# epruesse/SINA

Hardware: AMD Instinct MI355X
Metric: aligned sequences/sec (whole node), 100k full-length 16S vs SILVA-NR-scale ref (higher is better)
Workload: dtype f32

## Files before the change

include/sina_hip.h:

```cpp
#ifndef SINA_HIP_H
#define SINA_HIP_H

#include <stddef.h>
#include <stdint.h>

#ifdef __cplusplus
extern "C" {
#endif

#define SINA_HIP_ABI_VERSION 5

typedef struct sina_hip_ctx sina_hip_ctx;


int sina_hip_abi_version(void);
const char *sina_hip_last_error(void);
int sina_hip_last_error_is_limit(void);

int sina_hip_init(int device, sina_hip_ctx **ctx);
int sina_hip_fork(sina_hip_ctx *parent, sina_hip_ctx **ctx);
int sina_hip_prewarm(sina_hip_ctx *ctx, int kind);
void sina_hip_destroy(sina_hip_ctx *ctx);
int sina_hip_sync(sina_hip_ctx *ctx);


int sina_hip_upload_refs(sina_hip_ctx *ctx, const uint32_t *ab, const uint64_t *off,
                         uint32_t n_refs, uint32_t width);

int sina_hip_build_index(sina_hip_ctx *ctx, unsigned k, int nofast);

int sina_hip_download_index(sina_hip_ctx *ctx, uint32_t *offsets, uint32_t *ids);

int sina_hip_upload_index(sina_hip_ctx *ctx, unsigned k, int nofast, const uint32_t *offsets,
                          const uint32_t *ids, uint64_t n_postings);

typedef struct sina_hip_store_view {
    void *ref_ab;       uint64_t ref_ab_bytes;
    void *ref_off;      uint64_t ref_off_bytes;
    void *idx_offsets;  uint64_t idx_offsets_bytes;
    void *idx_ids;      uint64_t idx_ids_bytes;
    uint32_t n_refs, width, k, nofast;
    uint64_t n_postings, total_bases;
} sina_hip_store_view;
int sina_hip_store_view_get(sina_hip_ctx *ctx, sina_hip_store_view *view);
int sina_hip_store_alloc_like(sina_hip_ctx *ctx, sina_hip_store_view *shape);

int sina_hip_kmer_topk(sina_hip_ctx *ctx, const uint8_t *qmask, const uint64_t *qoff, uint32_t nq,
                       uint32_t max, uint32_t *out_ids, float *out_scores, uint32_t *out_n);

int sina_hip_kmer_scores(sina_hip_ctx *ctx, const uint8_t *qmask, uint32_t qlen, int16_t *scores);

#define SINA_CMP_IUPAC_OPTIMISTIC 0
#define SINA_CMP_IUPAC_PESSIMISTIC 1
#define SINA_CMP_IUPAC_EXACT 2
typedef struct sina_hip_match_counts {
    int32_t only_a_overhang, only_b_overhang, only_a, only_b, match, mismatch;
} sina_hip_match_counts;
int sina_hip_compare(sina_hip_ctx *ctx, const uint32_t *q_ab, const uint64_t *q_off, uint32_t nq,
                     const uint32_t *cand_ids, const uint64_t *cand_off, int iupac_rule, int filter_lowercase,
                     sina_hip_match_counts *out);

enum { SINA_OVERHANG_ATTACH = 0, SINA_OVERHANG_REMOVE = 1, SINA_OVERHANG_EDGE = 2 };
enum { SINA_LOWERCASE_NONE = 0, SINA_LOWERCASE_ORIGINAL = 1, SINA_LOWERCASE_UNALIGNED = 2 };
enum { SINA_INSERTION_SHIFT = 0, SINA_INSERTION_FORBID = 1, SINA_INSERTION_REMOVE = 2 };

typedef struct sina_hip_align_params {
    float match_score;
    float mismatch_score;
    float gap_penalty;
    float gap_ext_penalty;
    float fs_weight;
    int32_t overhang;
    int32_t lowercase;
    int32_t insertion;
    const float *weights;
    uint32_t n_weights;
    int32_t assemble;
} sina_hip_align_params;
void sina_hip_align_params_default(sina_hip_align_params *p);
const uint32_t *sina_hip_staged_out_pos(sina_hip_ctx *ctx);

#define SINA_HIP_MAX_QUERY_LEN 10240u

typedef struct sina_hip_graph_batch {
    uint32_t nq;
    const uint64_t *node_off;
    const uint64_t *edge_off;
    const uint32_t *node_pos;
    const uint8_t *node_mask;
    const float *node_weight;
    const uint32_t *pred_off;
    const uint32_t *pred;
    const uint32_t *succ_minpos;
    uint32_t width;
    const float *node_score16;
    const float *self_score16;
} sina_hip_graph_batch;

typedef struct sina_hip_align_out {
    uint32_t end_m, end_s;
    float raw;
    float sum_weight;
    int32_t aligned_bases;
    int32_t cutoff_head, cutoff_tail;
    uint32_t n_out;
    int32_t status;
    uint32_t assembled;
    uint32_t nast_total, nast_longest, nast_last_run;
} sina_hip_align_out;

int sina_hip_align_graphs(sina_hip_ctx *ctx, const sina_hip_graph_batch *g, const uint8_t *qmask,
                          const uint64_t *qoff, const sina_hip_align_params *p,
                          sina_hip_align_out *out, uint32_t *out_pos);

#define SINA_HIP_WIDE_CELLS ((uint64_t)1 << 29)
int sina_hip_align_graphs_any(sina_hip_ctx *ctx, const sina_hip_graph_batch *g, const uint8_t *qmask,
                              const uint64_t *qoff, const sina_hip_align_params *p,
                              sina_hip_align_out *out, uint32_t *out_pos);
int sina_hip_wide_queries(sina_hip_ctx *ctx, uint64_t *n);

int sina_hip_align_families(sina_hip_ctx *ctx, const uint32_t *fam_ids, const uint64_t *fam_off,
                            uint32_t nq, const uint8_t *qmask, const uint64_t *qoff,
                            const sina_hip_align_params *p, sina_hip_align_out *out,
                            uint32_t *out_pos);

int sina_hip_align_profiles(sina_hip_ctx *ctx, const uint32_t *fam_ids, const uint64_t *fam_off,
                            uint32_t nq, const uint8_t *qmask, const uint64_t *qoff,
                            const sina_hip_align_params *p, sina_hip_align_out *out,
                            uint32_t *out_pos);

int sina_hip_debug_mesh(sina_hip_ctx *ctx, const sina_hip_graph_batch *g, const uint8_t *qmask,
                        uint32_t qlen, const sina_hip_align_params *p, uint32_t *tb_vm,
                        uint32_t *tb_vs, float *value, int prune);

int sina_hip_debug_mesh_wide(sina_hip_ctx *ctx, const sina_hip_graph_batch *g, const uint8_t *qmask,
                             uint32_t qlen, const sina_hip_align_params *p, uint32_t *tb_vm,
                             uint32_t *tb_vs, float *value);

typedef struct sina_hip_dp_info {
    uint32_t end_m, end_s;
    float raw;
    int32_t status;
    uint32_t rows_swept, cells_swept, attempts;
    float gain0, ubound;
    uint32_t prune_step, prune_gmin;
    float scout;
} sina_hip_dp_info;
int sina_hip_debug_dp_info(sina_hip_ctx *ctx, uint32_t q, sina_hip_dp_info *out);
int sina_hip_debug_rgain(sina_hip_ctx *ctx, uint32_t n, uint32_t *out, uint32_t *cols_right );

int sina_hip_debug_family_graph(sina_hip_ctx *ctx, const uint32_t *fam_ids, uint32_t F, float fs_weight,
                                uint32_t ring_depth, uint32_t *n_nodes, uint32_t *n_edges, uint32_t *pos,
                                uint8_t *mask, float *weight, uint32_t *pred_off, uint32_t *pred,
                                uint32_t *succ_minpos, uint8_t *sink, uint32_t *spill_idx, uint32_t cap_nodes,
                                uint32_t cap_edges);

int sina_hip_debug_family_profile(sina_hip_ctx *ctx, const uint32_t *fam_ids, uint32_t F, float match,
                                  float mismatch, float gap, float gap_ext, uint32_t *n_nodes, uint32_t *pos,
                                  float *score16, float *self16, uint32_t cap_nodes);

typedef struct sina_hip_stats {
    double dp_ms;
    double backtrack_ms;
    double graph_ms;
    double kmer_count_ms;
    double kmer_select_ms;
    uint64_t dp_cells;
    uint64_t postings;
    uint32_t dp_launches, kmer_launches;
    double compare_ms;
    uint64_t compare_bases;
    uint32_t compare_launches;
    uint32_t n_dense_lists;
    double dp_busy_ms;
    uint64_t dags_built;
    uint64_t dags_used;
    uint64_t dp_rows;
    uint64_t dp_rows_swept;
    uint64_t dp_cells_swept;
    uint64_t dp_queries_pruned;
    uint64_t dp_second_attempts;
    uint64_t dp_full_sweeps;
    double dp_prune_rho;
    uint64_t graph_bytes;
    uint32_t graph_launches, kmer_queries;
    double scout_ms;
    uint32_t scout_launches, pad_;
} sina_hip_stats;
int sina_hip_get_stats(sina_hip_ctx *ctx, sina_hip_stats *s);

#ifdef __cplusplus
}
#endif
#endif
```

sina_amd/capi.py:

```python
import ctypes as C
import os

import numpy as np

_HERE = os.path.dirname(os.path.abspath(__file__))
LIB_PATH = os.path.abspath(os.environ["SINA_HIP_LIB"]) if os.environ.get("SINA_HIP_LIB") else os.path.join(_HERE, "libsina_hip.so")

u8p = C.POINTER(C.c_uint8)
u32p = C.POINTER(C.c_uint32)
u64p = C.POINTER(C.c_uint64)
f32p = C.POINTER(C.c_float)
i16p = C.POINTER(C.c_int16)

ABI_SYMBOLS = [
    "sina_hip_abi_version", "sina_hip_last_error", "sina_hip_init", "sina_hip_fork", "sina_hip_prewarm", "sina_hip_destroy",
    "sina_hip_sync",
    "sina_hip_upload_refs", "sina_hip_build_index", "sina_hip_download_index", "sina_hip_upload_index", "sina_hip_store_view_get",
    "sina_hip_store_alloc_like", "sina_hip_kmer_topk", "sina_hip_kmer_scores", "sina_hip_compare",
    "sina_hip_align_params_default", "sina_hip_staged_out_pos", "sina_hip_align_graphs", "sina_hip_align_families",
    "sina_hip_align_profiles", "sina_hip_debug_family_profile",
    "sina_hip_debug_mesh", "sina_hip_debug_family_graph", "sina_hip_debug_dp_info", "sina_hip_debug_rgain", "sina_hip_get_stats",
    "sina_hip_align_graphs_any", "sina_hip_debug_mesh_wide", "sina_hip_wide_queries", "sina_hip_last_error_is_limit",
]


class AlignParams(C.Structure):
    _fields_ = [("match_score", C.c_float), ("mismatch_score", C.c_float), ("gap_penalty", C.c_float),
                ("gap_ext_penalty", C.c_float), ("fs_weight", C.c_float), ("overhang", C.c_int32),
                ("lowercase", C.c_int32), ("insertion", C.c_int32), ("weights", f32p),
                ("n_weights", C.c_uint32), ("assemble", C.c_int32)]


class GraphBatch(C.Structure):
    _fields_ = [("nq", C.c_uint32), ("node_off", u64p), ("edge_off", u64p), ("node_pos", u32p),
                ("node_mask", u8p), ("node_weight", f32p), ("pred_off", u32p), ("pred", u32p),
                ("succ_minpos", u32p), ("width", C.c_uint32), ("node_score16", f32p), ("self_score16", f32p)]


class AlignOut(C.Structure):
    _fields_ = [("end_m", C.c_uint32), ("end_s", C.c_uint32), ("raw", C.c_float), ("sum_weight", C.c_float),
                ("aligned_bases", C.c_int32), ("cutoff_head", C.c_int32), ("cutoff_tail", C.c_int32),
                ("n_out", C.c_uint32), ("status", C.c_int32), ("assembled", C.c_uint32),
                ("nast_total", C.c_uint32), ("nast_longest", C.c_uint32), ("nast_last_run", C.c_uint32)]


ALIGN_OUT_DTYPE = np.dtype([("end_m", "<u4"), ("end_s", "<u4"), ("raw", "<f4"), ("sum_weight", "<f4"),
                            ("aligned_bases", "<i4"), ("cutoff_head", "<i4"), ("cutoff_tail", "<i4"),
                            ("n_out", "<u4"), ("status", "<i4"), ("assembled", "<u4"), ("nast_total", "<u4"),
                            ("nast_longest", "<u4"), ("nast_last_run", "<u4")])


class StoreView(C.Structure):
    _fields_ = [("ref_ab", C.c_void_p), ("ref_ab_bytes", C.c_uint64), ("ref_off", C.c_void_p),
                ("ref_off_bytes", C.c_uint64), ("idx_offsets", C.c_void_p), ("idx_offsets_bytes", C.c_uint64),
                ("idx_ids", C.c_void_p), ("idx_ids_bytes", C.c_uint64), ("n_refs", C.c_uint32),
                ("width", C.c_uint32), ("k", C.c_uint32), ("nofast", C.c_uint32), ("n_postings", C.c_uint64),
                ("total_bases", C.c_uint64)]


class Stats(C.Structure):
    _fields_ = [("dp_ms", C.c_double), ("backtrack_ms", C.c_double), ("graph_ms", C.c_double),
                ("kmer_count_ms", C.c_double), ("kmer_select_ms", C.c_double), ("dp_cells", C.c_uint64),
                ("postings", C.c_uint64), ("dp_launches", C.c_uint32), ("kmer_launches", C.c_uint32),
                ("compare_ms", C.c_double), ("compare_bases", C.c_uint64), ("compare_launches", C.c_uint32),
                ("n_dense_lists", C.c_uint32), ("dp_busy_ms", C.c_double), ("dags_built", C.c_uint64),
                ("dags_used", C.c_uint64), ("dp_rows", C.c_uint64), ("dp_rows_swept", C.c_uint64),
                ("dp_cells_swept", C.c_uint64), ("dp_queries_pruned", C.c_uint64), ("dp_second_attempts", C.c_uint64),
                ("dp_full_sweeps", C.c_uint64), ("dp_prune_rho", C.c_double), ("graph_bytes", C.c_uint64),
                ("graph_launches", C.c_uint32), ("kmer_queries", C.c_uint32), ("scout_ms", C.c_double),
                ("scout_launches", C.c_uint32), ("pad_", C.c_uint32)]


class DpInfo(C.Structure):
    _fields_ = [("end_m", C.c_uint32), ("end_s", C.c_uint32), ("raw", C.c_float), ("status", C.c_int32),
                ("rows_swept", C.c_uint32), ("cells_swept", C.c_uint32), ("attempts", C.c_uint32),
                ("gain0", C.c_float), ("ubound", C.c_float), ("prune_step", C.c_uint32), ("prune_gmin", C.c_uint32),
                ("scout", C.c_float)]


_lib = None


def load():
    global _lib
    if _lib is not None:
        return _lib
    if not os.path.exists(LIB_PATH):
        raise RuntimeError("sina_amd/libsina_hip.so is missing: run `python -c 'import __graft_entry__ as g; "
                           "g.build()'` (hipcc --offload-arch=gfx950). There is no CPU fallback.")
    L = C.CDLL(LIB_PATH)
    vp = C.c_void_p
    L.sina_hip_abi_version.restype = C.c_int
    L.sina_hip_last_error.restype = C.c_char_p
    L.sina_hip_init.argtypes = [C.c_int, C.POINTER(vp)]
    L.sina_hip_fork.argtypes = [vp, C.POINTER(vp)]
    L.sina_hip_prewarm.argtypes = [vp, C.c_int]
    L.sina_hip_destroy.argtypes = [vp]
    L.sina_hip_destroy.restype = None
    L.sina_hip_sync.argtypes = [vp]
    L.sina_hip_staged_out_pos.restype = C.POINTER(C.c_uint32)
    L.sina_hip_staged_out_pos.argtypes = [vp]
    L.sina_hip_upload_refs.argtypes = [vp, u32p, u64p, C.c_uint32, C.c_uint32]
    L.sina_hip_build_index.argtypes = [vp, C.c_uint, C.c_int]
    L.sina_hip_upload_index.argtypes = [vp, C.c_uint, C.c_int, u32p, u32p, C.c_uint64]
    L.sina_hip_download_index.argtypes = [vp, u32p, u32p]
    L.sina_hip_store_view_get.argtypes = [vp, C.POINTER(StoreView)]
    L.sina_hip_store_alloc_like.argtypes = [vp, C.POINTER(StoreView)]
    L.sina_hip_kmer_topk.argtypes = [vp, u8p, u64p, C.c_uint32, C.c_uint32, u32p, f32p, u32p]
    L.sina_hip_kmer_scores.argtypes = [vp, u8p, C.c_uint32, i16p]
    L.sina_hip_compare.argtypes = [vp, u32p, u64p, C.c_uint32, u32p, u64p, C.c_int, C.c_int, C.c_void_p]
    L.sina_hip_align_params_default.argtypes = [C.POINTER(AlignParams)]
    L.sina_hip_align_params_default.restype = None
    L.sina_hip_align_graphs.argtypes = [vp, C.POINTER(GraphBatch), u8p, u64p, C.POINTER(AlignParams),
                                        C.POINTER(AlignOut), u32p]
    L.sina_hip_align_graphs_any.argtypes = L.sina_hip_align_graphs.argtypes
    L.sina_hip_wide_queries.argtypes = [vp, u64p]
    L.sina_hip_last_error_is_limit.restype = C.c_int
    L.sina_hip_debug_mesh_wide.argtypes = [vp, C.POINTER(GraphBatch), u8p, C.c_uint32, C.POINTER(AlignParams),
                                           u32p, u32p, f32p]
    L.sina_hip_align_families.argtypes = [vp, u32p, u64p, C.c_uint32, u8p, u64p, C.POINTER(AlignParams),
                                          C.POINTER(AlignOut), u32p]
    L.sina_hip_align_profiles.argtypes = L.sina_hip_align_families.argtypes
    L.sina_hip_debug_family_profile.argtypes = [vp, u32p, C.c_uint32, C.c_float, C.c_float, C.c_float, C.c_float, u32p, u32p,
                                                f32p, f32p, C.c_uint32]
    L.sina_hip_debug_mesh.argtypes = [vp, C.POINTER(GraphBatch), u8p, C.c_uint32, C.POINTER(AlignParams),
                                      u32p, u32p, f32p, C.c_int]
    L.sina_hip_debug_family_graph.argtypes = [vp, u32p, C.c_uint32, C.c_float, C.c_uint32, u32p, u32p, u32p, u8p,
                                              f32p, u32p, u32p, u32p, u8p, u32p, C.c_uint32, C.c_uint32]
    L.sina_hip_get_stats.argtypes = [vp, C.POINTER(Stats)]
    L.sina_hip_debug_dp_info.argtypes = [vp, C.c_uint32, C.POINTER(DpInfo)]
    L.sina_hip_debug_rgain.argtypes = [vp, C.c_uint32, u32p, u32p]
    _lib = L
    return L


class SinaHipError(RuntimeError):
    pass


def _ptr(a, t):
    return a.ctypes.data_as(t)


def _c(a, dt):
    return np.ascontiguousarray(a, dtype=dt)


class Context:

    def __init__(self, device=0, _parent=None):
        self.L = load()
        self.h = C.c_void_p()
        if _parent is None:
            self._check(self.L.sina_hip_init(device, C.byref(self.h)))
        else:
            self._check(self.L.sina_hip_fork(_parent.h, C.byref(self.h)))
        self._parent = _parent
        self.device = device
        self.n_refs = 0 if _parent is None else _parent.n_refs

    def fork(self):
        return Context(self.device, _parent=self)

    def _check(self, rc):
        if rc != 0:
            raise SinaHipError(self.L.sina_hip_last_error().decode())

    def close(self):
        if self.h:
            self.L.sina_hip_destroy(self.h)
            self.h = C.c_void_p()

    def __del__(self):
        try:
# ... 91 lines not shown
        gb.succ_minpos = _ptr(arrs["succ_minpos"], u32p) if "succ_minpos" in arrs else None
        gb.width = width
        if node_score16 is not None:
            arrs["node_score16"] = _c(np.asarray(node_score16).reshape(-1), np.float32)
            arrs["self_score16"] = _c(self_score16, np.float32)
            assert len(arrs["node_score16"]) == 16 * int(node_off[nq]) and len(arrs["self_score16"]) == 16
            gb.node_score16 = _ptr(arrs["node_score16"], f32p)
            gb.self_score16 = _ptr(arrs["self_score16"], f32p)
        gb._keep = arrs
        return gb

    def align_graphs(self, gb, qmask, qoff, params=None):
        params = params or self.params()
        qmask = _c(qmask, np.uint8)
        qoff = _c(qoff, np.uint64)
        out = np.zeros(gb.nq, ALIGN_OUT_DTYPE)
        pos = np.zeros(max(len(qmask), 1), np.uint32)
        self._check(self.L.sina_hip_align_graphs(self.h, C.byref(gb), _ptr(qmask, u8p), _ptr(qoff, u64p),
                                                 C.byref(params), out.ctypes.data_as(C.POINTER(AlignOut)),
                                                 _ptr(pos, u32p)))
        return out, pos

    def align_graphs_any(self, gb, qmask, qoff, params=None, staged=False):
        params = params or self.params()
        qmask = _c(qmask, np.uint8)
        qoff = _c(qoff, np.uint64)
        out = np.zeros(gb.nq, ALIGN_OUT_DTYPE)
        pos = np.zeros(max(len(qmask), 1), np.uint32)
        self._check(self.L.sina_hip_align_graphs_any(self.h, C.byref(gb), _ptr(qmask, u8p), _ptr(qoff, u64p),
                                                     C.byref(params), out.ctypes.data_as(C.POINTER(AlignOut)),
                                                     None if staged else _ptr(pos, u32p)))
        if staged:
            n = int(qoff[-1] - qoff[0])
            pos[:n] = np.ctypeslib.as_array(self.L.sina_hip_staged_out_pos(self.h), shape=(max(n, 1),))[:n]
        return out, pos

    def wide_queries(self):
        n = C.c_uint64()
        self._check(self.L.sina_hip_wide_queries(self.h, C.byref(n)))
        return int(n.value)

    def last_error_is_limit(self):
        return bool(self.L.sina_hip_last_error_is_limit())

    def debug_mesh_wide(self, gb, qmask, params=None, want_value=True):
        params = params or self.params()
        qmask = _c(qmask, np.uint8)
        n = int(gb._keep["node_off"][1])
        L = len(qmask)
        vm = np.zeros((n, L), np.uint32)
        vs = np.zeros((n, L), np.uint32)
        val = np.zeros((n, L), np.float32) if want_value else None
        self._check(self.L.sina_hip_debug_mesh_wide(self.h, C.byref(gb), _ptr(qmask, u8p), L, C.byref(params),
                                                    _ptr(vm, u32p), _ptr(vs, u32p),
                                                    _ptr(val, f32p) if want_value else None))
        return vm, vs, val

    def compare(self, q_ab, q_off, cand_ids, cand_off, iupac=0, filter_lc=False):
        q_ab = _c(q_ab, np.uint32)
        q_off = _c(q_off, np.uint64)
        cand_ids = _c(cand_ids, np.uint32)
        cand_off = _c(cand_off, np.uint64)
        out = np.zeros((max(len(cand_ids), 1), 6), np.int32)
        self._check(self.L.sina_hip_compare(self.h, _ptr(q_ab, u32p), _ptr(q_off, u64p), len(q_off) - 1,
                                            _ptr(cand_ids, u32p), _ptr(cand_off, u64p), int(iupac),
                                            int(filter_lc), out.ctypes.data_as(C.c_void_p)))
        return out[:len(cand_ids)]

    def align_families(self, fam_ids, fam_off, qmask, qoff, params=None):
        params = params or self.params()
        fam_ids = _c(fam_ids, np.uint32)
        fam_off = _c(fam_off, np.uint64)
        qmask = _c(qmask, np.uint8)
        qoff = _c(qoff, np.uint64)
        nq = len(qoff) - 1
        out = np.zeros(nq, ALIGN_OUT_DTYPE)
        pos = np.zeros(max(len(qmask), 1), np.uint32)
        self._check(self.L.sina_hip_align_families(self.h, _ptr(fam_ids, u32p), _ptr(fam_off, u64p), nq,
                                                   _ptr(qmask, u8p), _ptr(qoff, u64p), C.byref(params),
                                                   out.ctypes.data_as(C.POINTER(AlignOut)), _ptr(pos, u32p)))
        return out, pos

    def align_profiles(self, fam_ids, fam_off, qmask, qoff, params=None):
        params = params or self.params()
        fam_ids = _c(fam_ids, np.uint32)
        fam_off = _c(fam_off, np.uint64)
        qmask = _c(qmask, np.uint8)
        qoff = _c(qoff, np.uint64)
        nq = len(qoff) - 1
        out = np.zeros(nq, ALIGN_OUT_DTYPE)
        pos = np.zeros(max(len(qmask), 1), np.uint32)
        self._check(self.L.sina_hip_align_profiles(self.h, _ptr(fam_ids, u32p), _ptr(fam_off, u64p), nq,
                                                   _ptr(qmask, u8p), _ptr(qoff, u64p), C.byref(params),
                                                   out.ctypes.data_as(C.POINTER(AlignOut)), _ptr(pos, u32p)))
        return out, pos

    def debug_family_profile(self, fam_ids, match, mismatch, gap, gap_ext):
        fam_ids = _c(fam_ids, np.uint32)
        cap = 65536
        nn = C.c_uint32()
        pos = np.zeros(cap, np.uint32)
        sc = np.zeros((cap, 16), np.float32)
        own = np.zeros(16, np.float32)
        self._check(self.L.sina_hip_debug_family_profile(self.h, _ptr(fam_ids, u32p), len(fam_ids), match, mismatch, gap,
                                                         gap_ext, C.byref(nn), _ptr(pos, u32p), _ptr(sc, f32p),
                                                         _ptr(own, f32p), cap))
        return pos[:nn.value].copy(), sc[:nn.value].copy(), own

    def debug_mesh(self, gb, qmask, params=None, want_value=True, prune=False):
        params = params or self.params()
        qmask = _c(qmask, np.uint8)
        n = int(gb._keep["node_off"][1])
        L = len(qmask)
        vm = np.zeros((n, L), np.uint32)
        vs = np.zeros((n, L), np.uint32)
        val = np.zeros((n, L), np.float32) if want_value else None
        self._check(self.L.sina_hip_debug_mesh(self.h, C.byref(gb), _ptr(qmask, u8p), L, C.byref(params),
                                               _ptr(vm, u32p), _ptr(vs, u32p),
                                               _ptr(val, f32p) if want_value else None, 1 if prune else 0))
        return vm, vs, val

    def debug_family_graph(self, fam_ids, fs_weight=1.0, ring_depth=4):
        fam_ids = _c(fam_ids, np.uint32)
        cap_n, cap_e = 65536, 400000
        nn, ne = C.c_uint32(), C.c_uint32()
        pos = np.zeros(cap_n, np.uint32)
        mask = np.zeros(cap_n, np.uint8)
        w = np.zeros(cap_n, np.float32)
        poff = np.zeros(cap_n + 1, np.uint32)
        pred = np.zeros(cap_e, np.uint32)
        smin = np.zeros(cap_n, np.uint32)
        sink = np.zeros(cap_n, np.uint8)
        spill = np.zeros(cap_n, np.uint32)
        self._check(self.L.sina_hip_debug_family_graph(self.h, _ptr(fam_ids, u32p), len(fam_ids), fs_weight,
                                                       ring_depth, C.byref(nn), C.byref(ne), _ptr(pos, u32p),
                                                       _ptr(mask, u8p), _ptr(w, f32p), _ptr(poff, u32p),
                                                       _ptr(pred, u32p), _ptr(smin, u32p), _ptr(sink, u8p),
                                                       _ptr(spill, u32p), cap_n, cap_e))
        n, e = nn.value, ne.value
        return dict(n=n, pos=pos[:n].copy(), mask=mask[:n].copy(), weight=w[:n].copy(), pred_off=poff[:n + 1].copy(),
                    pred=pred[:e].copy(), succ_minpos=smin[:n].copy(), sink=sink[:n].copy(), spill=spill[:n].copy())

    def dp_info(self, q=0):
        d = DpInfo()
        self._check(self.L.sina_hip_debug_dp_info(self.h, q, C.byref(d)))
        return {f[0]: getattr(d, f[0]) for f in DpInfo._fields_}

    def rgain(self, n):
        out = np.zeros(max(n, 1), np.uint32)
        cols = np.zeros(max(n, 1), np.uint32)
        self._check(self.L.sina_hip_debug_rgain(self.h, n, _ptr(out, u32p), _ptr(cols, u32p)))
        return out[:n], cols[:n]

    def stats(self):
        s = Stats()
        self._check(self.L.sina_hip_get_stats(self.h, C.byref(s)))
        return {f[0]: getattr(s, f[0]) for f in Stats._fields_}
```

sina_amd/csrc/api.hip:

```cpp
#include <algorithm>
#include <cmath>
#include <cstdlib>
#include <cstring>

#include "common.h"
#include "ctx.h"

namespace sina_hip {

static thread_local std::string g_last_error;
static thread_local bool g_last_error_is_limit = false;
void set_error(const std::string &msg) {
    g_last_error = msg;
    g_last_error_is_limit = false;
}
void set_limit_error(const std::string &msg) {
    g_last_error = msg;
    g_last_error_is_limit = true;
}

int plan_dp(sina_hip_ctx *c, uint32_t maxL, DpPlan *pl) {
    if (!pick_geom(maxL, &pl->geom)) SH_FAIL_LIMIT("align: query longer than SINA_HIP_MAX_QUERY_LEN bases");
    const size_t slot = dp_slot_bytes(pl->geom), fixed = dp_fixed_lds_bytes(pl->geom);
    size_t budget = c->lds_budget ? c->lds_budget : dp_default_lds_budget(pl->geom);
// ... 19 lines not shown
    pp.kappa64 = 64.0f * 1.0001f * kappa;
    pp.amax = prune_gain_units(wmax, pp.kappa64);
    if (pp.amax > 250u || (uint64_t)pp.amax * maxL >= (1u << 23)) return pp;
    if (pp.kappa64 <= 0.f) pp.kappa64 = 1e-30f;
    DpGeom g;
    if (pick_geom(maxL, &g) && g.T <= 64) return pp;
    pp.on = 1;
    return pp;
}

struct HostPrep {
    std::vector<QDesc> qd;
    std::vector<uint4> rec;
    std::vector<uint2> rgain;
    bool rgain_ok = true;
    float wmax = 0.f, wmin = 0.f;
    std::vector<uint32_t> pred;
    std::vector<uint32_t> last;
    uint64_t tb_cells = 0, spill_rows = 0, cells = 0;
};

static int prep_range(const sina_hip_graph_batch *g, const uint64_t *qoff, uint32_t q0, uint32_t q1, int Lp, int W,
                       HostPrep *hp, float kappa64, uint32_t *spill_q) {
    const uint64_t nbase = g->node_off[q0], ebase = g->edge_off[q0];
    const uint64_t nn = g->node_off[q1] - nbase;
    hp->qd.resize(q1 - q0);
    hp->rec.resize(nn);
    hp->rgain.assign(kappa64 > 0.f ? nn : 0, uint2{0u, 0u});
    hp->rgain_ok = true;
    hp->pred.resize(g->edge_off[q1] - ebase + 8);
    hp->tb_cells = hp->spill_rows = hp->cells = 0;
    uint32_t erec_cursor = 0;
    for (uint32_t q = q0; q < q1; q++) {
        QDesc &d = hp->qd[q - q0];
        const uint64_t no = g->node_off[q], eo = g->edge_off[q];
        const uint32_t N = (uint32_t)(g->node_off[q + 1] - no);
        d.node_off = no - nbase;
        d.erec_off = erec_cursor;
        erec_cursor += dp_edge_entries(N);
        d.edge_off = eo - ebase;
        d.q_off = qoff[q] - qoff[q0];
        d.tb_off = hp->tb_cells;
        d.spill_off = hp->spill_rows;
        d.N = N;
        d.L = (uint32_t)(qoff[q + 1] - qoff[q]);
        const uint32_t *po = g->pred_off + no + q;
        uint4 *rec = hp->rec.data() + d.node_off;
        for (uint32_t m = 0; m < N; m++) {
            if (po[m + 1] < po[m]) SH_FAIL("align_graphs: a node has more than 255 predecessors (or pred_off is not ascending)");
            if (po[m + 1] - po[m] > 255u)
                SH_FAIL_LIMIT("align_graphs: a node has more than 255 predecessors (or pred_off is not ascending)");
            for (uint32_t e = po[m]; e < po[m + 1]; e++)
                if (g->pred[eo + e] >= m) SH_FAIL("align_graphs: predecessor ids must be smaller than the node's id");
            uint32_t wbits;
            memcpy(&wbits, &g->node_weight[no + m], 4);
            rec[m].x = po[m];
            rec[m].y = wbits;
            rec[m].z = ((po[m + 1] - po[m]) & 0xffu) | ((uint32_t)(g->node_mask[no + m] & 0xffu) << 8) | kRecSink;
            rec[m].w = kRowNone;
        }
        std::vector<uint32_t> &last = hp->last;
        last.assign(N, 0);
        for (uint32_t m = 0; m < N; m++) {
            for (uint32_t e = po[m]; e < po[m + 1]; e++) {
                const uint32_t p = g->pred[eo + e];
                rec[p].z &= ~kRecSink;
                last[p] = m;
                if (m - p > (uint32_t)kFarLds) rec[p].z |= kRecFence;
            }
        }
        d.first_sink = 0;
        d.gmin = 0;
        for (uint32_t m = 0; m < N; m++)
            if (rec[m].z & kRecSink) {
                d.first_sink = m;
                break;
            }
        uint32_t nsp = 0;
        uint32_t free_at[64];
        const uint32_t seg_len = dp_slot_segment(N);
        for (uint32_t m = 0; m < N; m++) {
            if (m % seg_len == 0)
                for (int x = 0; x < W; x++) free_at[x] = 0;
            if (rec[m].z & kRecSink) continue;
            if (last[m] == m + 1) continue;
            int slot = -1;
            const uint32_t seg_end = std::min<uint32_t>(N, (m / seg_len + 1) * seg_len);
            if (!(rec[m].z & kRecFence) && last[m] < seg_end)
                for (int x = 0; x < W; x++)
                    if (free_at[x] <= m) {
                        slot = x;
                        break;
                    }
            if (slot >= 0) {
                free_at[slot] = last[m];
                rec[m].w = (uint32_t)slot;
            } else {
                rec[m].w = kRowSpilled | nsp++;
            }
        }
        for (uint32_t m = 0; m < N; m++) {
            uint32_t first_far = 0;
            uint32_t dist = po[m + 1] > po[m] ? 0u : kRecDistFar;
            for (uint32_t e = po[m]; e < po[m + 1]; e++) {
                const uint32_t p = g->pred[eo + e];
                const uint32_t pw = rec[p].w == kRowNone ? 0u : rec[p].w;
                const bool sp = (pw & kRowSpilled) != 0;
                if (sp && first_far == 0) first_far = e - po[m] + 1;
                dist = std::max(dist, m - p);
                hp->pred[d.edge_off + e] = p | ((pw & 0x7FFFu) << 16) | (sp ? kPredSpilled : 0u);
            }
            rec[m].z |= (first_far << 24) | (std::min(dist, kRecDistFar) << kRecDistShift);
        }
        if (nsp > kMaxSpillRows) {
            if (spill_q) *spill_q = q;
            SH_FAIL_LIMIT("align_graphs: too many spill rows for one query");
        }
        if (kappa64 > 0.f) {
            uint2 *rg = hp->rgain.data() + d.node_off;
            const uint32_t *pos = g->node_pos + no;
            bool ok = true;
            for (uint32_t m = 0; m < N && ok; m++) {
                if (m > 0 && pos[m] < pos[m - 1]) ok = false;
                for (uint32_t e = po[m]; e < po[m + 1] && ok; e++)
                    if (pos[g->pred[eo + e]] >= pos[m]) ok = false;
            }
            if (!ok) hp->rgain_ok = false;
            uint32_t right = 0, cols_right = 0, gmin = 0xFFFFFFFFu;
            for (uint32_t m = N; ok && m > 0;) {
                uint32_t first = m - 1, mx = 0;
                while (first > 0 && pos[first - 1] == pos[m - 1]) first--;
                for (uint32_t j = first; j < m; j++) {
                    mx = std::max(mx, prune_gain_units(g->node_weight[no + j], kappa64));
                    rg[j] = uint2{right, last[j] | (cols_right << 16)};
                }
                right += mx;
                cols_right++;
                gmin = std::min(gmin, mx);
                m = first;
            }
            d.gmin = ok ? gmin : 0u;
        }
        d.n_spill = nsp;
        hp->spill_rows += nsp;
        hp->tb_cells += (uint64_t)N * Lp;
        hp->cells += (uint64_t)N * d.L;
    }
    return 0;
}

int run_dp_device(sina_hip_ctx *c, const DpPlan &pl, const QDesc *qd_host, uint32_t bq, uint64_t n_node_entries,
                  uint64_t tb_cells, uint64_t spill_rows, uint64_t cells, uint64_t nqm, const sina_hip_align_params *p, uint32_t width,
                  sina_hip_align_out *out, uint32_t *out_pos, bool want_dbg_value, const PrunePlan &pp,
                  const uint32_t *chain_ref) {
    hipStream_t s = c->stream;
    const int Lp = pl.geom.Lp();
    const bool weighted = p->weights != nullptr && p->n_weights > 0;
    const bool forbid = p->insertion == SINA_INSERTION_FORBID;
    uint64_t edge_entries = 0;
    for (uint32_t q = 0; q < bq; q++) edge_entries += dp_edge_entries(qd_host[q].N);
    (void)n_node_entries;
    if (c->spill.reserve(std::max<uint64_t>(spill_rows, 1) * 8 * (uint64_t)Lp) ||
        c->edge.reserve(std::max<uint64_t>(1, (uint64_t)(pl.geom.T / 64 - 1) * edge_entries) * sizeof(EdgeRec)) ||
        c->res.reserve(sizeof(DpResult) * bq) || c->out.reserve(sizeof(sina_hip_align_out) * bq) ||
        c->out_pos.reserve(4 * std::max<uint64_t>(nqm, 1)))
        return 1;
    if (want_dbg_value && c->dbg.reserve(4 * tb_cells)) return 1;
    std::vector<uint32_t> order(bq);
    for (uint32_t q = 0; q < bq; q++) order[q] = q;
    std::stable_sort(order.begin(), order.end(), [&](uint32_t x, uint32_t y) {
        return (uint64_t)qd_host[x].N * qd_host[x].L > (uint64_t)qd_host[y].N * qd_host[y].L;
    });
    if (c->order.reserve(4 * (size_t)bq)) return 1;
    if (upload(c, 0, c->order.p, order.data(), 4 * (size_t)bq, s)) return 1;
    DpArgs a;
    a.dry = DryArgs{nullptr, nullptr, 0};
    a.qd = c->qd.as<QDesc>();
    a.order = c->order.as<uint32_t>();
    a.rec = c->rec.as<uint4>();
    a.pred = c->pred.as<uint32_t>();
    a.node_pos = c->node_pos.as<uint32_t>();
    a.succ_minpos = c->succ_minpos.as<uint32_t>();
    a.qmask = c->qmask.as<uint8_t>();
    a.tb = nullptr;
    a.dbg_value = want_dbg_value ? c->dbg.as<float>() : nullptr;
    a.spill = c->spill.as<float>();
    a.edge = c->edge.as<EdgeRec>();
    a.edge_stride = edge_entries;
    a.res = c->res.as<DpResult>();
    a.weights = weighted ? c->weights.as<float>() : nullptr;
    a.n_weights = weighted ? p->n_weights : 0;
    a.ms = -p->match_score;
    a.mms = -p->mismatch_score;
    a.gp = p->gap_penalty;
    a.gpe = p->gap_ext_penalty;
    a.prof16 = c->profile_batch ? c->prof16.as<float>() : nullptr;
    c->last_bq = bq;
    c->last_prune_step = pp.on ? pp.amax : 0u;
    a.reach = pp.on ? c->rgain.as<uint2>() : nullptr;
    a.prune = pp.on;
    a.prune_amax = pp.amax;
    a.prune_rho = 0.f;
    bool rho_fixed = false;
    if (pp.on) {
        if (const std::string r = test_knob("rho"); !r.empty()) {
            a.prune_rho = (float)atof(r.c_str());
            rho_fixed = a.prune_rho > 0.f;
        }
        if (!rho_fixed) {
            std::lock_guard<std::mutex> slk(c->st->stats_mu);
            a.prune_rho = c->st->prune_rho;
        }
    }
    {
        uint32_t max_n = 0;
        for (uint32_t q = 0; q < bq; q++) max_n = std::max<uint32_t>(max_n, qd_host[q].N);
        a.below_init = (!weighted && !forbid && dp_below_init(max_n, a.gp, a.gpe)) ? 1 : 0;
    }
    a.scout_u = nullptr;
    a.scout_bias = (float)atof(test_knob("scout_add").c_str());
    c->last_scout = false;
    if (const std::string fixed = test_knob("scout_set"); !fixed.empty() && pp.on && !rho_fixed) {
        std::vector<float> vals(bq, (float)atof(fixed.c_str()));
        if (c->scout_u.reserve(4 * (size_t)bq)) return 1;
        if (upload(c, 7, c->scout_u.p, vals.data(), 4 * (size_t)bq, s)) return 1;
        a.scout_u = c->scout_u.as<float>();
        c->last_scout = true;
    } else if (chain_ref != nullptr && pp.on && !rho_fixed && a.below_init && a.gp >= a.gpe && pl.geom.T > 64 && test_knob("scout") != "0") {
        if (c->scout.reserve(4 * (size_t)bq) || c->scout_u.reserve(4 * (size_t)bq)) return 1;
        if (upload(c, 7, c->scout.p, chain_ref, 4 * (size_t)bq, s)) return 1;
        SH_CHECK(hipEventRecord(c->ev[3], s));
        if (launch_chain_scout(a, bq, c->st->ref_ab.as<uint32_t>(), c->st->ref_off.as<uint64_t>(), c->scout.as<uint32_t>(),
                               c->scout_u.as<float>(), s))
            return 1;
        SH_CHECK(hipEventRecord(c->ev[4], s));
        SH_CHECK(wait_event(c->ev[4]));
        float sms = 0;
        SH_CHECK(hipEventElapsedTime(&sms, c->ev[3], c->ev[4]));
        {
            std::lock_guard<std::mutex> slk(c->st->stats_mu);
            c->st->stats.scout_ms += sms;
            c->st->stats.scout_launches++;
        }
        a.scout_u = c->scout_u.as<float>();
        c->last_scout = true;
    }
    if (a.scout_u != nullptr && !rho_fixed) {
        std::lock_guard<std::mutex> slk(c->st->stats_mu);
        a.prune_rho = c->st->prune_rho_guard;
    }
    const uint64_t tb_bytes = tb_cell_bytes(forbid) * tb_cells;
    tb_plane_lease plane;
    if (plane.acquire(c, std::max<uint64_t>(tb_bytes, 16))) return 1;
    c->last_tb = plane.ptr;
    a.tb = plane.ptr;
    if (want_dbg_value && pp.on) SH_CHECK(hipMemsetD32Async(reinterpret_cast<hipDeviceptr_t>(c->dbg.p), 0x49742400 , tb_cells, s));
    if (c->dbg_planes && !forbid) SH_CHECK(hipMemsetD16Async(reinterpret_cast<hipDeviceptr_t>(plane.ptr), (unsigned short)kTbNone, tb_cells, s));

    BtArgs b;
    b.qd = a.qd;
    b.rec = a.rec;
    b.pred = a.pred;
    b.node_pos = a.node_pos;
    b.tb = a.tb;
    b.res = a.res;
    b.weights = a.weights;
    b.n_weights = a.n_weights;
    b.out = c->out.as<sina_hip_align_out>();
    b.out_pos = c->out_pos.as<uint32_t>();
    b.nq = bq;
    b.width = width;
    b.Lp = (uint32_t)Lp;
    b.ms = a.ms;
    b.overhang = p->overhang;
    b.lazy_sidx = forbid ? 0 : 1;
    b.qmask = a.qmask;
    b.lowercase = p->lowercase;
    b.self16 = c->profile_batch ? c->self16.as<float>() : nullptr;
    b.asm_cap = 0;
    for (uint32_t q = 0; q < bq; q++) b.asm_cap = std::max<uint32_t>(b.asm_cap, qd_host[q].L);
    uint64_t dp_no = ~0ull;
    bool bt_done = false;
    {
        SH_CHECK(hipEventRecord(c->ev[8], s));
        s = c->stream_dp;
        SH_CHECK(hipStreamWaitEvent(s, c->ev[8], 0));
        heavy_launch hl(c, s, kHeavyDp);
        SH_CHECK(hipEventRecord(c->ev[0], hl.stream()));
        a.dry = hl.dry();
        if (launch_mesh_dp(pl.geom, weighted, forbid, a, bq, pl.lds, hl.stream())) return 1;
        SH_CHECK(hipEventRecord(c->ev[1], hl.stream()));
        if (hl.lk.owns_lock() && c->st->dp_end[0]) {
            dp_no = c->st->dp_seq++;
            SH_CHECK(hipEventRecord(c->st->dp_end[dp_no % 8], hl.stream()));
            c->st->dp_end_no[dp_no % 8].store(dp_no, std::memory_order_release);
        }
        if (hl.chained) {
            if (launch_backtrack(b, hl.stream())) return 1;
            if (p->assemble && launch_assemble(b, hl.stream())) return 1;
            SH_CHECK(hipEventRecord(c->ev[2], hl.stream()));
            bt_done = true;
        }
        if (hl.done()) return 1;
    }
    if (!bt_done) {
        if (launch_backtrack(b, s)) return 1;
        if (p->assemble && launch_assemble(b, s)) return 1;
        SH_CHECK(hipEventRecord(c->ev[2], s));
    }
    if (c->h_out.reserve(sizeof(sina_hip_align_out) * bq) || c->h_res.reserve(sizeof(DpResult) * bq)) return 1;
    unsigned char *staged_pos = static_cast<unsigned char *>(c->h_out_pos.p) + 4 * c->out_pos_base;
    SH_CHECK(hipMemcpyAsync(c->h_out.p, c->out.p, sizeof(sina_hip_align_out) * bq, hipMemcpyDeviceToHost, s));
    SH_CHECK(hipMemcpyAsync(c->h_res.p, c->res.p, sizeof(DpResult) * bq, hipMemcpyDeviceToHost, s));
    SH_CHECK(hipMemcpyAsync(staged_pos, c->out_pos.p, 4 * nqm, hipMemcpyDeviceToHost, s));
    SH_CHECK(wait_stream(c, s));
    memcpy(out, c->h_out.p, sizeof(sina_hip_align_out) * bq);
    if (out_pos) memcpy(out_pos, staged_pos, 4 * nqm);
    float ms = 0;
    SH_CHECK(hipEventElapsedTime(&ms, c->ev[0], c->ev[1]));
    float shared = 0;
    if (dp_no != ~0ull && dp_no > 0 && c->st->dp_end_no[(dp_no - 1) % 8].load(std::memory_order_acquire) == dp_no - 1) {
        float to_prev_end = 0;
        const hipError_t e = hipEventElapsedTime(&to_prev_end, c->ev[0], c->st->dp_end[(dp_no - 1) % 8]);
        if (e == hipSuccess && c->st->dp_end_no[(dp_no - 1) % 8].load(std::memory_order_acquire) == dp_no - 1)
            shared = std::min(ms, std::max(0.f, to_prev_end));
        else (void)hipGetLastError();
    }
    const uint32_t kstrip = 64u * (uint32_t)pl.geom.B;
    uint64_t rows_nominal = 0, rows_swept = 0, cells_swept = 0, n_pruned = 0, n_second = 0, n_full = 0;
    std::vector<float> ratios;
    const DpResult *hres = c->h_res.as<DpResult>();
    for (uint32_t q = 0; q < bq; q++) {
        const uint64_t strips = (qd_host[q].L - 1) / kstrip + 1;
        rows_nominal += strips * qd_host[q].N;
        const DpResult &r = hres[q];
        if (r.attempts == 0) {
            rows_swept += strips * qd_host[q].N;
            cells_swept += (uint64_t)qd_host[q].N * qd_host[q].L;
            continue;
        }
        rows_swept += r.rows_done;
        cells_swept += r.cells_done;
        n_pruned++;
        n_second += r.attempts == 2 ? 1 : 0;
        n_full += r.attempts >= 3 ? 1 : 0;
        if (r.status == 0 && r.gain0 > 0.f && r.raw < 0.f) ratios.push_back(-r.raw / r.gain0);
    }
    float rho_seen = -1.f, rho_guard_seen = -1.f;
    if (!ratios.empty()) {
        rho_seen = *std::min_element(ratios.begin(), ratios.end()) - 0.015f;
        const size_t at = ratios.size() / 50;
        std::nth_element(ratios.begin(), ratios.begin() + (std::ptrdiff_t)at, ratios.end());
        rho_guard_seen = ratios[at] - 0.015f;
    }
    std::lock_guard<std::mutex> slk(c->st->stats_mu);
    c->st->stats.dp_ms += ms;
    c->st->stats.dp_busy_ms += ms - shared;
    SH_CHECK(hipEventElapsedTime(&ms, c->ev[1], c->ev[2]));
    c->st->stats.backtrack_ms += ms;
    c->st->stats.dp_cells += cells;
    c->st->stats.dp_launches++;
    c->st->stats.dp_rows += rows_nominal;
    c->st->stats.dp_rows_swept += rows_swept;
    c->st->stats.dp_cells_swept += cells_swept;
    c->st->stats.dp_queries_pruned += n_pruned;
    c->st->stats.dp_second_attempts += n_second;
    c->st->stats.dp_full_sweeps += n_full;
    if (rho_seen > 0.f) {
        float &rho = c->st->prune_rho;
        rho = rho_seen < rho ? rho_seen : 0.5f * (rho + rho_seen);
        rho = std::min(0.99f, std::max(0.05f, rho));
        float &rg = c->st->prune_rho_guard;
        rg = rho_guard_seen < rg ? rho_guard_seen : 0.5f * (rg + rho_guard_seen);
        rg = std::min(0.99f, std::max(0.05f, rg));
    }
    c->st->stats.dp_prune_rho = c->st->prune_rho;
    return 0;
}

int make_streams(sina_hip_ctx *c) {
    SH_CHECK(hipStreamCreateWithFlags(&c->stream, hipStreamNonBlocking));
    SH_CHECK(hipStreamCreateWithFlags(&c->stream_dp, hipStreamNonBlocking));
    return 0;
}

int upload_weights(sina_hip_ctx *c, const sina_hip_align_params *p) {
    if (p->weights != nullptr && p->n_weights > 0) {
        if (c->weights.reserve(sizeof(float) * p->n_weights)) return 1;
        SH_CHECK(hipMemcpyAsync(c->weights.p, p->weights, sizeof(float) * p->n_weights, hipMemcpyHostToDevice,
                                c->stream));
    }
    return 0;
}

static bool weighted_scheme(const sina_hip_align_params *p) { return p->weights != nullptr && p->n_weights > 0; }

static int align_graphs_impl(sina_hip_ctx *c, const sina_hip_graph_batch *g, const uint8_t *qmask,
                             const uint64_t *qoff, const sina_hip_align_params *p, sina_hip_align_out *out,
// ... 322 lines not shown
    c->free_all();
    for (auto &e : c->ev) (void)hipEventDestroy(e);
    (void)hipStreamDestroy(c->stream);
    if (c->stream_dp) (void)hipStreamDestroy(c->stream_dp);
    delete c;
}

int sina_hip_sync(sina_hip_ctx *c) {
    if (!c) SH_FAIL("sync: null ctx");
    SH_CHECK(hipSetDevice(c->device));
    SH_CHECK(hipStreamSynchronize(c->stream));
    SH_CHECK(hipStreamSynchronize(c->stream_dp));
    if (c->st->heavy) SH_CHECK(hipStreamSynchronize(c->st->heavy));
    if (c->st->heavy2) SH_CHECK(hipStreamSynchronize(c->st->heavy2));
    return 0;
}

const uint32_t *sina_hip_staged_out_pos(sina_hip_ctx *c) {
    return c ? static_cast<const uint32_t *>(c->h_out_pos.p) : nullptr;
}

void sina_hip_align_params_default(sina_hip_align_params *p) {
    memset(p, 0, sizeof(*p));
    p->match_score = 2;
    p->mismatch_score = -1;
    p->gap_penalty = 5;
    p->gap_ext_penalty = 2;
    p->fs_weight = 1;
    p->overhang = SINA_OVERHANG_ATTACH;
    p->lowercase = SINA_LOWERCASE_NONE;
    p->insertion = SINA_INSERTION_SHIFT;
}

int sina_hip_upload_refs(sina_hip_ctx *c, const uint32_t *ab, const uint64_t *off, uint32_t n_refs,
                         uint32_t width) {
    if (!c || !ab || !off) SH_FAIL("upload_refs: null argument");
    if (!c->owns_store) SH_FAIL("upload_refs: a forked context cannot change the reference store");
    std::lock_guard<std::mutex> lk(c->mu);
    SH_CHECK(hipSetDevice(c->device));
    const uint64_t total = off[n_refs];
    if (c->st->ref_ab.reserve(4 * std::max<uint64_t>(total, 1)) || c->st->ref_off.reserve(8 * ((uint64_t)n_refs + 1)))
        return 1;
    SH_CHECK(hipMemcpyAsync(c->st->ref_ab.p, ab, 4 * total, hipMemcpyHostToDevice, c->stream));
    SH_CHECK(hipMemcpyAsync(c->st->ref_off.p, off, 8 * ((uint64_t)n_refs + 1), hipMemcpyHostToDevice, c->stream));
    SH_CHECK(hipStreamSynchronize(c->stream));
    {
        std::lock_guard<std::mutex> alk(c->st->aux_mu);
        c->st->ref_off_host.assign(off, off + n_refs + 1);
        c->st->ref_off_host_ready.store(true, std::memory_order_release);
    }
    c->st->n_refs = n_refs;
    c->st->width = width;
    c->st->total_bases = total;
    c->st->have_refs = true;
    return 0;
}

int sina_hip_align_graphs(sina_hip_ctx *c, const sina_hip_graph_batch *g, const uint8_t *qmask,
                          const uint64_t *qoff, const sina_hip_align_params *p, sina_hip_align_out *out,
                          uint32_t *out_pos) {
    if (!c) SH_FAIL("align_graphs: null ctx");
    std::lock_guard<std::mutex> lk(c->mu);
    sina_hip_hint_guard hints(c);
    return align_graphs_impl(c, g, qmask, qoff, p, out, out_pos, nullptr, nullptr, nullptr);
}

int sina_hip_align_graphs_any(sina_hip_ctx *c, const sina_hip_graph_batch *g, const uint8_t *qmask,
                              const uint64_t *qoff, const sina_hip_align_params *p, sina_hip_align_out *out,
                              uint32_t *out_pos) {
    if (!c) SH_FAIL("align_graphs_any: null ctx");
    std::lock_guard<std::mutex> lk(c->mu);
    sina_hip_hint_guard hints(c);
    return align_graphs_any_impl(c, g, qmask, qoff, p, out, out_pos);
}

int sina_hip_wide_queries(sina_hip_ctx *c, uint64_t *n) {
    if (!c || !n) SH_FAIL("wide_queries: null argument");
    std::lock_guard<std::mutex> lk(c->mu);
    *n = c->wide_queries;
    return 0;
}

int sina_hip_debug_mesh_wide(sina_hip_ctx *c, const sina_hip_graph_batch *g, const uint8_t *qmask, uint32_t qlen,
                             const sina_hip_align_params *p, uint32_t *tb_vm, uint32_t *tb_vs, float *value) {
    if (!c || !g || g->nq != 1 || !qmask || !p || !tb_vm || !tb_vs) SH_FAIL("debug_mesh_wide: needs exactly one query");
    std::lock_guard<std::mutex> lk(c->mu);
    SH_CHECK(hipSetDevice(c->device));
    if (p->insertion == SINA_INSERTION_FORBID && !g->succ_minpos) SH_FAIL("debug_mesh_wide: insertion=forbid needs succ_minpos");
    if (g->node_score16 != nullptr && (!g->self_score16 || weighted_scheme(p)))
        SH_FAIL("debug_mesh_wide: a profile batch needs self_score16 and takes no positional weights");
    const uint64_t qoff[2] = {0, qlen};
    std::vector<uint8_t> wide;
    if (classify_any(g, qoff, true, &wide)) return 1;
    if (c->h_out_pos.reserve(4 * std::max<uint64_t>(qlen, 1))) return 1;
    sina_hip_align_out o;
    const uint32_t q0 = 0;
    return run_wide(c, g, qmask, qoff, p, &q0, 1, &o, nullptr, tb_vm, tb_vs, value);
}

int sina_hip_debug_mesh(sina_hip_ctx *c, const sina_hip_graph_batch *g, const uint8_t *qmask, uint32_t qlen,
                        const sina_hip_align_params *p, uint32_t *tb_vm, uint32_t *tb_vs, float *value, int prune) {
    if (!c || !g || g->nq != 1 || !tb_vm || !tb_vs) SH_FAIL("debug_mesh: needs exactly one query");
    std::lock_guard<std::mutex> lk(c->mu);
    struct no_prune_scope {
        sina_hip_ctx *c;
        ~no_prune_scope() { c->no_prune = false; }
    } scope{c};
    c->no_prune = prune == 0;
    const uint64_t qoff[2] = {0, qlen};
    sina_hip_align_out o;
    std::vector<uint32_t> pos(qlen);
    return align_graphs_impl(c, g, qmask, qoff, p, &o, pos.data(), value, tb_vm, tb_vs);
}

int sina_hip_debug_dp_info(sina_hip_ctx *c, uint32_t q, sina_hip_dp_info *out) {
    if (!c || !out) SH_FAIL("debug_dp_info: null argument");
    std::lock_guard<std::mutex> lk(c->mu);
    if (q >= c->last_bq || !c->res.p) SH_FAIL("debug_dp_info: no such query in the last launch");
    SH_CHECK(hipSetDevice(c->device));
    DpResult r;
    SH_CHECK(hipMemcpy(&r, c->res.as<DpResult>() + q, sizeof r, hipMemcpyDeviceToHost));
    out->end_m = r.end_m;
    out->end_s = r.end_s;
    out->raw = r.raw;
    out->status = r.status;
    out->rows_swept = r.rows_done;
    out->cells_swept = r.cells_done;
    out->attempts = r.attempts;
    out->gain0 = r.gain0;
    out->ubound = r.ubound;
    out->prune_step = c->last_prune_step;
    QDesc d;
    SH_CHECK(hipMemcpy(&d, c->qd.as<QDesc>() + q, sizeof d, hipMemcpyDeviceToHost));
    out->prune_gmin = d.gmin;
    out->scout = NAN;
    if (c->last_scout && c->scout_u.p) SH_CHECK(hipMemcpy(&out->scout, c->scout_u.as<float>() + q, sizeof(float), hipMemcpyDeviceToHost));
    return 0;
}

int sina_hip_debug_rgain(sina_hip_ctx *c, uint32_t n, uint32_t *out, uint32_t *cols_right) {
    if (!c || !out) SH_FAIL("debug_rgain: null argument");
    std::lock_guard<std::mutex> lk(c->mu);
    if (!c->rgain.p || c->rgain.cap < 8 * (size_t)n) SH_FAIL("debug_rgain: no bound of that many nodes on the device");
    SH_CHECK(hipSetDevice(c->device));
    std::vector<uint2> tmp(n);
    SH_CHECK(hipMemcpy(tmp.data(), c->rgain.p, 8 * (size_t)n, hipMemcpyDeviceToHost));
    for (uint32_t i = 0; i < n; i++) {
        out[i] = tmp[i].x;
        if (cols_right) cols_right[i] = tmp[i].y >> 16;
    }
    return 0;
}

int sina_hip_get_stats(sina_hip_ctx *c, sina_hip_stats *s) {
    if (!c || !s) SH_FAIL("get_stats: null argument");
    std::lock_guard<std::mutex> slk(c->st->stats_mu);
    *s = c->st->stats;
    s->n_dense_lists = c->st->dense_ready.load() ? c->st->n_dense : 0;
    return 0;
}

}
```

sina_amd/csrc/common.h:

```cpp
#pragma once

#include <hip/hip_runtime.h>
#include <stdint.h>

#include <algorithm>
#include <atomic>
#include <mutex>
#include <string>
#include <vector>

#include <cstdio>
#include <cstdlib>
#include <ctime>

#include "sina_hip.h"

namespace sina_hip {

void set_error(const std::string &msg);
void set_limit_error(const std::string &msg);

inline std::string test_knob(const char *key) {
    const char *e = getenv("SINA_HIP_TEST");
    if (!e) return std::string();
// ... 37 lines not shown
        if (bytes <= cap) return 0;
        if (p) (void)hipFree(p);
        p = nullptr;
        cap = 0;
        size_t want = bytes + bytes / 4 + 4096;
        if (hint) want = std::max(want, hint->load(std::memory_order_relaxed));
        trace_alloc(want);
        SH_CHECK(hipMalloc(&p, want));
        cap = want;
        return 0;
    }
    static void trace_alloc(size_t bytes) {
        static const bool on = getenv("SINA_HIP_TRACE_ALLOC") != nullptr;
        if (on) {
            timespec ts;
            clock_gettime(CLOCK_MONOTONIC, &ts);
            fprintf(stderr, "[sina_hip] %.3f hipMalloc %.1f MB\n", ts.tv_sec % 1000 + ts.tv_nsec * 1e-9, bytes / 1048576.0);
        }
    }
    int reserve_exact(size_t bytes) {
        if (bytes <= cap) return 0;
        if (p) (void)hipFree(p);
        p = nullptr;
        cap = 0;
        trace_alloc(bytes);
        SH_CHECK(hipMalloc(&p, bytes));
        cap = bytes;
        return 0;
    }
    void release() {
        if (p) (void)hipFree(p);
        p = nullptr;
        cap = 0;
    }
    template <typename T> T *as() const { return reinterpret_cast<T *>(p); }
};

struct HostBuf {
    void *p = nullptr;
    size_t cap = 0;
    int reserve(size_t bytes) {
        if (bytes <= cap) return 0;
        if (p) (void)hipHostFree(p);
        p = nullptr;
        cap = 0;
        const size_t want = bytes + bytes / 4 + 4096;
        if (getenv("SINA_HIP_TRACE_ALLOC")) {
            timespec ts;
            clock_gettime(CLOCK_MONOTONIC, &ts);
            fprintf(stderr, "[sina_hip] %.3f hipHostMalloc %.1f MB\n", ts.tv_sec % 1000 + ts.tv_nsec * 1e-9, want / 1048576.0);
        }
        SH_CHECK(hipHostMalloc(&p, want, hipHostMallocDefault));
        cap = want;
        return 0;
    }
    void release() {
        if (p) (void)hipHostFree(p);
        p = nullptr;
        cap = 0;
    }
    template <typename T> T *as() const { return reinterpret_cast<T *>(p); }
};

struct DryArgs {
    uint32_t *counter, *flag;
    uint32_t seq;
};
#ifdef __HIPCC__
__device__ __forceinline__ void dry_signal(const DryArgs &d, uint32_t n_workgroups, bool one_thread) {
    if (d.counter != nullptr && one_thread) {
        if (atomicAdd(d.counter, 1u) == n_workgroups - 1u) {
            __hip_atomic_store(d.counter, 0u, __ATOMIC_RELAXED, __HIP_MEMORY_SCOPE_AGENT);
            __hip_atomic_fetch_max(d.flag, d.seq, __ATOMIC_RELEASE, __HIP_MEMORY_SCOPE_SYSTEM);
        }
    }
}
#endif


struct QDesc {
    uint64_t node_off;
    uint64_t edge_off;
    uint64_t q_off;
    uint64_t tb_off;
    uint64_t spill_off;
    uint32_t N, L;
    uint32_t n_spill;
    uint32_t erec_off;
    uint32_t first_sink;
    uint32_t gmin;
};
static_assert(sizeof(QDesc) == 64, "uploaded as an array");

constexpr uint32_t kRecSink = 1u << 16;
constexpr uint32_t kRecFence = 1u << 17;
constexpr int kRecDistShift = 18;
constexpr uint32_t kRecDistFar = 63u;
constexpr uint32_t kRowNone = 0xFFFFFFFFu;
constexpr uint32_t kRowSpilled = 0x80000000u;
constexpr uint32_t kPredSpilled = 0x80000000u;
constexpr uint32_t kMaxSpillRows = 32768;
constexpr int kFarLds = 192;
__host__ __device__ inline uint32_t dp_slot_segment(uint32_t n_rows) {
    const uint32_t s = (n_rows + 15u) / 16u;
    return s < 256u ? 256u : s;
}

struct EdgeRec {
    float bnd;
    float xv;
    uint32_t xe;
    uint32_t gmax;
};
static_assert(sizeof(EdgeRec) == 16, "read back with one 16-byte scalar load");
inline uint32_t dp_edge_entries(uint32_t n_rows) { return (n_rows + 3u) & ~3u; }

constexpr uint32_t kTbSMask = 0x3FFFu;
constexpr uint32_t kTbExt = 1u << 14;
constexpr uint32_t kTbOpLast = 1u << 15;
static_assert(SINA_HIP_MAX_QUERY_LEN <= kTbSMask, "value_sidx field of the 32-bit trace-back cell");
constexpr uint32_t kTbTypeMask = 3u;
constexpr uint32_t kTbDel = 0u, kTbMatch = 1u, kTbIns = 2u, kTbNone = 3u;
constexpr uint32_t kTb16Ext = 1u << 2;
constexpr uint32_t kTb16XLast = 1u << 3;
constexpr int kTb16OrdShift = 4;
inline size_t tb_cell_bytes(bool forbid) { return forbid ? 4 : 2; }

struct DpResult {
    uint32_t end_m, end_s;
    float raw;
    int32_t status;
    uint32_t rows_done, cells_done, attempts;
    float gain0, ubound;
    uint32_t pad_;
};
static_assert(sizeof(DpResult) == 40, "downloaded as an array");

constexpr float kPruneUnit = 1.0f / 64.0f;
__host__ __device__ inline uint32_t prune_gain_units(float w, float kappa64) {
    const float x = w * kappa64;
    uint32_t u = (uint32_t)x;
    if ((float)u < x) u++;
    return u + 1u;
}
struct PrunePlan {
    int on = 0;
    float kappa64 = 0.f;
    uint32_t amax = 0;
};

inline bool dp_below_init(uint32_t max_n, float gp, float gpe) {
    return gp >= 0.f && gpe >= 0.f && 1.0f + (float)max_n * gp * 1.01f + gp + gpe < 900000.0f;
}

struct DpArgs {
    const QDesc *qd;
    const uint32_t *order;
    const uint4 *rec;
    const uint32_t *pred;
    const uint32_t *node_pos;
    const uint32_t *succ_minpos;
    const uint8_t *qmask;
    int below_init;
    void *tb;
    float *dbg_value;
    float *spill;
    EdgeRec *edge;
    uint64_t edge_stride;
    DpResult *res;
    const float *weights;
    uint32_t n_weights;
    float ms, mms, gp, gpe;
    const float *prof16;
    DryArgs dry;
    const uint2 *reach;
    int prune;
    float prune_rho;
    uint32_t prune_amax;
    float scout_bias;
    const float *scout_u;
};

struct BtArgs {
    const QDesc *qd;
    const uint4 *rec;
    const uint32_t *pred;
    const uint32_t *node_pos;
    const void *tb;
    const DpResult *res;
    const float *weights;
    uint32_t n_weights;
    sina_hip_align_out *out;
    uint32_t *out_pos;
    uint32_t nq, width, Lp;
    float ms;
    int overhang;
    int lazy_sidx;
    const uint8_t *qmask;
    int lowercase;
    uint32_t asm_cap;
    const float *self16;
};

struct DpGeom {
    int T, B;
    int Lp() const { return T * B; }
};
bool pick_geom(uint32_t maxL, DpGeom *g);
#ifndef SINA_DP_SIMPLE_WAVES8
#define SINA_DP_SIMPLE_WAVES8 3
#endif
constexpr int dp_waves_per_simd(int B) { return B <= 4 ? 5 : (B <= 8 ? SINA_DP_SIMPLE_WAVES8 : 2); }
size_t dp_slot_bytes(const DpGeom &g);
size_t dp_fixed_lds_bytes(const DpGeom &g);
int dp_max_ring(const DpGeom &g);
size_t dp_default_lds_budget(const DpGeom &g);
int launch_mesh_dp(const DpGeom &g, bool weighted, bool forbid, const DpArgs &a, uint32_t nq,
                   size_t lds_bytes, hipStream_t s);
constexpr int kScoutBand = 8;
int launch_chain_scout(const DpArgs &a, uint32_t nq, const uint32_t *ref_ab, const uint64_t *ref_off,
                       const uint32_t *chain_ref , float *out_u , hipStream_t s);
int launch_backtrack(const BtArgs &a, hipStream_t s);
bool backtrack_by_lanes(const BtArgs &a);
int launch_assemble(const BtArgs &a, hipStream_t s);
int allow_full_lds(const void *kernel);

struct DpPlan {
    DpGeom geom;
    int W;
    size_t lds;
};

}

struct sina_hip_ctx;

namespace sina_hip {
int plan_dp(sina_hip_ctx *c, uint32_t maxL, DpPlan *pl);
int upload_weights(sina_hip_ctx *c, const sina_hip_align_params *p);
int run_dp_device(sina_hip_ctx *c, const DpPlan &pl, const QDesc *qd_host, uint32_t bq, uint64_t n_node_entries,
                  uint64_t tb_cells, uint64_t spill_rows, uint64_t cells, uint64_t nqm, const sina_hip_align_params *p, uint32_t width,
                  sina_hip_align_out *out, uint32_t *out_pos, bool want_dbg_value, const PrunePlan &pp,
                  const uint32_t *chain_ref = nullptr);
PrunePlan prune_plan(const sina_hip_align_params *p, float wmax, float wmin, uint32_t maxL, bool profile_batch);

}
```

sina_amd/csrc/ctx.h:

```cpp
#pragma once

#include <atomic>
#include <algorithm>
#include <condition_variable>
#include <cmath>
#include <cstring>

#include "common.h"

struct sina_hip_store {
    sina_hip::DevBuf ref_ab, ref_off, idx_off, idx_ids;
    std::vector<uint64_t> ref_off_host;
    std::atomic<bool> ref_off_host_ready{false};
    uint32_t n_refs = 0, width = 0, k = 0, nofast = 0;
    uint64_t n_postings = 0, total_bases = 0;
    bool have_refs = false, have_index = false;
    sina_hip::DevBuf dense_id, dense_bits;
    uint32_t n_dense = 0, dense_words = 0;
    std::atomic<bool> dense_ready{false};
    std::mutex aux_mu;
    std::mutex stats_mu;
    hipStream_t heavy = nullptr;
    std::mutex heavy_mu;
    hipStream_t heavy2 = nullptr;
// ... 257 lines not shown
    for (;;) {
        const hipError_t e = hipEventQuery(ev);
        if (e != hipErrorNotReady) return e;
        if (timeout_s > 0.0) {
            timespec t1;
            clock_gettime(CLOCK_MONOTONIC, &t1);
            if ((double)(t1.tv_sec - t0.tv_sec) + 1e-9 * (double)(t1.tv_nsec - t0.tv_nsec) > timeout_s) return hipErrorNotReady;
        }
        timespec ts{0, ns};
        nanosleep(&ts, nullptr);
        if (ns < 1000000) ns += ns / 2;
    }
}
inline hipError_t wait_stream(sina_hip_ctx *c, hipStream_t s) {
    const hipError_t e = hipEventRecord(c->ev[9], s);
    return e != hipSuccess ? e : wait_event(c->ev[9]);
}
inline int upload(sina_hip_ctx *c, int slot, void *dst, const void *src, size_t bytes, hipStream_t s) {
    if (bytes == 0) return 0;
    if (c->h_stage[slot].reserve(bytes)) return 1;
    memcpy(c->h_stage[slot].p, src, bytes);
    SH_CHECK(hipMemcpyAsync(dst, c->h_stage[slot].p, bytes, hipMemcpyHostToDevice, s));
    return 0;
}
inline int download(sina_hip_ctx *c, int slot, const void *src, size_t bytes, hipStream_t s) {
    if (bytes == 0) return 0;
    if (c->h_stage[slot].reserve(bytes)) return 1;
    SH_CHECK(hipMemcpyAsync(c->h_stage[slot].p, src, bytes, hipMemcpyDeviceToHost, s));
    return 0;
}
inline bool chain_kernels() {
    static const bool on = [] {
        const char *v = getenv("SINA_HIP_CHAIN");
        if (v && *v) return *v != '0';
        const char *pmc = getenv("ROCPROF_COUNTER_COLLECTION");
        return !(pmc && *pmc && *pmc != '0');
    }();
    return on;
}
enum heavy_kind { kHeavyKmer = 0, kHeavyGraph = 1, kHeavyDp = 2 };
constexpr int kHeavyDepth = 2;
struct heavy_launch {
    sina_hip_ctx *c;
    hipStream_t own, hs;
    std::unique_lock<std::mutex> lk;
    bool failed = false;
    int turn = 0;
    int kind = 0;
    bool signals_dry = false;
    bool admitted = false;
    bool chained = false;
    uint32_t my_seq = 0;
    heavy_launch(sina_hip_ctx *c_, hipStream_t own_, int kind_ = kHeavyKmer) : c(c_), own(own_), hs(own_), kind(kind_) {
        if (!c->st->heavy) return;
        sina_hip_store *st = c->st;
        if (st->wedged.load(std::memory_order_relaxed)) {
            failed = true;
            return;
        }
        failed = hipEventRecord(c->ev[10], own) != hipSuccess;
        lk = std::unique_lock<std::mutex>(st->heavy_mu);
        const bool chain = chain_kernels() && st->heavy2 && st->dry_mem && !st->chain_broken.load(std::memory_order_relaxed);
        chained = chain;
        if (chain) {
            const uint64_t me = st->heavy_ticket++;
            st->heavy_waiting.push_back({me, kind});
            st->heavy_cv.wait(lk, [&] {
                if (st->heavy_outstanding >= kHeavyDepth) return false;
                auto oldest_of = [&](int k) {
                    const sina_hip_store::heavy_waiter *o = nullptr;
                    for (const auto &w : st->heavy_waiting)
                        if ((k < 0 || w.kind == k) && (!o || w.ticket < o->ticket)) o = &w;
                    return o;
                };
                const sina_hip_store::heavy_waiter *pick = oldest_of(kHeavyGraph);
                if (!pick) pick = oldest_of(kHeavyKmer);
                if (!pick) pick = oldest_of(-1);
                return pick && pick->ticket == me;
            });
            for (size_t i = 0; i < st->heavy_waiting.size(); i++)
                if (st->heavy_waiting[i].ticket == me) {
                    st->heavy_waiting.erase(st->heavy_waiting.begin() + (std::ptrdiff_t)i);
                    break;
                }
            ++st->heavy_outstanding;
            admitted = true;
        }
        turn = chain ? st->heavy_turn : 0;
        hs = turn ? st->heavy2 : st->heavy;
        failed = failed || hipStreamWaitEvent(hs, c->ev[10], 0) != hipSuccess;
        if (chain && st->heavy_prev_any) {
            if (st->heavy_prev_dry)
                failed = failed || hipStreamWaitValue32(hs, st->dry_flag, st->heavy_prev_seq, hipStreamWaitValueGte, 0xffffffffu) != hipSuccess;
            else
                failed = failed || hipStreamWaitEvent(hs, st->heavy_done[turn ^ 1], 0) != hipSuccess;
        }
        if (chain) my_seq = ++st->heavy_seq;
    }
    hipStream_t stream() const { return hs; }
    DryArgs dry() {
        DryArgs d{nullptr, nullptr, 0};
        sina_hip_store *st = c->st;
        if (!lk.owns_lock() || !chained) return d;
        d.flag = st->dry_flag;
        d.counter = st->dry_mem + my_seq % sina_hip_store::kDryCounters;
        d.seq = my_seq;
        signals_dry = true;
        return d;
    }
    int done() {
        if (hs == own) return failed ? 1 : 0;
        failed = failed || hipEventRecord(c->ev[11], hs) != hipSuccess;
        if (lk.owns_lock()) {
            sina_hip_store *st = c->st;
            if (chained) {
                failed = failed || hipEventRecord(st->heavy_done[turn], hs) != hipSuccess;
                st->heavy_prev_dry = signals_dry && !failed;
                st->heavy_prev_seq = my_seq;
                st->heavy_prev_any = true;
                st->heavy_turn = turn ^ 1;
            }
            lk.unlock();
            c->st->heavy_cv.notify_all();
        }
        const hipError_t we = wait_event(c->ev[11], chained ? kChainTimeoutS : 0.0);
        if (we == hipErrorNotReady) {
            c->st->chain_broken.store(true, std::memory_order_relaxed);
            c->st->wedged.store(true, std::memory_order_relaxed);
            leave();
            set_error("heavy_launch: a chained launch did not end within 120 s -- a tool that serialises kernels across "
                      "queues? (set SINA_HIP_CHAIN=0); the store takes no further launches, its buffers stay allocated");
            return 1;
        }
        failed = failed || we != hipSuccess;
        leave();
        if (failed) set_error("heavy_launch: event hand-over failed");
        return failed ? 1 : 0;
    }
    void leave() {
        if (!admitted) return;
        admitted = false;
        sina_hip_store *st = c->st;
        if (!lk.owns_lock()) lk = std::unique_lock<std::mutex>(st->heavy_mu);
        --st->heavy_outstanding;
        lk.unlock();
        st->heavy_cv.notify_all();
    }
    ~heavy_launch() { leave(); }
};
}

namespace sina_hip {
constexpr int kFamilyMax = 128;
constexpr int kBuiltWords = 8;
struct BuiltGraphs {
    uint32_t ncap = 0;
    std::vector<uint64_t> pred_off;
    std::vector<uint32_t> sizes;
};
using family_builder = int (*)(sina_hip_ctx *c, const uint32_t *fam_ids, const uint64_t *fam_off, uint32_t q0, uint32_t n,
                               const sina_hip_align_params *p, int W, const PrunePlan &pp, BuiltGraphs *bg);
int align_family_batches(sina_hip_ctx *c, const char *who, family_builder build, bool profile_batch, const uint32_t *fam_ids,
                         const uint64_t *fam_off, uint32_t nq, const uint8_t *qmask, const uint64_t *qoff,
                         const sina_hip_align_params *p, sina_hip_align_out *out, uint32_t *out_pos);
}

namespace sina_hip {
uint64_t wide_budget_cells();
int run_wide(sina_hip_ctx *c, const sina_hip_graph_batch *g, const uint8_t *qmask, const uint64_t *qoff,
             const sina_hip_align_params *p, const uint32_t *qs, uint32_t n, sina_hip_align_out *out, uint32_t *out_pos,
             uint32_t *dbg_vm = nullptr, uint32_t *dbg_vs = nullptr, float *dbg_value = nullptr);
}

struct sina_hip_hint_guard {
    sina_hip_ctx *c;
    explicit sina_hip_hint_guard(sina_hip_ctx *c) : c(c) {}
    ~sina_hip_hint_guard() { c->publish_hints(); }
};
```

sina_amd/csrc/graph_build.hip:

```cpp
#include <algorithm>
#include <cstring>
#include <type_traits>

#include "common.h"
#include "ctx.h"

namespace sina_hip {
namespace {

#ifndef SINA_GRAPH_THREADS
#define SINA_GRAPH_THREADS 512
#endif
#ifndef SINA_GRAPH_MINWAVES
#define SINA_GRAPH_MINWAVES 8
#endif
constexpr int kGT = SINA_GRAPH_THREADS;
constexpr uint32_t kNoPrev = 0xFFFFu;
constexpr int kMaxFam = kFamilyMax;
constexpr int kSz = kBuiltWords;
#ifndef SINA_GRAPH_KTC
#define SINA_GRAPH_KTC 128
#endif
#ifndef SINA_GRAPH_TNW
#define SINA_GRAPH_TNW 512
#endif
constexpr int kTC = SINA_GRAPH_KTC;
constexpr int kTNW = SINA_GRAPH_TNW;
static_assert(kTC % 64 == 0 && kTC < 255 && kTNW >= 32 && kTNW % 2 == 0, "tile geometry");
static_assert((kMaxFam * (kTC / 64) + SINA_GRAPH_THREADS / 64 - 1) / (SINA_GRAPH_THREADS / 64) <= 64, "far-entry flags of a wave fit 64 bits");

#ifdef SINA_DP_PROFILE
__device__ unsigned long long g_graph_prof[16];
#define GP_DECL unsigned long long gp_[16] = {}; unsigned long long gt_ = __builtin_amdgcn_s_memtime();
#define GP(i) { const unsigned long long t_ = __builtin_amdgcn_s_memtime(); gp_[i] += t_ - gt_; gt_ = t_; }
#define GP_FLUSH if (threadIdx.x == 0) { for (int i_ = 0; i_ < 16; i_++) atomicAdd(&g_graph_prof[i_], gp_[i_]); }
#else
#define GP_DECL
#define GP(i)
#define GP_FLUSH
#endif

struct GraphArgs {
    const uint32_t *ref_ab;
    const uint64_t *ref_off;
    const uint32_t *fam_ids;
    const uint64_t *fam_off;
    const uint64_t *pred_off;
    const float *wtab;
    uint4 *rec;
    uint32_t *node_pos;
    uint32_t *succ_min;
    uint32_t *far_mark;
    uint32_t *pred;
    uint32_t *sizes;
    uint32_t width, ncap;
    uint32_t tile_bytes;
    uint32_t bitmap_off;
    uint32_t member_off;
    uint32_t member_cap;
    uint32_t fam_cap;
    int W;
    int want_smin;
    uint2 *reach;
    float kappa64;
};

struct Member {
    uint64_t beg;
    uint32_t len;
    uint32_t cur, curn;
    uint32_t carry, carryn;
    uint32_t id;
};
static_assert(sizeof(Member) == 32, "LDS layout");
constexpr uint32_t kOCpos = 0;
constexpr uint32_t kONbase = kOCpos + 4 * kTC;
constexpr uint32_t kOPres = kONbase + 4 * (kTC + 2);
constexpr uint32_t kOWA = kOPres + 4 * kTC;
constexpr uint32_t kOWC = kOWA + 4 * kTNW;
constexpr uint32_t kOWD = kOWC + 4 * kTNW;
constexpr uint32_t kOWB = (kOWD + 4 * kTNW + 7) & ~7u;
constexpr uint32_t kOLi = kOWB + 8 * kTNW;
constexpr uint32_t kONn = kOLi + 32 * kTC;
constexpr uint32_t kONfar = kONn + kTC;
constexpr uint32_t kOMask = kONfar + kTNW;
constexpr uint32_t kONcol = kOMask + kTNW;
constexpr uint32_t kOE = (kONcol + kTNW + 15) & ~15u;

template <typename In, typename Out>
__device__ uint32_t block_exscan(const In *in, Out *out, uint32_t n, uint32_t *tmp) {
    const uint32_t tid = threadIdx.x;
    const uint32_t chunk = (n + kGT - 1) / kGT;
    const uint32_t b = min(n, tid * chunk), e = min(n, b + chunk);
    uint32_t s = 0;
    for (uint32_t i = b; i < e; i++) s += (uint32_t)in[i];
    uint32_t x = s;
    const int lane = tid & 63, wave = tid >> 6;
#pragma unroll
    for (int off = 1; off < 64; off <<= 1) {
        const uint32_t y = __shfl_up(x, off);
        if (lane >= off) x += y;
    }
    if (lane == 63) tmp[wave] = x;
    __syncthreads();
    uint32_t base = 0, total = 0;
    for (int w = 0; w < kGT / 64; w++) {
        if (w < wave) base += tmp[w];
        total += tmp[w];
    }
    uint32_t run = base + x - s;
    __syncthreads();
    for (uint32_t i = b; i < e; i++) {
        const uint32_t v = (uint32_t)in[i];
        out[i] = (Out)run;
        run += v;
    }
    __syncthreads();
    return total;
}

template <typename Get, typename Out>
__device__ uint32_t block_exscan_f(uint32_t n, Get get, Out *out, uint32_t *tmp) {
    const uint32_t tid = threadIdx.x;
    const uint32_t chunk = (n + kGT - 1) / kGT;
    const uint32_t b = min(n, tid * chunk), e = min(n, b + chunk);
    uint32_t s = 0;
    for (uint32_t i = b; i < e; i++) s += get(i);
    uint32_t x = s;
    const int lane = tid & 63, wave = tid >> 6;
#pragma unroll
    for (int off = 1; off < 64; off <<= 1) {
        const uint32_t y = __shfl_up(x, off);
        if (lane >= off) x += y;
    }
    if (lane == 63) tmp[wave] = x;
    __syncthreads();
    uint32_t base = 0, total = 0;
    for (int w = 0; w < kGT / 64; w++) {
        if (w < wave) base += tmp[w];
        total += tmp[w];
    }
    uint32_t run = base + x - s;
    __syncthreads();
    for (uint32_t i = b; i < e; i++) {
        const uint32_t v = get(i);
        out[i] = (Out)run;
        run += v;
    }
    __syncthreads();
    return total;
}

__device__ __attribute__((noinline)) void fill_tile(const uint32_t *__restrict__ ref_ab, uint32_t bitmap_off, uint32_t member_off,
                                                    uint32_t nwords, uint32_t n_tasks, uint32_t c0, uint32_t tc) {
    extern __shared__ __attribute__((aligned(16))) unsigned char smem[];
    uint32_t *cposT = reinterpret_cast<uint32_t *>(smem + kOCpos);
    uint32_t *presT = reinterpret_cast<uint32_t *>(smem + kOPres);
    uint16_t *eE = reinterpret_cast<uint16_t *>(smem + kOE);
    const uint32_t *bitmap = reinterpret_cast<const uint32_t *>(smem + bitmap_off);
    const uint16_t *wrank = reinterpret_cast<const uint16_t *>(bitmap + nwords);
    Member *mb = reinterpret_cast<Member *>(smem + member_off);
    constexpr uint32_t kEAbsent = 0x00FFu, kEFirst = 1u << 13;
    constexpr uint32_t kCH = kTC / 64, kNW = kGT / 64;
    const uint32_t wave = (uint32_t)__builtin_amdgcn_readfirstlane((int)(threadIdx.x >> 6));
    const uint32_t lane = threadIdx.x & 63u;
    auto rank = [&](uint32_t pos) -> uint32_t {
        return (uint32_t)wrank[pos >> 5] + __popc(bitmap[pos >> 5] & ((1u << (pos & 31)) - 1u));
    };
        for (uint32_t t4 = wave; t4 < n_tasks; t4 += 8 * kNW) {
            uint32_t abv[8];
#pragma unroll
            for (int u = 0; u < 8; u++) {
                const uint32_t task = t4 + (uint32_t)u * kNW;
                abv[u] = 0xFFFFFFFFu;
                if (task < n_tasks) {
                    const uint32_t j = task / kCH;
                    const uint32_t cur = (uint32_t)__builtin_amdgcn_readfirstlane((int)mb[j].cur);
                    const uint32_t len = (uint32_t)__builtin_amdgcn_readfirstlane((int)mb[j].len);
                    const uint64_t beg = mb[j].beg;
                    const uint64_t begs = ((uint64_t)(uint32_t)__builtin_amdgcn_readfirstlane((int)(uint32_t)(beg >> 32)) << 32) |
                                          (uint32_t)__builtin_amdgcn_readfirstlane((int)(uint32_t)beg);
                    const uint32_t i = cur + (task % kCH) * 64u + lane;
                    if (i < len) abv[u] = ref_ab[begs + i];
                }
            }
#pragma unroll
            for (int u = 0; u < 8; u++) {
                const uint32_t task = t4 + (uint32_t)u * kNW;
                if (task >= n_tasks) continue;
                const uint32_t j = task / kCH, slot0 = (task % kCH) * 64u, slot = slot0 + lane;
                const uint32_t cur = (uint32_t)__builtin_amdgcn_readfirstlane((int)mb[j].cur);
                uint32_t ev = kEAbsent;
                if (abv[u] != 0xFFFFFFFFu) {
                    const uint32_t ab = abv[u];
                    const uint32_t pos = ab & 0xFFFFFFu;
                    const uint32_t c = rank(pos) - c0;
                    if (c < tc) {
                        const uint32_t m = (ab >> 24) & 0x1Fu;
                        ev = c | (m << 8) | (cur + slot == 0 ? kEFirst : 0u);
                        atomicOr(&presT[c], 1u << m);
                        cposT[c] = pos;
                    }
                }
                eE[j * (uint32_t)kTC + slot] = (uint16_t)ev;
                const uint32_t n_in = (uint32_t)__popcll(__builtin_amdgcn_ballot_w64(ev != kEAbsent));
                if (n_in && lane == 0) atomicMax(&mb[j].curn, cur + slot0 + n_in);
            }
        }
}

__device__ __forceinline__ uint32_t node_of_entry(uint32_t ev) {
    extern __shared__ __attribute__((aligned(16))) unsigned char smem[];
    const uint32_t *nbaseT = reinterpret_cast<const uint32_t *>(smem + kONbase);
    const uint32_t *presT = reinterpret_cast<const uint32_t *>(smem + kOPres);
    const uint8_t *liOf = smem + kOLi;
    const uint32_t c = ev & 0xFFu, m = (ev >> 8) & 31u;
    const uint32_t b = nbaseT[c];
    return b + liOf[b + __popc(presT[c] & ((1u << m) - 1u))];
}
__global__ void __launch_bounds__(kGT) __attribute__((amdgpu_waves_per_eu(SINA_GRAPH_MINWAVES, SINA_GRAPH_MINWAVES))) family_graph_kernel(GraphArgs a) {
    extern __shared__ __attribute__((aligned(16))) unsigned char smem[];
    __shared__ uint32_t s_tmp[kGT / 64 + 8];
    const uint32_t q = blockIdx.x, tid = threadIdx.x;
    const uint32_t nwords = (a.width + 31) / 32;
    const uint64_t f0 = a.fam_off[q];
    const uint32_t F = (uint32_t)(a.fam_off[q + 1] - f0);
    uint32_t *cposT = reinterpret_cast<uint32_t *>(smem + kOCpos);
    uint32_t *nbaseT = reinterpret_cast<uint32_t *>(smem + kONbase);
    uint32_t *presT = reinterpret_cast<uint32_t *>(smem + kOPres);
    uint32_t *wA = reinterpret_cast<uint32_t *>(smem + kOWA);
    uint32_t *wC = reinterpret_cast<uint32_t *>(smem + kOWC);
    uint32_t *wD = reinterpret_cast<uint32_t *>(smem + kOWD);
    unsigned long long *wB = reinterpret_cast<unsigned long long *>(smem + kOWB);
    uint8_t *liOf = smem + kOLi;
    uint8_t *nn = smem + kONn;
    uint8_t *nfarN = smem + kONfar;
    uint8_t *maskN = smem + kOMask;
    uint8_t *ncolN = smem + kONcol;
    uint16_t *eE = reinterpret_cast<uint16_t *>(smem + kOE);
    uint32_t *bitmap = reinterpret_cast<uint32_t *>(smem + a.bitmap_off);
    uint16_t *wrank = reinterpret_cast<uint16_t *>(bitmap + nwords);
    Member *mb = reinterpret_cast<Member *>(smem + a.member_off);
    constexpr uint32_t kEFirst = 1u << 13;
    constexpr uint32_t kCH = kTC / 64, kNW = kGT / 64;
    const uint32_t wave = (uint32_t)__builtin_amdgcn_readfirstlane((int)(threadIdx.x >> 6));
    const uint32_t lane = threadIdx.x & 63u;
    const uint32_t n_tasks = F * kCH;

    uint32_t *sz = a.sizes + kSz * (size_t)q;
    for (uint32_t j = tid; j < F; j += kGT) {
        const uint32_t id = a.fam_ids[f0 + j];
        mb[j].id = id;
        mb[j].beg = a.ref_off[id];
        mb[j].len = (uint32_t)(a.ref_off[id + 1] - a.ref_off[id]);
        mb[j].cur = mb[j].curn = 0;
        mb[j].carry = mb[j].carryn = kNoPrev;
    }
    for (uint32_t i = tid; i < nwords; i += kGT) bitmap[i] = 0;
    __syncthreads();
    GP_DECL

    for (uint32_t j0 = 0; j0 < F; j0 += 8) {
        uint32_t maxlen = 0;
#pragma unroll
        for (int u = 0; u < 8; u++) maxlen = max(maxlen, j0 + u < F ? mb[j0 + u].len : 0u);
        for (uint32_t i = tid; i < maxlen; i += kGT) {
            uint32_t ab[8];
#pragma unroll
            for (int u = 0; u < 8; u++)
                ab[u] = (j0 + u < F && i < mb[j0 + u].len) ? a.ref_ab[mb[j0 + u].beg + i] : 0xFFFFFFFFu;
#pragma unroll
            for (int u = 0; u < 8; u++)
                if (ab[u] != 0xFFFFFFFFu) {
                    const uint32_t pos = ab[u] & 0xFFFFFFu;
                    atomicOr(&bitmap[pos >> 5], 1u << (pos & 31));
                }
        }
    }
    __syncthreads();
    GP(0)
    {
        const uint32_t chunk = (nwords + kGT - 1) / kGT;
        const uint32_t b = min(nwords, tid * chunk), e = min(nwords, b + chunk);
        uint32_t s = 0;
        for (uint32_t i = b; i < e; i++) s += __popc(bitmap[i]);
        uint32_t x = s;
        const int lane = tid & 63, wave = tid >> 6;
#pragma unroll
        for (int off = 1; off < 64; off <<= 1) {
            const uint32_t y = __shfl_up(x, off);
            if (lane >= off) x += y;
        }
        if (lane == 63) s_tmp[wave] = x;
        __syncthreads();
        uint32_t base = 0, total = 0;
        for (int w = 0; w < kGT / 64; w++) {
            if (w < wave) base += s_tmp[w];
            total += s_tmp[w];
        }
        uint32_t run = base + x - s;
        for (uint32_t i = b; i < e; i++) {
            wrank[i] = (uint16_t)run;
            run += __popc(bitmap[i]);
        }
        if (tid == 0) s_tmp[kGT / 64] = total;
    }
    __syncthreads();
    const uint32_t NC = s_tmp[kGT / 64];
    if (NC > 65535u) {
        if (tid == 0) {
            sz[0] = NC;
            sz[1] = sz[2] = 0;
            sz[3] = 2;
        }
        return;
    }
    auto rank = [&](uint32_t pos) -> uint32_t {
        return (uint32_t)wrank[pos >> 5] + __popc(bitmap[pos >> 5] & ((1u << (pos & 31)) - 1u));
    };
    uint4 *rec = a.rec + (size_t)q * a.ncap;
    uint32_t *node_pos = a.node_pos + (size_t)q * a.ncap;
    uint32_t *smin = a.succ_min + (size_t)q * a.ncap;
    uint32_t *last = a.far_mark + (size_t)q * a.ncap;
    uint32_t *pred = a.pred + a.pred_off[q];
    const float *wt = a.wtab + (size_t)F * (kMaxFam + 1);
    uint32_t N = 0, E = 0;
    GP(1)

    for (uint32_t c0 = 0; c0 < NC; c0 += kTC) {
        const uint32_t tc = min((uint32_t)kTC, NC - c0);
        for (uint32_t i = tid; i < (uint32_t)kTC; i += kGT) presT[i] = 0;
        __syncthreads();
        GP(2)
        fill_tile(a.ref_ab, a.bitmap_off, a.member_off, nwords, n_tasks, c0, tc);
        __syncthreads();
        for (uint32_t c = tid; c < tc; c += kGT) nn[c] = (uint8_t)__popc(presT[c]);
        __syncthreads();
        GP(3)
        const uint32_t tn = block_exscan(nn, nbaseT, tc, s_tmp);
        if (tid == 0) nbaseT[tc] = tn;
        for (uint32_t ln = tid; ln < tn; ln += kGT)
            if (N + ln < a.ncap) {
                last[N + ln] = 0;
                if (a.want_smin) smin[N + ln] = 0xFFFFFFFFu;
            }
        __syncthreads();
        GP(5)
        uint32_t te = 0;
        for (uint32_t ca = 0; ca < tc;) {
            const uint32_t w0 = nbaseT[ca];
            uint32_t cb = tc;
            if (tn - w0 > (uint32_t)kTNW) {
                uint32_t lo = ca + 1, hi = tc;
                while (lo < hi) {
                    const uint32_t mid = (lo + hi + 1) / 2;
                    if (nbaseT[mid] - w0 <= (uint32_t)kTNW) lo = mid;
                    else hi = mid - 1;
                }
                cb = lo;
            }
            const uint32_t wn = nbaseT[cb] - w0;
            for (uint32_t i = tid; i < wn; i += kGT) {
                wA[i] = 0;
                wB[i] = 0;
                wC[i] = 0xFFFFFFFFu;
                nfarN[i] = 0;
            }
            __syncthreads();
            for (uint32_t task = wave; task < n_tasks; task += kNW) {
                const uint32_t j = task / kCH, slot = (task % kCH) * 64u + lane;
                const uint32_t ev = eE[j * (uint32_t)kTC + slot];
                const uint32_t c = ev & 0xFFu;
                if (c >= ca && c < cb) {
                    const uint32_t m = (ev >> 8) & 31u;
                    atomicMin(&wC[nbaseT[c] + __popc(presT[c] & ((1u << m) - 1u)) - w0], j);
                }
            }
            __syncthreads();
            for (uint32_t c = ca + tid; c < cb; c += kGT) {
                const uint32_t base = nbaseT[c], k = nn[c];
                uint32_t pp = presT[c];
                for (uint32_t x = 0; x < k; x++) {
                    const uint32_t mj = wC[base - w0 + x];
                    uint32_t r = 0;
                    for (uint32_t y = 0; y < k; y++) r += (wC[base - w0 + y] < mj) ? 1u : 0u;
                    liOf[base + x] = (uint8_t)r;
                    maskN[base - w0 + r] = (uint8_t)(__ffs(pp) - 1);
                    ncolN[base - w0 + r] = (uint8_t)c;
                    pp &= pp - 1u;
                }
            }
            __syncthreads();
            GP(4)
            auto node_of = [&](uint32_t ev) -> uint32_t { return node_of_entry(ev); };
            unsigned long long farbits = 0;
            {
                uint32_t it = 0;
                for (uint32_t task = wave; task < n_tasks; task += kNW, it++) {
                    const uint32_t j = task / kCH, slot = (task % kCH) * 64u + lane;
                    const uint32_t ev = eE[j * (uint32_t)kTC + slot];
                    const uint32_t c = ev & 0xFFu;
                    const bool mine = c >= ca && c < cb;
                    const uint32_t ln = mine ? node_of(ev) : 0u;
                    uint32_t lnp = __shfl_up(ln, 1);
                    const bool left_mine = __shfl_up(mine ? 1 : 0, 1) != 0;
                    if (!mine) continue;
                    const uint32_t node = N + ln;
                    const bool first = (ev & kEFirst) != 0;
                    atomicAdd(&wA[ln - w0], first ? 1u : 0x10001u);
                    if (mb[j].cur + slot + 1 == mb[j].curn) mb[j].carryn = node;
                    if (!first) {
                        if (slot && (lane == 0 || !left_mine)) lnp = node_of(eE[j * (uint32_t)kTC + slot - 1]);
                        const uint32_t pn = slot ? N + lnp : mb[j].carry;
                        const uint32_t d = node - pn;
                        if (d <= 64u) atomicOr(&wB[ln - w0], 1ull << (d - 1u));
                        else farbits |= 1ull << it;
                    }
                }
            }
            for (uint32_t i = tid; i < wn; i += kGT) wC[i] = 0xFFFFFFFFu;
            __syncthreads();
            GP(6)
            const uint32_t te_w = block_exscan_f(wn, [&](uint32_t i) { return wA[i] >> 16; }, wD, s_tmp);
            while (__syncthreads_or(farbits != 0 ? 1 : 0)) {
                uint32_t it = 0;
                for (uint32_t task = wave; task < n_tasks; task += kNW, it++) {
                    if (!((farbits >> it) & 1ull)) continue;
                    const uint32_t j = task / kCH, slot = (task % kCH) * 64u + lane;
                    const uint32_t ln = node_of(eE[j * (uint32_t)kTC + slot]);
                    const uint32_t pn = slot ? N + node_of(eE[j * (uint32_t)kTC + slot - 1]) : mb[j].carry;
                    atomicMin(&wC[ln - w0], pn);
                }
                __syncthreads();
                it = 0;
                for (uint32_t task = wave; task < n_tasks; task += kNW, it++) {
                    if (!((farbits >> it) & 1ull)) continue;
                    const uint32_t j = task / kCH, slot = (task % kCH) * 64u + lane;
                    const uint32_t ln = node_of(eE[j * (uint32_t)kTC + slot]);
                    const uint32_t pn = slot ? N + node_of(eE[j * (uint32_t)kTC + slot - 1]) : mb[j].carry;
                    if (wC[ln - w0] == pn) farbits &= ~(1ull << it);
                }
                __syncthreads();
                for (uint32_t i = tid; i < wn; i += kGT) {
                    const uint32_t v = wC[i];
                    if (v == 0xFFFFFFFFu) continue;
                    const uint32_t node = N + w0 + i;
                    if (node < a.ncap) {
                        pred[E + te + wD[i] + nfarN[i]] = v;
                        if (a.want_smin) atomicMin(&smin[v], cposT[ncolN[i]]);
                        atomicMax(&last[v], node);
                    }
                    nfarN[i]++;
                    wC[i] = 0xFFFFFFFFu;
                }
            }
            for (uint32_t i = tid; i < wn; i += kGT) {
                const uint32_t node = N + w0 + i;
                if (node >= a.ncap) continue;
                const uint32_t seg = E + te + wD[i];
                const uint32_t pos = cposT[ncolN[i]];
                uint32_t np = nfarN[i];
                unsigned long long bits = wB[i];
                while (bits) {
                    const uint32_t hi = 63u - (uint32_t)__clzll((long long)bits);
                    bits ^= 1ull << hi;
                    const uint32_t pa = node - (hi + 1u);
                    pred[seg + np] = pa;
                    np++;
                    if (a.want_smin) atomicMin(&smin[pa], pos);
                    atomicMax(&last[pa], node);
                }
                uint4 r;
                r.x = seg;
                r.y = __float_as_uint(wt[wA[i] & 0xFFFFu]);
                r.z = (np & 0xFFu) | ((uint32_t)maskN[i] << 8);
                r.w = kRowNone;
                rec[node] = r;
                node_pos[node] = pos;
            }
            te += te_w;
            ca = cb;
            __syncthreads();
        }
        for (uint32_t j = tid; j < F; j += kGT) {
            mb[j].cur = mb[j].curn;
            mb[j].carry = mb[j].carryn;
        }
        N += tn;
        E += te;
        __syncthreads();
        GP(7)
    }
    if (N > a.ncap || N > 65535u) {
        if (tid == 0) {
            sz[0] = N;
            sz[1] = sz[2] = 0;
            sz[3] = 2;
        }
        return;
    }
    GP(8)
    const uint32_t seg_len = dp_slot_segment(N);
    const uint32_t n_seg = (N + seg_len - 1) / seg_len;
    uint32_t *codeL = reinterpret_cast<uint32_t *>(smem);
    const bool in_lds = (size_t)N * 4 <= a.tile_bytes;
    if (tid == 0) s_tmp[kGT / 64 + 1] = 0xFFFFFFFFu;
    __syncthreads();
    for (uint32_t i = tid; i < N; i += kGT) {
        uint32_t z = rec[i].z;
        const uint32_t l = last[i];
        if (l == 0) {
            z |= kRecSink;
            atomicMin(&s_tmp[kGT / 64 + 1], i);
            if (a.want_smin) smin[i] = 1000000u;
        }
        if (l > i && l - i > (uint32_t)kFarLds) z |= kRecFence;
        rec[i].z = z;
        if (in_lds) codeL[i] = l | ((z & kRecSink) ? (1u << 30) : 0u) | ((z & kRecFence) ? (1u << 31) : 0u);
    }
    __syncthreads();
    GP(9)
    if (tid < n_seg) {
        auto walk = [&](auto kslots) {
            constexpr int K = decltype(kslots)::value;
            uint32_t fa[K];
#pragma unroll
            for (int x = 0; x < K; x++) fa[x] = (x < a.W) ? 0u : 0xFFFFFFFFu;
            uint32_t nsp = 0;
            const uint32_t b = tid * seg_len, e = min(N, b + seg_len);
            for (uint32_t m = b; m < e; m++) {
                uint32_t l, sink, fence;
                if (in_lds) {
                    const uint32_t cd = codeL[m];
                    l = cd & 0xFFFFu;
                    sink = cd & (1u << 30);
                    fence = cd & (1u << 31);
                } else {
                    const uint32_t z = rec[m].z;
                    l = last[m];
                    sink = z & kRecSink;
                    fence = z & kRecFence;
                }
                uint32_t wv = kRowNone;
                if (!sink && l != m + 1) {
                    const bool may_slot = !fence && l < e;
                    uint32_t slot = K;
#pragma unroll
                    for (int x = K - 1; x >= 0; x--) slot = (may_slot && fa[x] <= m) ? (uint32_t)x : slot;
#pragma unroll
                    for (int x = 0; x < K; x++) fa[x] = (slot == (uint32_t)x) ? l : fa[x];
                    wv = slot < (uint32_t)K ? slot : (kRowSpilled | nsp++);
                }
                if (in_lds) codeL[m] = wv;
                else rec[m].w = wv;
            }
            mb[tid].id = nsp;
        };
        if (a.W <= 4) walk(std::integral_constant<int, 4>());
        else walk(std::integral_constant<int, 8>());
    }
    __syncthreads();
    {
        uint32_t tot = 0;
        for (uint32_t g = 0; g < n_seg; g++) tot += mb[g].id;
        for (uint32_t i = tid; i < N; i += kGT) {
            uint32_t w = in_lds ? codeL[i] : rec[i].w;
            if (w != kRowNone && (w & kRowSpilled)) {
                uint32_t base = 0;
                for (uint32_t g = 0; g < i / seg_len; g++) base += mb[g].id;
                w += base;
            }
            rec[i].w = w;
            if (in_lds) codeL[i] = w;
        }
        if (tid == 0) {
            sz[0] = N;
            sz[1] = E;
            sz[2] = tot;
            sz[3] = (tot > kMaxSpillRows) ? 4u : 0u;
            sz[4] = s_tmp[kGT / 64 + 1];
        }
    }
    __syncthreads();
    GP(10)
    for (uint32_t i = tid; i < N; i += kGT) {
        const uint4 r = rec[i];
        const uint32_t np = r.z & 0xFFu;
        uint32_t first_far = 0;
        uint32_t dist = np ? 0u : kRecDistFar;
        for (uint32_t x = 0; x < np; x++) {
            const uint32_t pa = pred[r.x + x];
            uint32_t pw = in_lds ? codeL[pa] : rec[pa].w;
            if (pw == kRowNone) pw = 0;
            const bool sp = (pw & kRowSpilled) != 0;
            if (sp && first_far == 0) first_far = x + 1;
            dist = max(dist, i - pa);
            pred[r.x + x] = pa | ((pw & 0x7FFFu) << 16) | (sp ? kPredSpilled : 0u);
        }
        rec[i].z = r.z | (first_far << 24) | (min(dist, kRecDistFar) << kRecDistShift);
    }
    GP(11)
    if (a.reach != nullptr) {
        uint2 *rg = a.reach + (size_t)q * a.ncap;
        uint32_t *cw = in_lds ? codeL : (a.want_smin ? last : smin);
        if (tid == 0) s_tmp[kGT / 64 + 2] = 0xFFFFFFFFu;
        __syncthreads();
        for (uint32_t i = tid; i < N; i += kGT) {
            const uint32_t pos = node_pos[i];
            if (i > 0 && node_pos[i - 1] == pos) continue;
            uint32_t mx = 0;
            for (uint32_t j = i; j < N && node_pos[j] == pos; j++) {
                mx = max(mx, prune_gain_units(__uint_as_float(rec[j].y), a.kappa64));
                cw[j] = 0;
            }
            cw[i] = mx;
            atomicMin(&s_tmp[kGT / 64 + 2], mx);
        }
        __syncthreads();
        if (tid == 0) sz[5] = s_tmp[kGT / 64 + 2];
        const uint32_t total = block_exscan(cw, cw, N, s_tmp);
        for (uint32_t i = tid; i < N; i += kGT) {
            const uint32_t pos = node_pos[i];
            if (i > 0 && node_pos[i - 1] == pos) continue;
            const uint32_t right = (i + 1 < N) ? total - cw[i + 1] : 0u;
            const uint32_t cols_right = NC - 1u - rank(pos);
            for (uint32_t j = i; j < N && node_pos[j] == pos; j++) rg[j] = uint2{right, ((a.want_smin && !in_lds) ? 0u : last[j]) | (cols_right << 16)};
        }
    }
    GP(12)
    GP_FLUSH
}

size_t graph_bitmap_off(uint32_t max_family) { return ((size_t)kOE + 2 * (size_t)max_family * kTC + 15) & ~(size_t)15; }
size_t graph_lds_bytes(uint32_t width, uint32_t max_family) {
    const size_t nwords = (width + 31) / 32;
    return graph_bitmap_off(max_family) + ((6 * nwords + 15) & ~(size_t)15);
}
size_t graph_member_cap(uint32_t max_family) { return std::max<size_t>(16, (max_family + 1) & ~(size_t)1); }
size_t graph_lds_total(uint32_t width, uint32_t max_family) {
    return graph_lds_bytes(width, max_family) + sizeof(Member) * graph_member_cap(max_family);
}

}
}

using namespace sina_hip;

namespace {

int build_family_graphs(sina_hip_ctx *c, const uint32_t *fam_ids, const uint64_t *fam_off, uint32_t q0,
                        uint32_t bq, float fs_weight, int W, BuiltGraphs *bg, bool want_smin, float kappa64) {
    hipStream_t s = c->stream;
    if (ensure_ref_off_host(c)) return 1;
    if (!(c->wtab_fs_weight == fs_weight) || !c->g_wtab.p) {
        std::vector<float> wt((size_t)(kMaxFam + 1) * (kMaxFam + 1), 0.f);
        const float weight = fs_weight;
        for (unsigned F = 1; F <= (unsigned)kMaxFam; F++)
            for (unsigned cnt = 0; cnt <= F; cnt++)
                wt[(size_t)F * (kMaxFam + 1) + cnt] =
                    (float)(1.0 / (double)(weight + 1) + (double)(weight * ((float)cnt / (float)F)));
        if (c->g_wtab.reserve(wt.size() * 4)) return 1;
        SH_CHECK(hipMemcpyAsync(c->g_wtab.p, wt.data(), wt.size() * 4, hipMemcpyHostToDevice, s));
        SH_CHECK(hipStreamSynchronize(s));
        c->wtab_fs_weight = fs_weight;
    }
    std::vector<uint64_t> foff(bq + 1), elems(bq, 0);
    uint32_t max_f = 1;
    bg->pred_off.assign(bq, 0);
    for (uint32_t q = 0; q <= bq; q++) foff[q] = fam_off[q0 + q] - fam_off[q0];
    for (uint32_t q = 0; q < bq; q++) {
        max_f = std::max<uint32_t>(max_f, (uint32_t)(foff[q + 1] - foff[q]));
        for (uint64_t x = fam_off[q0 + q]; x < fam_off[q0 + q + 1]; x++) {
            const uint32_t id = fam_ids[x];
            if (id >= c->st->n_refs) SH_FAIL("align_families: reference id out of range");
            elems[q] += c->st->ref_off_host[id + 1] - c->st->ref_off_host[id];
        }
    }
    uint32_t ncap = std::min<uint32_t>(65535, 12288);
    for (int attempt = 0;; attempt++) {
        uint64_t pred_total = 0;
        for (uint32_t q = 0; q < bq; q++) {
            bg->pred_off[q] = pred_total;
            pred_total += elems[q] + 8;
        }
        const size_t glds_tables = graph_lds_bytes(c->st->width, max_f);
        const size_t glds = graph_lds_total(c->st->width, max_f);
        if (glds > 160 * 1024) SH_FAIL_LIMIT("align_families: family too wide for the device DAG build");
        if (c->g_fam_ids.reserve(4 * std::max<uint64_t>(foff[bq], 1)) || c->g_fam_off.reserve(8 * ((uint64_t)bq + 1)) ||
            c->g_tmp1.reserve(8 * (uint64_t)bq) ||
            c->rec.reserve(sizeof(uint4) * (uint64_t)bq * ncap) || c->node_pos.reserve(4 * (uint64_t)bq * ncap) ||
            c->succ_minpos.reserve(4 * (uint64_t)bq * ncap) || c->g_tmp3.reserve(4 * (uint64_t)bq * ncap) ||
            c->pred.reserve(4 * pred_total) || c->g_sizes.reserve(4 * kSz * (uint64_t)bq) ||
            (kappa64 > 0.f && c->rgain.reserve(8 * (uint64_t)bq * ncap)))
            return 1;
        if (upload(c, 1, c->g_fam_ids.p, fam_ids + fam_off[q0], 4 * foff[bq], s) ||
            upload(c, 2, c->g_fam_off.p, foff.data(), 8 * ((uint64_t)bq + 1), s) ||
            upload(c, 3, c->g_tmp1.p, bg->pred_off.data(), 8 * (uint64_t)bq, s))
            return 1;
        GraphArgs ga;
        ga.ref_ab = c->st->ref_ab.as<uint32_t>();
        ga.ref_off = c->st->ref_off.as<uint64_t>();
        ga.fam_ids = c->g_fam_ids.as<uint32_t>();
        ga.fam_off = c->g_fam_off.as<uint64_t>();
        ga.pred_off = c->g_tmp1.as<uint64_t>();
        ga.wtab = c->g_wtab.as<float>();
        ga.rec = c->rec.as<uint4>();
        ga.node_pos = c->node_pos.as<uint32_t>();
        ga.succ_min = c->succ_minpos.as<uint32_t>();
        ga.far_mark = c->g_tmp3.as<uint32_t>();
        ga.pred = c->pred.as<uint32_t>();
        ga.sizes = c->g_sizes.as<uint32_t>();
        ga.width = c->st->width;
        ga.ncap = ncap;
        ga.bitmap_off = (uint32_t)graph_bitmap_off(max_f);
        ga.tile_bytes = ga.bitmap_off;
        ga.member_off = (uint32_t)glds_tables;
        ga.member_cap = (uint32_t)graph_member_cap(max_f);
        ga.fam_cap = max_f;
        ga.W = W;
        ga.want_smin = want_smin ? 1 : 0;
        ga.reach = kappa64 > 0.f ? c->rgain.as<uint2>() : nullptr;
        ga.kappa64 = kappa64;
        if (allow_full_lds(reinterpret_cast<const void *>(family_graph_kernel))) return 1;
        bg->sizes.resize(kSz * (size_t)bq);
        {
            heavy_launch hl(c, s, kHeavyGraph);
            SH_CHECK(hipEventRecord(c->ev[6], hl.stream()));
            hipLaunchKernelGGL(family_graph_kernel, dim3(bq), dim3(kGT), glds, hl.stream(), ga);
            SH_CHECK(hipGetLastError());
            SH_CHECK(hipEventRecord(c->ev[7], hl.stream()));
            if (hl.done()) return 1;
        }
        if (download(c, 4, c->g_sizes.p, 4 * kSz * (uint64_t)bq, s)) return 1;
        SH_CHECK(wait_stream(c, s));
        memcpy(bg->sizes.data(), c->h_stage[4].p, 4 * kSz * (uint64_t)bq);
        float gms = 0;
        SH_CHECK(hipEventElapsedTime(&gms, c->ev[6], c->ev[7]));
        {
            uint64_t bytes = 0;
            for (uint32_t q = 0; q < bq; q++)
                bytes += 4 * elems[q] + (uint64_t)bg->sizes[kSz * q] * (16 + 4 + (kappa64 > 0.f ? 8 : 0)) + 4 * (uint64_t)bg->sizes[kSz * q + 1];
            std::lock_guard<std::mutex> slk(c->st->stats_mu);
            c->st->stats.graph_ms += gms;
            c->st->stats.graph_bytes += bytes;
            c->st->stats.graph_launches++;
        }
        uint32_t need_n = 0;
        for (uint32_t q = 0; q < bq; q++) {
            if (bg->sizes[kSz * q + 3] == 2) need_n = std::max(need_n, bg->sizes[kSz * q]);
            if (bg->sizes[kSz * q + 3] == 4) SH_FAIL_LIMIT("align_families: too many spill rows for one query");
        }
        if (!need_n) break;
        if (attempt >= 3 || need_n > 65535u) SH_FAIL_LIMIT("align_families: family DAG exceeds device limits");
        ncap = std::min<uint32_t>(65535, need_n + need_n / 8 + 16);
    }
    bg->ncap = ncap;
    return 0;
}

int build_graphs_for_launch(sina_hip_ctx *c, const uint32_t *fam_ids, const uint64_t *fam_off, uint32_t q0, uint32_t n,
                            const sina_hip_align_params *p, int W, const PrunePlan &pp, BuiltGraphs *bg) {
    return build_family_graphs(c, fam_ids, fam_off, q0, n, p->fs_weight, W, bg, p->insertion == SINA_INSERTION_FORBID,
                               pp.on ? pp.kappa64 : 0.f);
}

}

namespace sina_hip {

int align_family_batches(sina_hip_ctx *c, const char *who, family_builder build, bool profile_batch, const uint32_t *fam_ids,
                         const uint64_t *fam_off, uint32_t nq, const uint8_t *qmask, const uint64_t *qoff,
                         const sina_hip_align_params *p, sina_hip_align_out *out, uint32_t *out_pos) {
    const std::string w(who);
    if (!c || !fam_ids || !fam_off || !qmask || !qoff || !p || !out)
        SH_FAIL(w + ": null argument");
    std::lock_guard<std::mutex> lk(c->mu);
    sina_hip_hint_guard hints(c);
    if (!c->st->have_refs) SH_FAIL(w + ": upload references first");
    if (nq == 0) return 0;
    SH_CHECK(hipSetDevice(c->device));
    hipStream_t s = c->stream;
    if (c->st->width > 524288u) SH_FAIL_LIMIT(w + ": alignment wider than 524288 columns (use align_graphs)");
    if (profile_batch && p->weights != nullptr && p->n_weights > 0)
        SH_FAIL(w + ": a profile batch takes no positional weights (scoring_scheme_profile)");
    uint32_t maxL = 0;
    for (uint32_t q = 0; q < nq; q++) {
        const uint64_t L = qoff[q + 1] - qoff[q], F = fam_off[q + 1] - fam_off[q];
        if (L == 0 || L > 65535) SH_FAIL(w + ": query length must be in 1..65535");
        if (F == 0 || F > (uint64_t)kMaxFam) SH_FAIL(w + ": family size must be in 1..128");
        maxL = std::max<uint32_t>(maxL, (uint32_t)L);
    }
    DpPlan pl;
    if (plan_dp(c, maxL, &pl)) return 1;
    const int Lp = pl.geom.Lp();
    if (upload_weights(c, p)) return 1;
    if (c->h_out_pos.reserve(4 * std::max<uint64_t>(qoff[nq] - qoff[0], 1))) return 1;

    const uint64_t tb_budget_cells = tb_plane_budget(c) / tb_cell_bytes(p->insertion == SINA_INSERTION_FORBID);
    const uint32_t slots = dp_wave_slots(c, pl.geom.B);
    const uint32_t chunk_q = 3 * slots;
    BuiltGraphs bg;
    std::vector<uint32_t> dag_of;
    std::vector<uint32_t> ufam_ids;
    std::vector<uint64_t> ufam_off;
    for (uint32_t q0 = 0; q0 < nq; q0 += chunk_q) {
        const uint32_t bq = std::min(chunk_q, nq - q0);
        dag_of.assign(bq, 0);
        uint32_t n_dags = bq;
        const uint32_t *b_ids = fam_ids;
        const uint64_t *b_off = fam_off;
        uint32_t b_q0 = q0;
        if (bq > 1) {
            auto fam_hash = [&](uint32_t q) {
                uint64_t h = 0xcbf29ce484222325ull ^ (fam_off[q + 1] - fam_off[q]);
                for (uint64_t x = fam_off[q]; x < fam_off[q + 1]; x++) {
                    h = (h ^ fam_ids[x]) * 0x100000001b3ull;
                    h ^= h >> 31;
                }
                return h;
            };
            size_t cap = 16;
            while (cap < 2 * (size_t)bq) cap <<= 1;
            std::vector<uint32_t> slot(cap, 0xFFFFFFFFu), first;
            std::vector<uint64_t> hq(bq);
            for (uint32_t q = 0; q < bq; q++) {
                hq[q] = fam_hash(q0 + q);
                size_t at = (size_t)(hq[q] >> 17) & (cap - 1);
                for (;;) {
                    const uint32_t u = slot[at];
                    if (u == 0xFFFFFFFFu) {
                        slot[at] = (uint32_t)first.size();
                        dag_of[q] = (uint32_t)first.size();
                        first.push_back(q);
                        break;
                    }
                    const uint32_t f = first[u];
                    const uint64_t la = fam_off[q0 + q + 1] - fam_off[q0 + q], lb = fam_off[q0 + f + 1] - fam_off[q0 + f];
                    if (hq[f] == hq[q] && la == lb && memcmp(fam_ids + fam_off[q0 + q], fam_ids + fam_off[q0 + f], 4 * la) == 0) {
                        dag_of[q] = u;
                        break;
                    }
                    at = (at + 1) & (cap - 1);
                }
            }
            n_dags = (uint32_t)first.size();
            if (n_dags < bq) {
                ufam_off.assign((size_t)n_dags + 1, 0);
                for (uint32_t u = 0; u < n_dags; u++)
                    ufam_off[u + 1] = ufam_off[u] + (fam_off[q0 + first[u] + 1] - fam_off[q0 + first[u]]);
                ufam_ids.resize(ufam_off[n_dags]);
                for (uint32_t u = 0; u < n_dags; u++)
                    memcpy(ufam_ids.data() + ufam_off[u], fam_ids + fam_off[q0 + first[u]], 4 * (ufam_off[u + 1] - ufam_off[u]));
                b_ids = ufam_ids.data();
                b_off = ufam_off.data();
                b_q0 = 0;
            } else {
                for (uint32_t q = 0; q < bq; q++) dag_of[q] = q;
            }
        } else {
            for (uint32_t q = 0; q < bq; q++) dag_of[q] = q;
        }
        PrunePlan pp;
        if (!profile_batch)
            pp = prune_plan(p, (float)(1.0 / (double)(p->fs_weight + 1) + (double)p->fs_weight), p->fs_weight >= 0.f ? 0.f : -1.f, maxL, false);
        if (build(c, b_ids, b_off, b_q0, n_dags, p, pl.W, pp, &bg)) return 1;
        {
            std::lock_guard<std::mutex> slk(c->st->stats_mu);
            c->st->stats.dags_built += n_dags;
            c->st->stats.dags_used += bq;
        }
        uint32_t r0 = 0;
        while (r0 < bq) {
            uint32_t r1 = r0;
            uint64_t tbc = 0, sprows = 0, cells = 0;
            uint32_t erec_cursor = 0;
            std::vector<QDesc> qd;
            std::vector<uint32_t> chain_ref;
            while (r1 < bq) {
                const uint32_t u = dag_of[r1];
                const uint32_t N = bg.sizes[kSz * u];
                if (r1 > r0 && tbc + (uint64_t)N * Lp > tb_budget_cells) break;
                QDesc d;
                d.node_off = (uint64_t)u * bg.ncap;
                d.edge_off = bg.pred_off[u];
                d.q_off = qoff[q0 + r1] - qoff[q0 + r0];
                d.tb_off = tbc;
                d.spill_off = sprows;
                d.N = N;
                d.L = (uint32_t)(qoff[q0 + r1 + 1] - qoff[q0 + r1]);
                d.n_spill = bg.sizes[kSz * u + 2];
                d.first_sink = bg.sizes[kSz * u + 4];
                d.gmin = bg.sizes[kSz * u + 5];
                d.erec_off = erec_cursor;
                erec_cursor += dp_edge_entries(N);
                qd.push_back(d);
                chain_ref.push_back(fam_ids[fam_off[q0 + r1]]);
                tbc += (uint64_t)N * Lp;
                sprows += d.n_spill;
                cells += (uint64_t)N * d.L;
                r1++;
            }
            {
                const uint32_t r1r = dp_round_range(r0, r1, bq, slots);
                for (uint32_t r = r1r; r < r1; r++) {
                    tbc -= (uint64_t)qd[r - r0].N * Lp;
                    sprows -= qd[r - r0].n_spill;
                    cells -= (uint64_t)qd[r - r0].N * qd[r - r0].L;
                }
                qd.resize(r1r - r0);
                chain_ref.resize(r1r - r0);
                r1 = r1r;
            }
            const uint32_t rq = r1 - r0;
            const uint64_t qbase = qoff[q0 + r0], nqm = qoff[q0 + r1] - qbase;
            if (c->qd.reserve(sizeof(QDesc) * rq) || c->qmask.reserve(std::max<uint64_t>(nqm, 1))) return 1;
            if (upload(c, 5, c->qd.p, qd.data(), sizeof(QDesc) * rq, s) || upload(c, 6, c->qmask.p, qmask + qbase, nqm, s))
                return 1;
            c->profile_batch = profile_batch;
            c->out_pos_base = qbase - qoff[0];
            if (run_dp_device(c, pl, qd.data(), rq, (uint64_t)n_dags * bg.ncap, tbc, sprows, cells, nqm, p, c->st->width,
                              out + q0 + r0, out_pos ? out_pos + qbase : nullptr, false, pp, profile_batch ? nullptr : chain_ref.data()))
                return 1;
            r0 = r1;
        }
    }
    return 0;
}

}

extern "C" {

int sina_hip_align_families(sina_hip_ctx *c, const uint32_t *fam_ids, const uint64_t *fam_off, uint32_t nq,
                            const uint8_t *qmask, const uint64_t *qoff, const sina_hip_align_params *p,
                            sina_hip_align_out *out, uint32_t *out_pos) {
    return align_family_batches(c, "align_families", build_graphs_for_launch, false, fam_ids, fam_off, nq, qmask, qoff, p, out, out_pos);
}

#ifdef SINA_DP_PROFILE
int sina_hip_debug_graph_profile(unsigned long long *out16, int reset) {
    SH_CHECK(hipMemcpyFromSymbol(out16, HIP_SYMBOL(g_graph_prof), sizeof(unsigned long long) * 16));
    if (reset) {
        unsigned long long z[16] = {};
        SH_CHECK(hipMemcpyToSymbol(HIP_SYMBOL(g_graph_prof), z, sizeof z));
    }
    return 0;
}
#endif

int sina_hip_debug_family_graph(sina_hip_ctx *c, const uint32_t *fam_ids, uint32_t F, float fs_weight,
                                uint32_t ring_depth, uint32_t *n_nodes, uint32_t *n_edges, uint32_t *pos,
                                uint8_t *mask, float *weight, uint32_t *pred_off, uint32_t *pred,
                                uint32_t *succ_minpos, uint8_t *sink, uint32_t *spill_idx, uint32_t cap_nodes,
                                uint32_t cap_edges) {
    if (!c || !fam_ids || !n_nodes || !n_edges) SH_FAIL("debug_family_graph: null argument");
    std::lock_guard<std::mutex> lk(c->mu);
    if (!c->st->have_refs) SH_FAIL("debug_family_graph: upload references first");
    if (F == 0 || F > (uint32_t)kMaxFam) SH_FAIL("debug_family_graph: family size must be in 1..128");
    SH_CHECK(hipSetDevice(c->device));
    const uint64_t foff[2] = {0, F};
    BuiltGraphs bg;
    if (build_family_graphs(c, fam_ids, foff, 0, 1, fs_weight, (int)ring_depth, &bg, true, fs_weight >= 0.f ? 64.0f * 1.0001f * 2.0f : 0.f)) return 1;
    const uint32_t N = bg.sizes[0];
    std::vector<uint4> rec(N);
    std::vector<uint32_t> pr(bg.sizes[1] + 8);
    SH_CHECK(hipMemcpy(rec.data(), c->rec.p, sizeof(uint4) * N, hipMemcpyDeviceToHost));
    SH_CHECK(hipMemcpy(pr.data(), c->pred.p, 4 * pr.size(), hipMemcpyDeviceToHost));
    uint32_t E = 0;
    for (uint32_t m = 0; m < N; m++) E += rec[m].z & 0xffu;
    *n_nodes = N;
    *n_edges = E;
    if (N > cap_nodes || E > cap_edges) SH_FAIL("debug_family_graph: output buffers too small");
    SH_CHECK(hipMemcpy(pos, c->node_pos.p, 4 * N, hipMemcpyDeviceToHost));
    SH_CHECK(hipMemcpy(succ_minpos, c->succ_minpos.p, 4 * N, hipMemcpyDeviceToHost));
    uint32_t e = 0;
    for (uint32_t m = 0; m < N; m++) {
        mask[m] = (uint8_t)((rec[m].z >> 8) & 0xffu);
        memcpy(&weight[m], &rec[m].y, 4);
        sink[m] = (rec[m].z & kRecSink) ? 1 : 0;
        spill_idx[m] = rec[m].w;
        pred_off[m] = e;
        for (uint32_t x = 0; x < (rec[m].z & 0xffu); x++) pred[e++] = pr[rec[m].x + x] & 0xffffu;
    }
    pred_off[N] = e;
    return 0;
}

}
```

sina_amd/csrc/mesh_dp.hip:

```cpp
#include <cstdio>
#include <cstdlib>
#include <type_traits>

#include "common.h"

namespace sina_hip {

namespace {

struct ChainState {
    float v;
    uint32_t e;
    uint32_t gsi;
    uint32_t gmax;
};

template <bool GSI>
__device__ __forceinline__ bool same_state(const ChainState &a, const ChainState &b) {
    if constexpr (GSI) return a.v == b.v && a.e == b.e && (!a.e || (a.gsi == b.gsi && a.gmax == b.gmax));
    else return a.v == b.v && a.e == b.e;
}

__device__ __forceinline__ uint32_t lane_shr1(uint32_t x) {
    return (uint32_t)__builtin_amdgcn_update_dpp(0, (int)x, 0x138 , 0xf, 0xf, false);
// ... 587 lines not shown
            const int b_ = it_ <= 4 ? it_ : (it_ <= 8 ? 5 : (it_ <= 16 ? 6 : (it_ <= 32 ? 7 : 8)));
            pa_[16 + b_] += 1;
        }
#endif
        SH_PROF(5)

        sload_wait(npe);
        if (have_left_strip) sload_wait(nedge);
        if (lane == 63 && have_right_strip) {
            EdgeRec er;
            er.bnd = fv[B - 1];
            er.xv = ex.v;
            er.xe = (ex.e << 31) | (kGsi ? ex.gsi : 0u);
            er.gmax = FORBID ? ex.gmax : 0u;
            e_out[m] = er;
        }
        if (r.keep != kRowNone && !SH_ABL(32)) {
            if (!(r.keep & kRowSpilled)) {
                unsigned char *myslot = ring + (size_t)r.keep * kSlotBytes;
                store_slot<B>(reinterpret_cast<float *>(myslot), lane, fv);
                store_slot<B>(reinterpret_cast<float *>(myslot + kValBytes), lane, gm);
                if (lane == 0 && have_left_strip) *reinterpret_cast<float *>(myslot + 2 * kValBytes) = edge_val;
            } else if (!SH_ABL(2)) {
                float *row = spill + (size_t)(r.keep & ~kRowSpilled) * (2 * Lp);
                store_cells<B>(row + s0, fv);
                store_cells<B>(row + Lp + s0, gm);
            }
        }
        SH_PROF(6)

        if (!SH_ABL(4)) {
            uint32_t tc[B];
#pragma unroll
            for (int k = 0; k < B; k++)
                tc[k] = kLazy ? (fvm[k] | (oplast[k] ? 0u : kTb16XLast)) : (fvm[k] | fvs[k] | (oplast[k] ? kTagOpLast : 0u));
            if constexpr (kLazy) {
                uint32_t tp[B / 2];
#pragma unroll
                for (int k = 0; k < B / 2; k++) tp[k] = tc[2 * k] | (tc[2 * k + 1] << 16);
                store_cells<B / 2>(reinterpret_cast<uint32_t *>(tb + (size_t)m * Lp + s0), tp);
            } else {
                store_cells<B>(tb + (size_t)m * Lp + s0, tc);
            }
        }
        if constexpr (DBG) {
            if (qi == 0) store_cells<B>(dbg_value + (size_t)m * Lp + s0, fv);
        }

        if (strip == strip_last && !SH_ABL(64)) {
            float v = 0.f;
            auto pick4 = [&](auto g4_tag) {
                constexpr int g4 = decltype(g4_tag)::value;
                if constexpr (4 * g4 < B) {
                    if (g4 == kg_last) {
                        uint32_t t = __float_as_uint(fv[4 * g4]);
                        t = (kr_is1 & __float_as_uint(fv[4 * g4 + 1])) | (~kr_is1 & t);
                        t = (kr_is2 & __float_as_uint(fv[4 * g4 + 2])) | (~kr_is2 & t);
                        t = (kr_is3 & __float_as_uint(fv[4 * g4 + 3])) | (~kr_is3 & t);
                        asm volatile("" : "+v"(t));
                        v = __uint_as_float(t);
                    }
                }
            };
            pick4(std::integral_constant<int, 0>{});
            pick4(std::integral_constant<int, 1>{});
            pick4(std::integral_constant<int, 2>{});
            static_assert(B <= 12, "pick4 covers three groups of four");
            if (own_last && (!lc_any || v < lc_min)) {
                lc_min = v;
                lc_arg = m;
                lc_any = true;
            }
            if (own_last && is_sink && !sk_any) lc_snk0 = v;
        }
        if (is_sink && !SH_ABL(64)) {
            float bv = __builtin_inff();
            uint32_t bs = 0xffffffffu;
#pragma unroll
            for (int k = 0; k < B; k++) {
                const uint32_t s = s0 + k;
                const bool b = (s < L) && (fv[k] < bv);
                bv = b ? fv[k] : bv;
                bs = b ? s : bs;
            }
#pragma unroll
            for (int off = 32; off > 0; off >>= 1) {
                const float ov = __shfl_xor(bv, off);
                const uint32_t os = __shfl_xor(bs, off);
                const bool b = (ov < bv) || (ov == bv && os < bs);
                bv = b ? ov : bv;
                bs = b ? os : bs;
            }
            if (!sk_any) snk0 = m;
            if (bv < sk_min) {
                sk_min = bv;
                sk_m = m;
                sk_s = bs;
            }
            sk_any = true;
        }
        SH_PROF(7)
        SH_PROF_CNT(8, 1)
        cur = nrec;
        cur_edge = nedge;
        cur_pe = npe;
#pragma unroll
        for (int i = 0; i < B / 4; i++) {
            prev_v.v[i] = typename Cells<B>::V{fv[4 * i], fv[4 * i + 1], fv[4 * i + 2], fv[4 * i + 3]};
            prev_g.v[i] = typename Cells<B>::V{gm[4 * i], gm[4 * i + 1], gm[4 * i + 2], gm[4 * i + 3]};
        }
        prev_edge_val = edge_val;
    }
    if (sk_any && (!all_any || sk_min < all_min || (sk_min == all_min && sk_m < all_m))) {
        all_min = sk_min;
        all_m = sk_m;
        all_s = sk_s;
    }
    all_any = all_any || sk_any;
    if (have_right_strip) {
        asm volatile("s_waitcnt vmcnt(0)" ::: "memory");
        __builtin_amdgcn_s_dcache_inv();
    }
    }
    SH_PROF_FLUSH

    const float v1min = __shfl(lc_min, lane_last);
    const float v_snk0 = __shfl(lc_snk0, lane_last);
    const uint32_t v1arg = __shfl(lc_arg, lane_last);
    if (lane == 0) {
        DpResult r;
        r.status = 0;
        uint32_t em = snk0, es = L - 1;
        float ev = v_snk0;
        if (v1min < v_snk0) {
            em = v1arg;
            ev = v1min;
        }
        if (all_any && all_min < ev) {
            em = all_m;
            es = all_s;
            ev = all_min;
        }
        if (!all_any) r.status = -2;
        r.end_m = em;
        r.end_s = es;
        r.raw = ev;
        r.rows_done = r.cells_done = r.attempts = r.pad_ = 0u;
        r.gain0 = 0.f;
        r.ubound = __builtin_inff();
        resv[qi] = r;
    }
}

template <int B, bool DBG, bool PRUNE>
__global__ void __launch_bounds__(64, (B <= 4 ? 4 : (B <= 8 ? SINA_DP_SIMPLE_WAVES8 : 2)))
mesh_dp_simple_kernel(const QDesc *__restrict__ qdv, const uint32_t *__restrict__ orderv, const uint4 *__restrict__ recv,
                      const uint32_t *__restrict__ predv, const uint8_t *__restrict__ qmaskv, void *__restrict__ tbv,
                      float *__restrict__ dbg_value, float *spillv, EdgeRec *edgev, uint64_t edge_stride,
                      uint32_t n_strips, DpResult *__restrict__ resv, float ms, float mms, float gp, float gpe, DryArgs dry,
                      const uint2 *__restrict__ reachv, float prune_rho, uint32_t prune_amax, uint32_t n_slots,
                      const float *__restrict__ scout_uv, float scout_bias) {
    static_assert(B % 4 == 0, "16-byte accesses per array");
    constexpr int kStrip = 64 * B;
    extern __shared__ __attribute__((aligned(16))) unsigned char smem[];
    const int lane = threadIdx.x;
    dry_signal(dry, gridDim.x, lane == 0);
    const uint32_t qi = orderv[blockIdx.x];
    const QDesc d = qdv[qi];
    const uint32_t N = uniform(d.N), L = uniform(d.L);
    const uint32_t Lp = n_strips * (uint32_t)kStrip;
    const uint32_t S = min(n_strips, (L - 1) / (uint32_t)kStrip + 1);
    const uint64_t node_off = uniform(d.node_off);
    const uint64_t erec_off = uniform(d.erec_off);
    unsigned char *ring = smem;
    constexpr size_t kValBytes = (size_t)kStrip * 4;
    constexpr size_t kSlotBytes = 2 * kValBytes + 16;
    const uint4 *__restrict__ rec = recv + node_off;
    const uint32_t *__restrict__ pred = predv + uniform(d.edge_off);
    uint16_t *__restrict__ tb = reinterpret_cast<uint16_t *>(tbv) + uniform(d.tb_off);
    float *spill = spillv + uniform(d.spill_off) * (size_t)(2 * Lp);
    const uint64_t q_off = uniform(d.q_off);

    const uint32_t strip_last = (L - 1) / (uint32_t)kStrip;
    const int lane_last = (int)(((L - 1) / B) & 63u);
    const int k_last = (int)((L - 1) % B);

    constexpr int32_t kNoBound = 1 << 29;
    constexpr float kDead = 1000000.0f;
    const uint2 *__restrict__ reach = PRUNE ? reachv + node_off : nullptr;
    const uint32_t gmin = uniform(d.gmin);

    const uint32_t first_sink = uniform(d.first_sink);
    int32_t U64 = kNoBound, U_scout = kNoBound;
    float gain0 = 0.f;
    auto col_bound = [&](uint2 rc, int32_t r) -> int32_t {
        const int32_t excess = (int32_t)(rc.y >> 16) - r;
        return U64 + (int32_t)rc.x - (excess > 0 ? (int32_t)gmin * excess : 0);
    };
    if constexpr (PRUNE) {
        const uint2 r0 = reach[0];
        const int32_t excess0 = (int32_t)(r0.y >> 16) + 1 - (int32_t)(L - 1);
        const uint32_t g_cols = uniform(r0.x) + prune_amax - (excess0 > 0 ? gmin * (uint32_t)excess0 : 0u), g_len = prune_amax * (L - 1);
        const uint32_t g0 = g_cols < g_len ? g_cols : g_len;
        gain0 = (float)g0 * kPruneUnit;
        U64 = -(int32_t)uniform((uint32_t)(int32_t)(prune_rho * (float)g0));
        if (scout_uv != nullptr) {
            const float su = __uint_as_float(uniform(__float_as_uint(scout_uv[qi]))) + scout_bias;
            if (su > -100000.0f && su < 100000.0f) {
                const float up = su * 64.0f;
                int32_t u = (int32_t)up;
                if ((float)u < up) u++;
                U_scout = u;
                const int32_t guard = -(int32_t)uniform((uint32_t)(int32_t)(fmaxf(prune_rho - 0.06f, 0.f) * (float)g0));
                U64 = u < guard ? u : guard;
            }
        }
    }
    uint32_t rows_done = 0, cells_done = 0, attempt = 0;
    const float gmin_f = (float)gmin * kPruneUnit;
    SH_PROF_DECL
    uint32_t res_m = 0, res_s = 0;
    float res_v = 0.f;
    int32_t res_status = 0;
    for (;;) {
    ++attempt;
    const float U_f = (float)U64 * kPruneUnit;
    float lc_min = PRUNE ? __builtin_inff() : 0.f, lc_snk0 = PRUNE ? kDead : 0.f;
    uint32_t lc_arg = 0;
    bool lc_any = false;
    float all_min = __builtin_inff();
    uint32_t all_m = 0, all_s = 0xffffffffu, snk0 = PRUNE ? first_sink : 0u;
    bool all_any = PRUNE;
    uint32_t m_free_dead = 0;
    constexpr uint32_t kNone = 0xFFFFFFFFu;
    uint32_t out_first = kNone, out_last = 0;
    if constexpr (PRUNE) {
        if (U64 + (int32_t)(prune_amax * (L - 1)) >= 64) {
            uint32_t lo = 0, hi = N;
            while (lo < hi) {
                const uint32_t mid = (lo + hi) >> 1;
                if (col_bound(reach[mid], (int32_t)(L - 1)) < 64) hi = mid;
                else lo = mid + 1;
            }
            m_free_dead = lo;
        }
    }

#ifdef SH_PROF_TIMERS
    if (attempt == 1 && lane == 0 && blockIdx.x < 16384) g_dp_span[2 * blockIdx.x] = wall_clock64();
#endif
    constexpr uint32_t kXL = kTb16XLast, kExtXL = kTb16Ext | kTb16XLast;
    const float gpv = opaque_v(gp), gpev = opaque_v(gpe);

    for (uint32_t strip = 0; strip < S; ++strip) {
    const uint32_t s0 = (strip * 64u + (uint32_t)lane) * B;
    const bool lane0 = lane == 0;
    const bool col0_mine = (strip == 0) && lane0;
    const uint64_t e_in = uniform((uint64_t)(edgev + (size_t)(strip ? strip - 1 : 0) * edge_stride + erec_off));
    EdgeRec *e_out = edgev + (size_t)strip * edge_stride + erec_off;
    const bool have_left_strip = uniform((uint32_t)(strip > 0)) != 0, have_right_strip = strip + 1 < S;

    uint32_t qcls[B];
#pragma unroll
    for (int k = 0; k < B; k++) {
        const uint32_t s = s0 + k;
        const uint32_t q = (s < L) ? (uint32_t)(qmaskv[q_off + s] & 0xf) : 0u;
        qcls[k] = ((q & 1u) << 6) | ((q & 2u) << 7) | ((q & 4u) << 7) | (q & 8u);
    }
    const bool own_last = (strip == strip_last) && (lane == lane_last);
    float sk_min = __builtin_inff();
    uint32_t sk_m = 0, sk_s = 0xffffffffu;
    bool sk_any = false;

    const uint64_t pred_addr = uniform((uint64_t)pred);
    uint32_t m_begin = 0, edge_end = 0, stop_at = 0;
    if constexpr (PRUNE) {
        const bool free_starts = U64 + (int32_t)prune_amax * ((int32_t)(L - 1) - (int32_t)(strip * (uint32_t)kStrip)) >= 64;
        if (strip == 0) {
            edge_end = m_free_dead;
        } else {
            edge_end = out_first != kNone ? out_last + 1u : 0u;
            if (!free_starts) m_begin = out_first != kNone ? out_first : N;
        }
        stop_at = (free_starts && m_free_dead > edge_end) ? m_free_dead : edge_end;
        out_first = kNone;
        out_last = 0;
    }
    const uint32_t jump_lo = m_begin;
    uint4 cur = rec[m_begin < N ? m_begin : 0u];
    u32x4 cur_pe = sload16(pred_addr + (uint64_t)cur.x * 4);
    u32x4 cur_edge = {0, 0, 0, 0};
    if (have_left_strip) cur_edge = sload16(e_in + (uint64_t)(m_begin < N ? m_begin : 0u) * sizeof(EdgeRec));
    uint2 reach_cur = {0u, 0u};
    if constexpr (PRUNE) reach_cur = reach[m_begin < N ? m_begin : 0u];
    sload_wait(cur_pe);
    sload_wait(cur_edge);
    Cells<B> prev_v, prev_g;
    float prev_edge_val = 0.f;
#pragma unroll
    for (int i = 0; i < B / 4; i++) prev_v.v[i] = prev_g.v[i] = typename Cells<B>::V{0.f, 0.f, 0.f, 0.f};

    float A_lane = 0.f, r_lane = 0.f;
    uint32_t dead_run = (PRUNE && m_begin > 0) ? 64u : 0u;
    uint32_t slot_dead = 0, rows_strip = 0;
    bool prev_dead = PRUNE && m_begin > 0;
    bool pe_valid = true;
    if constexpr (PRUNE) {
        A_lane = (float)(U64 + (int32_t)prune_amax * ((int32_t)(L - 1) - (int32_t)s0)) * kPruneUnit;
        r_lane = (float)((int32_t)(L - 1) - (int32_t)s0);
        if (m_begin > 0) {
            float dead_cells[B];
#pragma unroll
            for (int k = 0; k < B; k++) dead_cells[k] = kDead;
            for (uint32_t x = 0; x < n_slots; x++) {
                unsigned char *slot = ring + (size_t)x * kSlotBytes;
                store_slot<B>(reinterpret_cast<float *>(slot), lane, dead_cells);
                store_slot<B>(reinterpret_cast<float *>(slot + kValBytes), lane, dead_cells);
                if (lane0) *reinterpret_cast<float *>(slot + 2 * kValBytes) = kDead;
            }
            slot_dead = (1u << n_slots) - 1u;
        }
    }

    for (uint32_t m = m_begin; m < N; ++m) {
        if constexpr (PRUNE) {
            if (m >= stop_at) break;
        }
        if ((m & 127u) == 0) issue_priority_by_progress(strip * N + m, S * N);
        const uint32_t m_next = m + 1 < N ? m + 1 : m;
        const uint4 nrec = rec[m_next];
        uint2 nreach = {0u, 0u};
        if constexpr (PRUNE) nreach = reach[m_next];
        u32x4 nedge = {0, 0, 0, 0};
        if (have_left_strip) nedge = sload16(e_in + (uint64_t)m_next * sizeof(EdgeRec));

        SH_PROF(0)
        if constexpr (PRUNE) {
            if (have_left_strip && m >= edge_end) {
                cur_edge.x = cur_edge.y = __float_as_uint(kDead);
                cur_edge.z = cur_edge.w = 0u;
            }
        }
        const uint32_t r_pb = cur.x, r_z = cur.z, r_keep = cur.w;
        const uint32_t npred = r_z & 0xffu, mmask = (r_z >> 8) & 0xfu;
        const float wgt = __uint_as_float(cur.y);
        const float vM = ms * wgt, vX = mms * wgt;
        const float edge_val = __uint_as_float(cur_edge.x);
        const bool is_sink = (r_z & kRecSink) != 0;

        bool edge_dead = false;
        uint2 cur_reach = {0u, 0u};
        float Bm_row = 0.f, nc_row = 0.f;
        if constexpr (PRUNE) {
            edge_dead = m >= edge_end || (have_left_strip && cur_edge.w == 0u);
            const uint32_t dist = (r_z >> kRecDistShift) & 63u;
            const bool skip = edge_dead && dist != kRecDistFar && dist <= dead_run;
            if (skip) {
                if (lane == 63 && have_right_strip) {
                    EdgeRec er;
                    er.bnd = kDead;
// ... 702 lines not shown
        } else if (a.overhang == SINA_OVERHANG_EDGE) {
            int k = (int)s;
            while (k--) emit(width - (uint32_t)k - 1);
        }
    }
    o.sum_weight = sum_weight;
    o.aligned_bases = aligned;
    o.n_out = n;
    if (mem.writes) a.out[q] = o;
}

template <bool LAZY>
__global__ void __launch_bounds__(64) backtrack_kernel(BtArgs a) {
    __shared__ typename BtWindow<LAZY>::Lds lds;
    const uint32_t q = blockIdx.x;
    if (q >= a.nq) return;
    const QDesc d = a.qd[q];
    BtWindow<LAZY> mem(a, d, lds, threadIdx.x);
    walk_query<LAZY>(a, q, d, mem);
}

template <bool LAZY>
__global__ void __launch_bounds__(64) backtrack_lanes_kernel(BtArgs a) {
    const uint32_t q = blockIdx.x * 64u + threadIdx.x;
    if (q >= a.nq) return;
    const QDesc d = a.qd[q];
    BtDirect<LAZY> mem(a, d);
    walk_query<LAZY>(a, q, d, mem);
}


constexpr int kAsmMax = 4096;
__global__ void __launch_bounds__(64) assemble_kernel(BtArgs a) {
    extern __shared__ __attribute__((aligned(16))) unsigned char asm_lds[];
    unsigned long long *dupm = reinterpret_cast<unsigned long long *>(asm_lds);
    unsigned long long *movedm = dupm + kAsmMax / 64;
    uint32_t *colm = reinterpret_cast<uint32_t *>(movedm + kAsmMax / 64);
    __shared__ uint32_t facts[4];
    const uint32_t q = blockIdx.x, lane = threadIdx.x;
    if (q >= a.nq) return;
    const QDesc d = a.qd[q];
    const sina_hip_align_out o = a.out[q];
    const uint32_t n = o.n_out, width = a.width;
    if (o.status != 0 || n == 0 || n > a.asm_cap) return;
    uint32_t *pos = a.out_pos + d.q_off;
    const uint8_t *qm = a.qmask + d.q_off;
    const bool keep_over = a.overhang != SINA_OVERHANG_REMOVE;
    const uint32_t tail = keep_over ? (uint32_t)o.cutoff_tail : 0u;
    const uint32_t n_aligned = (uint32_t)o.aligned_bases;
    uint32_t carry = 0;
    bool beyond = false;
    for (uint32_t base = 0; base < n; base += 64) {
        const uint32_t i = base + lane;
        uint32_t v = i < n ? pos[i] : 0u;
#pragma unroll
        for (int off = 1; off < 64; off <<= 1) {
            const uint32_t y = __shfl_up(v, off);
            if ((int)lane >= off) v = max(v, y);
        }
        v = max(v, carry);
        uint32_t prev = __shfl_up(v, 1);
        if (lane == 0) prev = carry;
        const bool dup = i < n && i > 0 && v == prev;
        const unsigned long long dm = __builtin_amdgcn_ballot_w64(dup);
        if (lane == 0) {
            dupm[base >> 6] = dm;
            movedm[base >> 6] = 0ull;
        }
        if (i < n) {
            colm[i] = v;
            beyond = beyond || v >= width;
        }
        carry = __shfl(v, 63);
    }
    const bool any_beyond = __builtin_amdgcn_ballot_w64(beyond) != 0ull;
    __syncthreads();
    if (lane == 0) {
        uint32_t total = 0, longest = 0, last_run = 0, ok = any_beyond ? 0u : 1u;
        bool first = true;
        uint32_t i = 1;
        while (ok && i < n) {
            const unsigned long long word = dupm[i >> 6] >> (i & 63);
            if (word == 0ull) {
                i = ((i >> 6) + 1) << 6;
                continue;
            }
            i += (uint32_t)__ffsll((long long)word) - 1u;
            const uint32_t i0 = i - 1;
            uint32_t r = 0;
            while (i < n && ((dupm[i >> 6] >> (i & 63)) & 1ull)) {
                r++;
                i++;
            }
            const uint32_t anchor_col = width - 1 - colm[i0];
            const uint32_t next_col = i0 > 0 ? width - 1 - colm[i0 - 1] : width;
            if (next_col - (anchor_col + 1) < r) {
                ok = 0;
                break;
            }
            for (uint32_t t = 0; t < r; t++) {
                colm[i0 + t] = width - next_col + t;
                movedm[(i0 + t) >> 6] |= 1ull << ((i0 + t) & 63);
            }
            total += r;
            longest = max(longest, r);
            if (first) last_run = r;
            first = false;
        }
        facts[0] = ok;
        facts[1] = total;
        facts[2] = longest;
        facts[3] = last_run;
    }
    __syncthreads();
    if (!facts[0]) return;
    const uint32_t keep_case = a.lowercase == SINA_LOWERCASE_ORIGINAL ? 0xFFu : 0xEFu;
    const uint32_t lower = a.lowercase == SINA_LOWERCASE_UNALIGNED ? 0x10u : 0u;
    const uint32_t first_q = (uint32_t)o.end_s + tail;
    for (uint32_t base = 0; base < n; base += 64) {
        const uint32_t i = base + lane;
        if (i >= n) break;
        const bool overhang_base = i < tail || i >= tail + n_aligned;
        const bool moved = (movedm[i >> 6] >> (i & 63)) & 1ull;
        const uint32_t bits = ((uint32_t)qm[first_q - i] & keep_case) | ((overhang_base || moved) ? lower : 0u);
        pos[n - 1 - i] = ((width - 1 - colm[i]) & 0xFFFFFFu) | (bits << 24);
    }
    if (lane == 0) {
        sina_hip_align_out *out = a.out + q;
        out->assembled = 1;
        out->nast_total = facts[1];
        out->nast_longest = facts[2];
        out->nast_last_run = facts[3];
    }
}

template <int B>
int launch_tb(bool weighted, bool forbid, const DpArgs &a, uint32_t nq, uint32_t n_strips, size_t lds, hipStream_t s) {
#define SH_LAUNCH(WG, FB, BL)                                                                              \
    do {                                                                                                \
        auto kfn = a.dbg_value ? mesh_dp_kernel<B, WG, FB, BL, true> : mesh_dp_kernel<B, WG, FB, BL, false>;     \
        if (allow_full_lds(reinterpret_cast<const void *>(kfn))) return 1;                               \
        hipLaunchKernelGGL(kfn, dim3(nq), dim3(64), lds, s, a.qd, a.order, a.rec, a.pred, a.node_pos, a.succ_minpos, \
                           a.qmask, a.weights, a.n_weights, a.tb, a.dbg_value, a.spill, a.edge, a.edge_stride, \
                           n_strips, a.res, a.ms, a.mms, a.gp, a.gpe, a.prof16, a.dry);                  \
    } while (0)
    const bool generic_only = atoi(test_knob("generic").c_str()) != 0;
    if (!weighted && !forbid && a.below_init && a.gp >= a.gpe && !generic_only && a.prof16 == nullptr) {
        const bool prune = a.prune && a.reach != nullptr && n_strips >= 2;
        auto kfn = prune ? (a.dbg_value ? mesh_dp_simple_kernel<B, true, true> : mesh_dp_simple_kernel<B, false, true>)
                         : (a.dbg_value ? mesh_dp_simple_kernel<B, true, false> : mesh_dp_simple_kernel<B, false, false>);
        if (allow_full_lds(reinterpret_cast<const void *>(kfn))) return 1;
        hipLaunchKernelGGL(kfn, dim3(nq), dim3(64), lds, s, a.qd, a.order, a.rec, a.pred, a.qmask, a.tb, a.dbg_value, a.spill,
                           a.edge, a.edge_stride, n_strips, a.res, a.ms, a.mms, a.gp, a.gpe, a.dry, a.reach, a.prune_rho,
                           a.prune_amax, (uint32_t)(lds / dp_slot_bytes(DpGeom{64 * (int)n_strips, B})), prune ? a.scout_u : nullptr, a.scout_bias);
    } else if (!weighted && !forbid && a.below_init) SH_LAUNCH(false, false, true);
    else if (!weighted && !forbid) SH_LAUNCH(false, false, false);
    else if (weighted && !forbid) SH_LAUNCH(true, false, false);
    else if (!weighted && forbid) SH_LAUNCH(false, true, false);
    else SH_LAUNCH(true, true, false);
#undef SH_LAUNCH
    SH_CHECK(hipGetLastError());
    return 0;
}

}

int allow_full_lds(const void *kernel) {
    static std::mutex mu;
    static std::vector<std::pair<int, const void *>> done;
    int dev = 0;
    SH_CHECK(hipGetDevice(&dev));
    std::lock_guard<std::mutex> lk(mu);
    for (const auto &k : done)
        if (k.first == dev && k.second == kernel) return 0;
    hipFuncAttributes fa;
    SH_CHECK(hipFuncGetAttributes(&fa, kernel));
    const int room = 160 * 1024 - (int)fa.sharedSizeBytes;
    SH_CHECK(hipFuncSetAttribute(kernel, hipFuncAttributeMaxDynamicSharedMemorySize, room));
    done.emplace_back(dev, kernel);
    return 0;
}

static const int kLaneCells[] = {4, 8, 12};
static const double kLaneRate[] = {226.0, 461.0, 403.0};
constexpr int kMaxStrips = 40;

bool pick_geom(uint32_t maxL, DpGeom *g) {
    const std::string ov = test_knob("geom");
    if (!ov.empty()) {
        int t = 0, b = 0;
        if (sscanf(ov.c_str(), "%d,%d", &t, &b) == 2 && (uint32_t)(t * b) >= maxL && t % 64 == 0 && t >= 64 &&
            t <= 64 * kMaxStrips && (b == 4 || b == 8 || b == 12)) {
            g->T = t;
            g->B = b;
            return true;
        }
    }
    for (int i = 0; i < 3; i++)
        if (maxL <= 64u * (uint32_t)kLaneCells[i]) {
            g->T = 64;
            g->B = kLaneCells[i];
            return true;
        }
    double best = 0;
    bool found = false;
    for (int i = 1; i < 3; i++) {
        const int b = kLaneCells[i];
        const uint32_t strips = (maxL + 64u * b - 1) / (64u * b);
        if (strips > (uint32_t)kMaxStrips) continue;
        const double cost = (double)(strips * 64u * b) / kLaneRate[i];
        if (!found || cost < best) {
            best = cost;
            g->T = (int)strips * 64;
            g->B = b;
            found = true;
        }
    }
    return found;
}

size_t dp_slot_bytes(const DpGeom &g) { return (size_t)64 * g.B * 8 + 16; }
size_t dp_fixed_lds_bytes(const DpGeom &) { return 0; }
int dp_max_ring(const DpGeom &) { return 8; }
size_t dp_default_lds_budget(const DpGeom &g) { return (size_t)160 * 1024 / (4 * dp_waves_per_simd(g.B)) - 64; }

int launch_mesh_dp(const DpGeom &g, bool weighted, bool forbid, const DpArgs &a, uint32_t nq,
                   size_t lds, hipStream_t s) {
    const uint32_t n_strips = (uint32_t)g.T / 64;
    if (g.B == 4) return launch_tb<4>(weighted, forbid, a, nq, n_strips, lds, s);
    if (g.B == 8) return launch_tb<8>(weighted, forbid, a, nq, n_strips, lds, s);
    if (g.B == 12) return launch_tb<12>(weighted, forbid, a, nq, n_strips, lds, s);
    SH_FAIL("mesh_dp: unsupported geometry");
}

#ifdef SINA_DP_PROFILE
extern "C" int sina_hip_debug_dp_ablate(int mask) {
    SH_CHECK(hipMemcpyToSymbol(HIP_SYMBOL(g_dp_abl), &mask, sizeof mask));
    return 0;
}
extern "C" int sina_hip_debug_dp_spans(unsigned long long *out, unsigned n_queries) {
#if SINA_DP_PROFILE == 1
    SH_CHECK(hipMemcpyFromSymbol(out, HIP_SYMBOL(g_dp_span), sizeof(unsigned long long) * 2 * (n_queries < 16384u ? n_queries : 16384u)));
    return 0;
#else
    (void)out; (void)n_queries;
    return 1;
#endif
}
extern "C" int sina_hip_debug_dp_profile(unsigned long long *out32, int reset) {
    SH_CHECK(hipMemcpyFromSymbol(out32, HIP_SYMBOL(g_dp_prof), sizeof(unsigned long long) * 32));
    if (reset) {
        unsigned long long z[32] = {};
        SH_CHECK(hipMemcpyToSymbol(HIP_SYMBOL(g_dp_prof), z, sizeof z));
    }
    return 0;
}
#endif

int launch_assemble(const BtArgs &a0, hipStream_t s) {
    BtArgs a = a0;
    a.asm_cap = std::min<uint32_t>((a.asm_cap + 63u) & ~63u, (uint32_t)kAsmMax);
    const size_t lds = 2 * (size_t)(kAsmMax / 64) * 8 + 4 * (size_t)a.asm_cap;
    hipLaunchKernelGGL(assemble_kernel, dim3(a.nq), dim3(64), lds, s, a);
    SH_CHECK(hipGetLastError());
    return 0;
}

constexpr uint32_t kBtLanesMin = 8192, kBtLanesMaxLen = 2048;
bool backtrack_by_lanes(const BtArgs &a) {
    bool lanes = a.nq >= kBtLanesMin && a.asm_cap <= kBtLanesMaxLen;
    if (const std::string e = test_knob("bt_lanes"); !e.empty()) lanes = atoi(e.c_str()) != 0;
    return lanes;
}
int launch_backtrack(const BtArgs &a, hipStream_t s) {
    if (backtrack_by_lanes(a)) {
        if (a.lazy_sidx) hipLaunchKernelGGL(backtrack_lanes_kernel<true>, dim3((a.nq + 63u) / 64u), dim3(64), 0, s, a);
        else hipLaunchKernelGGL(backtrack_lanes_kernel<false>, dim3((a.nq + 63u) / 64u), dim3(64), 0, s, a);
    } else if (a.lazy_sidx) hipLaunchKernelGGL(backtrack_kernel<true>, dim3(a.nq), dim3(64), 0, s, a);
    else hipLaunchKernelGGL(backtrack_kernel<false>, dim3(a.nq), dim3(64), 0, s, a);
    SH_CHECK(hipGetLastError());
    return 0;
}

}
```

sina_amd/csrc/scout.hip:

```cpp
#include <algorithm>

#include "common.h"
#include "ctx.h"

namespace sina_hip {
namespace {

constexpr float kScoutDead = 1000000.0f;

template <int K>
__global__ void __launch_bounds__(64) chain_scout_kernel(const QDesc *__restrict__ qdv, const uint32_t *__restrict__ orderv,
                                                         const uint4 *__restrict__ recv, const uint32_t *__restrict__ node_posv,
                                                         const uint8_t *__restrict__ qmaskv, const uint32_t *__restrict__ ref_ab,
                                                         const uint64_t *__restrict__ ref_off, const uint32_t *__restrict__ chain_ref,
                                                         uint32_t nq, float ms, float mms, float gp, float gpe,
                                                         float *__restrict__ out_u) {
    static_assert(K % 4 == 0 && K >= 8 && K <= 32, "band width");
    const uint32_t slot = blockIdx.x * 64u + threadIdx.x;
    if (slot >= nq) return;
    const uint32_t qi = orderv[slot];
    const QDesc d = qdv[qi];
    const uint32_t N = d.N, L = d.L;
    const uint4 *__restrict__ rec = recv + d.node_off;
    const uint32_t *__restrict__ node_pos = node_posv + d.node_off;
    const uint32_t member = chain_ref[qi];
    const uint64_t b0 = ref_off[member], b1 = ref_off[member + 1];
    const int c_max = L > (uint32_t)K ? (int)(L - (uint32_t)K) : 0;
    const float credit = (float)d.gmin * kPruneUnit;

    float best = __builtin_inff();
    float pv[K], pg[K];
#pragma unroll
    for (int k = 0; k < K; k++) pv[k] = pg[k] = kScoutDead;
    int c = 0;
    int a_rel = K / 2;
    bool have_prev = false;
    uint32_t m = 0;
    uint32_t w[K / 4 + 1];
#pragma unroll
    for (int i = 0; i <= K / 4; i++) w[i] = 0u;
    uint64_t w_at = ~(uint64_t)0 - 16;
    uint32_t ab_next = b0 < b1 ? ref_ab[b0] : 0u;
    uint32_t wpos[3] = {0xFFFFFFFFu, 0xFFFFFFFFu, 0xFFFFFFFFu};
    uint4 wrec[3] = {};
    auto load_window = [&](uint32_t at) {
#pragma unroll
        for (int i = 0; i < 3; i++) {
            const uint32_t x = at + (uint32_t)i;
            wpos[i] = x < N ? node_pos[x] : 0xFFFFFFFFu;
            wrec[i] = rec[x < N ? x : 0];
        }
    };
    load_window(0);
    for (uint64_t bi = b0; bi < b1; ++bi) {
        const uint32_t ab = ab_next;
        if (bi + 1 < b1) ab_next = ref_ab[bi + 1];
        const uint32_t col = ab & 0xFFFFFFu, bmask = (ab >> 24) & 31u;
        uint32_t row = N;
        uint4 r = wrec[0];
        bool found = false;
#pragma unroll
        for (int i = 0; i < 3; i++)
            if (!found && wpos[i] == col && ((wrec[i].z >> 8) & 31u) == bmask) {
                found = true;
                row = m + (uint32_t)i;
                r = wrec[i];
            }
        if (!found) {
            while (m < N && node_pos[m] < col) ++m;
            row = m;
            r = rec[row < N ? row : 0];
            while (row < N && ((r.z >> 8) & 31u) != bmask) {
                ++row;
                if (row < N) r = rec[row];
            }
            if (row >= N || node_pos[row] != col) break;
        }
        m = row + 1;
        load_window(m);
        const uint32_t mmask = (r.z >> 8) & 0xfu;
        const float wgt = __uint_as_float(r.y);
        const float vM = ms * wgt, vX = mms * wgt;
        int delta = 0;
        if (have_prev) {
            delta = a_rel + 1 - K / 2;
            delta = delta < 0 ? 0 : (delta > 2 ? 2 : delta);
        }
        int cn = c + delta;
        cn = cn > c_max ? c_max : cn;
        delta = cn - c;
        c = cn;
        float csel[K];
        {
            const uint64_t at = d.q_off + (uint64_t)c;
            const uint64_t at4 = at & ~(uint64_t)3;
            if (at4 != w_at) {
                const uint32_t *qw = reinterpret_cast<const uint32_t *>(qmaskv + at4);
                if (at4 == w_at + 4) {
#pragma unroll
                    for (int i = 0; i < K / 4; i++) w[i] = w[i + 1];
                    w[K / 4] = qw[K / 4];
                } else {
#pragma unroll
                    for (int i = 0; i <= K / 4; i++) w[i] = qw[i];
                }
                w_at = at4;
            }
            const uint32_t sh = ((uint32_t)at & 3u) * 8u;
#pragma unroll
            for (int i = 0; i < K / 4; i++) {
                const uint32_t x = sh ? ((w[i] >> sh) | (w[i + 1] << (32u - sh))) : w[i];
#pragma unroll
                for (int j = 0; j < 4; j++) {
                    const int k = 4 * i + j;
                    const uint32_t s = (uint32_t)c + (uint32_t)k;
                    const uint32_t q = s < L ? ((x >> (8 * j)) & 0xfu) : 0u;
                    csel[k] = (q & mmask) != 0u ? vM : vX;
                }
            }
        }
        const bool col0 = c == 0;
        float loc[K], gm[K];
        if (!have_prev) {
            const bool source = (r.z & 0xffu) == 0u;
#pragma unroll
            for (int k = 0; k < K; k++) loc[k] = gm[k] = (source || (k == 0 && col0)) ? 1.0f : kScoutDead;
        } else {
            float sv[K + 1], sg[K];
#pragma unroll
            for (int k = 0; k <= K; k++) {
                const float d0 = k >= 1 ? pv[k - 1] : kScoutDead;
                const float d1 = k < K ? pv[k] : kScoutDead;
                const float d2 = k + 1 < K ? pv[k + 1] : kScoutDead;
                sv[k] = delta == 0 ? d0 : (delta == 1 ? d1 : d2);
            }
#pragma unroll
            for (int k = 0; k < K; k++) {
                const float d0 = pg[k];
                const float d1 = k + 1 < K ? pg[k + 1] : kScoutDead;
                const float d2 = k + 2 < K ? pg[k + 2] : kScoutDead;
                sg[k] = delta == 0 ? d0 : (delta == 1 ? d1 : d2);
            }
#pragma unroll
            for (int k = 0; k < K; k++) {
                const float v = sv[k + 1] + gp;
                const float g = sg[k] + gpe;
                const float cand = v < g ? v : g;
                gm[k] = cand;
                float mv = sv[k] + csel[k];
                float dv = cand;
                if (k == 0 && col0) {
                    mv = __builtin_inff();
                    dv = cand < 1.0f ? cand : 1.0f;
                }
                loc[k] = mv < dv ? mv : dv;
            }
        }
        float fv[K];
        fv[0] = loc[0];
        bool e_prev = col0 && fv[0] == 1.0f;
#pragma unroll
        for (int k = 1; k < K; k++) {
            const float gsx = fv[k - 1] + (e_prev ? gpe : gp);
            const bool ins = gsx <= loc[k];
            fv[k] = ins ? gsx : loc[k];
            e_prev = ins;
        }
        float vmin = __builtin_inff(), vcred = __builtin_inff();
#pragma unroll
        for (int k = 0; k < K; k++) {
            const bool real = (uint32_t)c + (uint32_t)k < L;
            fv[k] = real ? fv[k] : kScoutDead;
            gm[k] = real ? gm[k] : kScoutDead;
            vmin = fv[k] < vmin ? fv[k] : vmin;
            const float cr = fv[k] + credit * (float)k;
            if (cr < vcred) {
                vcred = cr;
                a_rel = k;
            }
            if ((uint32_t)c + (uint32_t)k == L - 1u) best = fv[k] < best ? fv[k] : best;
            pv[k] = fv[k];
            pg[k] = gm[k];
        }
        if (r.z & kRecSink) best = vmin < best ? vmin : best;
        have_prev = true;
    }
    out_u[qi] = best;
}

}

int launch_chain_scout(const DpArgs &a, uint32_t nq, const uint32_t *ref_ab, const uint64_t *ref_off,
                       const uint32_t *chain_ref, float *out_u, hipStream_t s) {
    const uint32_t blocks = (nq + 63u) / 64u;
    hipLaunchKernelGGL((chain_scout_kernel<kScoutBand>), dim3(blocks), dim3(64), 0, s, a.qd, a.order, a.rec, a.node_pos,
                       a.qmask, ref_ab, ref_off, chain_ref, nq, a.ms, a.mms, a.gp, a.gpe, out_u);
    SH_CHECK(hipGetLastError());
    return 0;
}

}
```

Baseline: 272,600.

## Fold chain scout into mesh DP kernel using graph-built chain rows and wave DPP

Removes the separate chain_scout kernel launch, which walked the reference's alignment per thread. That launch also needed a host-side event wait and timing step. The graph builder now records the chain row indices for the first family member. The DP kernel computes the scout upper bound inline with a 64-lane wave-wide banded DP that uses DPP shifts and prefix-min reductions. This removes a device-to-host synchronisation and a kernel launch per batch. In exchange it adds work and register pressure inside the DP kernel, and the band is now a fixed 64-wide window instead of an adaptive 8-wide one.

Result: faster. 293,800, median of 6 (+7.8%).

```diff
diff --git a/include/sina_hip.h b/include/sina_hip.h
--- a/include/sina_hip.h
+++ b/include/sina_hip.h
@@ -148,6 +148,7 @@
 } sina_hip_dp_info;
 int sina_hip_debug_dp_info(sina_hip_ctx *ctx, uint32_t q, sina_hip_dp_info *out);
 int sina_hip_debug_rgain(sina_hip_ctx *ctx, uint32_t n, uint32_t *out, uint32_t *cols_right );
+int sina_hip_debug_chain_rows(sina_hip_ctx *ctx, uint16_t *out, uint32_t cap, uint32_t *len);
 
 int sina_hip_debug_family_graph(sina_hip_ctx *ctx, const uint32_t *fam_ids, uint32_t F, float fs_weight,
                                 uint32_t ring_depth, uint32_t *n_nodes, uint32_t *n_edges, uint32_t *pos,
diff --git a/sina_amd/capi.py b/sina_amd/capi.py
--- a/sina_amd/capi.py
+++ b/sina_amd/capi.py
@@ -19,7 +19,7 @@
     "sina_hip_store_alloc_like", "sina_hip_kmer_topk", "sina_hip_kmer_scores", "sina_hip_compare",
     "sina_hip_align_params_default", "sina_hip_staged_out_pos", "sina_hip_align_graphs", "sina_hip_align_families",
     "sina_hip_align_profiles", "sina_hip_debug_family_profile",
-    "sina_hip_debug_mesh", "sina_hip_debug_family_graph", "sina_hip_debug_dp_info", "sina_hip_debug_rgain", "sina_hip_get_stats",
+    "sina_hip_debug_mesh", "sina_hip_debug_family_graph", "sina_hip_debug_dp_info", "sina_hip_debug_rgain", "sina_hip_debug_chain_rows", "sina_hip_get_stats",
     "sina_hip_align_graphs_any", "sina_hip_debug_mesh_wide", "sina_hip_wide_queries", "sina_hip_last_error_is_limit",
 ]
 
@@ -417,6 +417,13 @@
         self._check(self.L.sina_hip_debug_rgain(self.h, n, _ptr(out, u32p), _ptr(cols, u32p)))
         return out[:n], cols[:n]
 
+    def chain_rows(self):
+        cap = 65536
+        out = np.zeros(cap, np.uint16)
+        n = C.c_uint32()
+        self._check(self.L.sina_hip_debug_chain_rows(self.h, out.ctypes.data_as(C.POINTER(C.c_uint16)), cap, C.byref(n)))
+        return out[:min(n.value, cap)].copy()
+
     def stats(self):
         s = Stats()
         self._check(self.L.sina_hip_get_stats(self.h, C.byref(s)))
diff --git a/sina_amd/csrc/api.hip b/sina_amd/csrc/api.hip
--- a/sina_amd/csrc/api.hip
+++ b/sina_amd/csrc/api.hip
@@ -195,7 +195,7 @@
 int run_dp_device(sina_hip_ctx *c, const DpPlan &pl, const QDesc *qd_host, uint32_t bq, uint64_t n_node_entries,
                   uint64_t tb_cells, uint64_t spill_rows, uint64_t cells, uint64_t nqm, const sina_hip_align_params *p, uint32_t width,
                   sina_hip_align_out *out, uint32_t *out_pos, bool want_dbg_value, const PrunePlan &pp,
-                  const uint32_t *chain_ref) {
+                  uint32_t chain_ncap) {
     hipStream_t s = c->stream;
     const int Lp = pl.geom.Lp();
     const bool weighted = p->weights != nullptr && p->n_weights > 0;
@@ -225,7 +225,6 @@
     a.node_pos = c->node_pos.as<uint32_t>();
     a.succ_minpos = c->succ_minpos.as<uint32_t>();
     a.qmask = c->qmask.as<uint8_t>();
-    a.tb = nullptr;
     a.dbg_value = want_dbg_value ? c->dbg.as<float>() : nullptr;
     a.spill = c->spill.as<float>();
     a.edge = c->edge.as<EdgeRec>();
@@ -261,6 +260,9 @@
         a.below_init = (!weighted && !forbid && dp_below_init(max_n, a.gp, a.gpe)) ? 1 : 0;
     }
     a.scout_u = nullptr;
+    a.chain_rows = nullptr;
+    a.chain_sizes = nullptr;
+    a.chain_ncap = 0;
     a.scout_bias = (float)atof(test_knob("scout_add").c_str());
     c->last_scout = false;
     if (const std::string fixed = test_knob("scout_set"); !fixed.empty() && pp.on && !rho_fixed) {
@@ -269,24 +271,16 @@
         if (upload(c, 7, c->scout_u.p, vals.data(), 4 * (size_t)bq, s)) return 1;
         a.scout_u = c->scout_u.as<float>();
         c->last_scout = true;
-    } else if (chain_ref != nullptr && pp.on && !rho_fixed && a.below_init && a.gp >= a.gpe && pl.geom.T > 64 && test_knob("scout") != "0") {
-        if (c->scout.reserve(4 * (size_t)bq) || c->scout_u.reserve(4 * (size_t)bq)) return 1;
-        if (upload(c, 7, c->scout.p, chain_ref, 4 * (size_t)bq, s)) return 1;
-        SH_CHECK(hipEventRecord(c->ev[3], s));
-        if (launch_chain_scout(a, bq, c->st->ref_ab.as<uint32_t>(), c->st->ref_off.as<uint64_t>(), c->scout.as<uint32_t>(),
-                               c->scout_u.as<float>(), s))
-            return 1;
-        SH_CHECK(hipEventRecord(c->ev[4], s));
-        SH_CHECK(wait_event(c->ev[4]));
-        float sms = 0;
-        SH_CHECK(hipEventElapsedTime(&sms, c->ev[3], c->ev[4]));
-        {
-            std::lock_guard<std::mutex> slk(c->st->stats_mu);
-            c->st->stats.scout_ms += sms;
-            c->st->stats.scout_launches++;
-        }
+    } else if (chain_ncap != 0 && !weighted && !forbid && pp.on && !rho_fixed && a.below_init && a.gp >= a.gpe && pl.geom.T > 64 &&
+               test_knob("scout") != "0" && atoi(test_knob("generic").c_str()) == 0) {
+        if (c->scout_u.reserve(4 * (size_t)bq)) return 1;
         a.scout_u = c->scout_u.as<float>();
+        a.chain_rows = c->scout.as<uint16_t>();
+        a.chain_sizes = c->g_sizes.as<uint32_t>();
+        a.chain_ncap = chain_ncap;
         c->last_scout = true;
+        std::lock_guard<std::mutex> slk(c->st->stats_mu);
+        c->st->stats.scout_launches++;
     }
     if (a.scout_u != nullptr && !rho_fixed) {
         std::lock_guard<std::mutex> slk(c->st->stats_mu);
@@ -915,6 +909,19 @@
     return 0;
 }
 
+int sina_hip_debug_chain_rows(sina_hip_ctx *c, uint16_t *out, uint32_t cap, uint32_t *len) {
+    if (!c || !out || !len) SH_FAIL("debug_chain_rows: null argument");
+    std::lock_guard<std::mutex> lk(c->mu);
+    if (!c->scout.p || !c->g_sizes.p) SH_FAIL("debug_chain_rows: no device-built DAG in this context");
+    SH_CHECK(hipSetDevice(c->device));
+    uint32_t sizes[kBuiltWords];
+    SH_CHECK(hipMemcpy(sizes, c->g_sizes.p, sizeof sizes, hipMemcpyDeviceToHost));
+    *len = sizes[kBuiltChainLen];
+    const size_t n = std::min<size_t>(std::min<uint32_t>(*len, cap), c->scout.cap / 2);
+    if (n) SH_CHECK(hipMemcpy(out, c->scout.p, 2 * n, hipMemcpyDeviceToHost));
+    return 0;
+}
+
 int sina_hip_get_stats(sina_hip_ctx *c, sina_hip_stats *s) {
     if (!c || !s) SH_FAIL("get_stats: null argument");
     std::lock_guard<std::mutex> slk(c->st->stats_mu);
diff --git a/sina_amd/csrc/common.h b/sina_amd/csrc/common.h
--- a/sina_amd/csrc/common.h
+++ b/sina_amd/csrc/common.h
@@ -213,6 +213,9 @@
 inline bool dp_below_init(uint32_t max_n, float gp, float gpe) {
     return gp >= 0.f && gpe >= 0.f && 1.0f + (float)max_n * gp * 1.01f + gp + gpe < 900000.0f;
 }
+
+constexpr int kBuiltWords = 8;
+constexpr int kBuiltChainLen = 6;
 
 struct DpArgs {
     const QDesc *qd;
@@ -239,7 +242,10 @@
     float prune_rho;
     uint32_t prune_amax;
     float scout_bias;
-    const float *scout_u;
+    float *scout_u;
+    const uint16_t *chain_rows;
+    const uint32_t *chain_sizes;
+    uint32_t chain_ncap;
 };
 
 struct BtArgs {
@@ -278,9 +284,6 @@
 size_t dp_default_lds_budget(const DpGeom &g);
 int launch_mesh_dp(const DpGeom &g, bool weighted, bool forbid, const DpArgs &a, uint32_t nq,
                    size_t lds_bytes, hipStream_t s);
-constexpr int kScoutBand = 8;
-int launch_chain_scout(const DpArgs &a, uint32_t nq, const uint32_t *ref_ab, const uint64_t *ref_off,
-                       const uint32_t *chain_ref , float *out_u , hipStream_t s);
 int launch_backtrack(const BtArgs &a, hipStream_t s);
 bool backtrack_by_lanes(const BtArgs &a);
 int launch_assemble(const BtArgs &a, hipStream_t s);
@@ -302,7 +305,7 @@
 int run_dp_device(sina_hip_ctx *c, const DpPlan &pl, const QDesc *qd_host, uint32_t bq, uint64_t n_node_entries,
                   uint64_t tb_cells, uint64_t spill_rows, uint64_t cells, uint64_t nqm, const sina_hip_align_params *p, uint32_t width,
                   sina_hip_align_out *out, uint32_t *out_pos, bool want_dbg_value, const PrunePlan &pp,
-                  const uint32_t *chain_ref = nullptr);
+                  uint32_t chain_ncap = 0);
 PrunePlan prune_plan(const sina_hip_align_params *p, float wmax, float wmin, uint32_t maxL, bool profile_batch);
 
 }
diff --git a/sina_amd/csrc/ctx.h b/sina_amd/csrc/ctx.h
--- a/sina_amd/csrc/ctx.h
+++ b/sina_amd/csrc/ctx.h
@@ -433,7 +433,6 @@
 
 namespace sina_hip {
 constexpr int kFamilyMax = 128;
-constexpr int kBuiltWords = 8;
 struct BuiltGraphs {
     uint32_t ncap = 0;
     std::vector<uint64_t> pred_off;
diff --git a/sina_amd/csrc/graph_build.hip b/sina_amd/csrc/graph_build.hip
--- a/sina_amd/csrc/graph_build.hip
+++ b/sina_amd/csrc/graph_build.hip
@@ -53,6 +53,7 @@
     uint32_t *far_mark;
     uint32_t *pred;
     uint32_t *sizes;
+    uint16_t *chain_rows;
     uint32_t width, ncap;
     uint32_t tile_bytes;
     uint32_t bitmap_off;
@@ -323,6 +324,7 @@
     uint32_t *smin = a.succ_min + (size_t)q * a.ncap;
     uint32_t *last = a.far_mark + (size_t)q * a.ncap;
     uint32_t *pred = a.pred + a.pred_off[q];
+    uint16_t *chain_rows = a.chain_rows + (size_t)q * a.ncap;
     const float *wt = a.wtab + (size_t)F * (kMaxFam + 1);
     uint32_t N = 0, E = 0;
     GP(1)
@@ -409,6 +411,7 @@
                     const bool first = (ev & kEFirst) != 0;
                     atomicAdd(&wA[ln - w0], first ? 1u : 0x10001u);
                     if (mb[j].cur + slot + 1 == mb[j].curn) mb[j].carryn = node;
+                    if (j == 0 && mb[0].cur + slot < a.ncap) chain_rows[mb[0].cur + slot] = (uint16_t)node;
                     if (!first) {
                         if (slot && (lane == 0 || !left_mine)) lnp = node_of(eE[j * (uint32_t)kTC + slot - 1]);
                         const uint32_t pn = slot ? N + lnp : mb[j].carry;
@@ -579,6 +582,7 @@
             sz[2] = tot;
             sz[3] = (tot > kMaxSpillRows) ? 4u : 0u;
             sz[4] = s_tmp[kGT / 64 + 1];
+            sz[kBuiltChainLen] = mb[0].len;
         }
     }
     __syncthreads();
@@ -691,6 +695,7 @@
             c->rec.reserve(sizeof(uint4) * (uint64_t)bq * ncap) || c->node_pos.reserve(4 * (uint64_t)bq * ncap) ||
             c->succ_minpos.reserve(4 * (uint64_t)bq * ncap) || c->g_tmp3.reserve(4 * (uint64_t)bq * ncap) ||
             c->pred.reserve(4 * pred_total) || c->g_sizes.reserve(4 * kSz * (uint64_t)bq) ||
+            c->scout.reserve(2 * (uint64_t)bq * ncap) ||
             (kappa64 > 0.f && c->rgain.reserve(8 * (uint64_t)bq * ncap)))
             return 1;
         if (upload(c, 1, c->g_fam_ids.p, fam_ids + fam_off[q0], 4 * foff[bq], s) ||
@@ -710,6 +715,7 @@
         ga.far_mark = c->g_tmp3.as<uint32_t>();
         ga.pred = c->pred.as<uint32_t>();
         ga.sizes = c->g_sizes.as<uint32_t>();
+        ga.chain_rows = c->scout.as<uint16_t>();
         ga.width = c->st->width;
         ga.ncap = ncap;
         ga.bitmap_off = (uint32_t)graph_bitmap_off(max_f);
@@ -875,7 +881,6 @@
             uint64_t tbc = 0, sprows = 0, cells = 0;
             uint32_t erec_cursor = 0;
             std::vector<QDesc> qd;
-            std::vector<uint32_t> chain_ref;
             while (r1 < bq) {
                 const uint32_t u = dag_of[r1];
                 const uint32_t N = bg.sizes[kSz * u];
@@ -894,7 +899,6 @@
                 d.erec_off = erec_cursor;
                 erec_cursor += dp_edge_entries(N);
                 qd.push_back(d);
-                chain_ref.push_back(fam_ids[fam_off[q0 + r1]]);
                 tbc += (uint64_t)N * Lp;
                 sprows += d.n_spill;
                 cells += (uint64_t)N * d.L;
@@ -908,7 +912,6 @@
                     cells -= (uint64_t)qd[r - r0].N * qd[r - r0].L;
                 }
                 qd.resize(r1r - r0);
-                chain_ref.resize(r1r - r0);
                 r1 = r1r;
             }
             const uint32_t rq = r1 - r0;
@@ -919,7 +922,7 @@
             c->profile_batch = profile_batch;
             c->out_pos_base = qbase - qoff[0];
             if (run_dp_device(c, pl, qd.data(), rq, (uint64_t)n_dags * bg.ncap, tbc, sprows, cells, nqm, p, c->st->width,
-                              out + q0 + r0, out_pos ? out_pos + qbase : nullptr, false, pp, profile_batch ? nullptr : chain_ref.data()))
+                              out + q0 + r0, out_pos ? out_pos + qbase : nullptr, false, pp, profile_batch ? 0u : bg.ncap))
                 return 1;
             r0 = r1;
         }
diff --git a/sina_amd/csrc/mesh_dp.hip b/sina_amd/csrc/mesh_dp.hip
--- a/sina_amd/csrc/mesh_dp.hip
+++ b/sina_amd/csrc/mesh_dp.hip
@@ -763,6 +763,104 @@
     }
 }
 
+template <int CTRL, int ROW_MASK = 0xf>
+__device__ __forceinline__ float dpp_mov(float old, float x) {
+    return __int_as_float(__builtin_amdgcn_update_dpp(__float_as_int(old), __float_as_int(x), CTRL, ROW_MASK, 0xf, false));
+}
+constexpr int kDppRowShr = 0x110, kDppWaveShl1 = 0x130, kDppWaveShr1 = 0x138, kDppBcast15 = 0x142, kDppBcast31 = 0x143;
+__device__ __forceinline__ float lane_value(float x, uint32_t k) {
+    return __int_as_float(__builtin_amdgcn_readlane(__float_as_int(x), (int)k));
+}
+
+__device__ __forceinline__ float chain_scout_wave(const uint4 *__restrict__ rec, const uint16_t *__restrict__ chain, uint32_t M,
+                                                  uint32_t N, uint32_t L, const uint8_t *__restrict__ qm, float ms, float mms,
+                                                  float gp, float gpe, int lane) {
+    constexpr float kUnreached = 1000000.0f;
+    const float inf = __builtin_inff();
+    int off = ((int)L - (int)M) / 2;
+    off = off < -24 ? -24 : (off > 24 ? 24 : off);
+    const int c0 = off - 32;
+    const float kg = (float)lane * gpe;
+    const float open = gp - gpe;
+    float pv = kUnreached, pg = kUnreached;
+    float best = inf;
+    auto q_at = [&](int s) -> uint32_t { return (s >= 0 && (uint32_t)s < L) ? (uint32_t)qm[s] : 0u; };
+    uint32_t q = q_at(lane + c0);
+    struct Block {
+        float vM, vX;
+        uint32_t z, qe;
+    };
+    auto load_rows = [&](uint32_t base) -> uint32_t {
+        const uint32_t ci = base + (uint32_t)lane;
+        return chain[ci < M ? ci : M - 1u];
+    };
+    auto load_block = [&](uint32_t base, uint32_t row) {
+        const uint32_t ci = base + (uint32_t)lane;
+        row = row < N ? row : N - 1u;
+        const uint4 r = rec[row];
+        const float wgt = __uint_as_float(r.y);
+        Block b;
+        b.vM = ms * wgt;
+        b.vX = mms * wgt;
+        b.z = r.z;
+        b.qe = q_at((int)ci + 1 + 63 + c0);
+        return b;
+    };
+    Block cur = load_block(0, load_rows(0));
+    uint32_t rows_nxt = load_rows(64u < M ? 64u : 0u);
+    for (uint32_t base = 0; base < M; base += 64u) {
+        const uint32_t b1 = base + 64u < M ? base + 64u : base, b2 = base + 128u < M ? base + 128u : base;
+        const Block nxt = load_block(b1, rows_nxt);
+        rows_nxt = load_rows(b2);
+        const uint32_t n_rows = M - base < 64u ? M - base : 64u;
+        for (uint32_t j = 0; j < n_rows; ++j) {
+            const int i = (int)(base + j);
+            const float vM = lane_value(cur.vM, j), vX = lane_value(cur.vX, j);
+            const uint32_t z = (uint32_t)__builtin_amdgcn_readlane((int)cur.z, (int)j);
+            const float csel = (q & ((z >> 8) & 0xfu)) != 0u ? vM : vX;
+            const float nv = dpp_mov<kDppWaveShl1>(kUnreached, pv), ng = dpp_mov<kDppWaveShl1>(kUnreached, pg);
+            float cand = __builtin_fminf(nv + gp, ng + gpe);
+            float loc = __builtin_fminf(pv + csel, cand);
+            float p = loc - kg;
+            const int k0 = -i - c0;
+            if ((uint32_t)k0 < 64u) {
+                asm volatile("" : "+v"(loc));
+                if (i == 0) {
+                    const bool source = (z & 0xffu) == 0u;
+                    loc = cand = ((source && lane >= k0) || lane == k0) ? 1.0f : kUnreached;
+                } else if (lane == k0) {
+                    loc = __builtin_fminf(cand, 1.0f);
+                }
+                p = loc - kg;
+                if (lane == k0 && loc == 1.0f) p -= open;
+            }
+            p = __builtin_fminf(p, dpp_mov<kDppRowShr + 1>(p, p));
+            p = __builtin_fminf(p, dpp_mov<kDppRowShr + 2>(p, p));
+            p = __builtin_fminf(p, dpp_mov<kDppRowShr + 4>(p, p));
+            p = __builtin_fminf(p, dpp_mov<kDppRowShr + 8>(p, p));
+            p = __builtin_fminf(p, dpp_mov<kDppBcast15, 0xa>(p, p));
+            p = __builtin_fminf(p, dpp_mov<kDppBcast31, 0xc>(p, p));
+            const float gs = (dpp_mov<kDppWaveShr1>(inf, p) + kg) + open;
+            const float fv = __builtin_fminf(loc, gs);
+            const int kl = (int)L - 1 - i - c0;
+            if (kl >= 0 && kl < 64) best = __builtin_fminf(best, lane_value(fv, (uint32_t)kl));
+            if (z & kRecSink) {
+                const int s = i + lane + c0;
+                float v = (s >= 0 && (uint32_t)s < L) ? fv : inf;
+#pragma unroll
+                for (int o = 32; o > 0; o >>= 1) v = __builtin_fminf(v, __shfl_xor(v, o));
+                best = __builtin_fminf(best, v);
+            }
+            pv = fv;
+            pg = cand;
+            const uint32_t qn = (uint32_t)__builtin_amdgcn_readlane((int)cur.qe, (int)j);
+            q = (uint32_t)__builtin_amdgcn_update_dpp((int)qn, (int)q, kDppWaveShl1, 0xf, 0xf, false);
+        }
+        cur = nxt;
+    }
+    return __uint_as_float(uniform(__float_as_uint(best)));
+}
+
 template <int B, bool DBG, bool PRUNE>
 __global__ void __launch_bounds__(64, (B <= 4 ? 4 : (B <= 8 ? SINA_DP_SIMPLE_WAVES8 : 2)))
 mesh_dp_simple_kernel(const QDesc *__restrict__ qdv, const uint32_t *__restrict__ orderv, const uint4 *__restrict__ recv,
@@ -770,7 +868,8 @@
                       float *__restrict__ dbg_value, float *spillv, EdgeRec *edgev, uint64_t edge_stride,
                       uint32_t n_strips, DpResult *__restrict__ resv, float ms, float mms, float gp, float gpe, DryArgs dry,
                       const uint2 *__restrict__ reachv, float prune_rho, uint32_t prune_amax, uint32_t n_slots,
-                      const float *__restrict__ scout_uv, float scout_bias) {
+                      float *__restrict__ scout_uv, float scout_bias, const uint16_t *__restrict__ chain_rowsv,
+                      const uint32_t *__restrict__ chain_sizesv, uint32_t chain_ncap) {
     static_assert(B % 4 == 0, "16-byte accesses per array");
     constexpr int kStrip = 64 * B;
     extern __shared__ __attribute__((aligned(16))) unsigned char smem[];
@@ -816,7 +915,18 @@
         gain0 = (float)g0 * kPruneUnit;
         U64 = -(int32_t)uniform((uint32_t)(int32_t)(prune_rho * (float)g0));
         if (scout_uv != nullptr) {
-            const float su = __uint_as_float(uniform(__float_as_uint(scout_uv[qi]))) + scout_bias;
+            float su;
+            if (chain_rowsv != nullptr) {
+                const uint32_t dag = (uint32_t)(node_off / chain_ncap);
+                uint32_t M = uniform(chain_sizesv[(size_t)dag * kBuiltWords + kBuiltChainLen]);
+                M = M < N ? M : N;
+                su = M > 0 ? chain_scout_wave(rec, chain_rowsv + node_off, M, N, L, qmaskv + q_off, ms, mms, gp, gpe, lane)
+                           : __builtin_inff();
+                if (lane == 0) scout_uv[qi] = su;
+            } else {
+                su = __uint_as_float(uniform(__float_as_uint(scout_uv[qi])));
+            }
+            su += scout_bias;
             if (su > -100000.0f && su < 100000.0f) {
                 const float up = su * 64.0f;
                 int32_t u = (int32_t)up;
@@ -1825,7 +1935,8 @@
         if (allow_full_lds(reinterpret_cast<const void *>(kfn))) return 1;
         hipLaunchKernelGGL(kfn, dim3(nq), dim3(64), lds, s, a.qd, a.order, a.rec, a.pred, a.qmask, a.tb, a.dbg_value, a.spill,
                            a.edge, a.edge_stride, n_strips, a.res, a.ms, a.mms, a.gp, a.gpe, a.dry, a.reach, a.prune_rho,
-                           a.prune_amax, (uint32_t)(lds / dp_slot_bytes(DpGeom{64 * (int)n_strips, B})), prune ? a.scout_u : nullptr, a.scout_bias);
+                           a.prune_amax, (uint32_t)(lds / dp_slot_bytes(DpGeom{64 * (int)n_strips, B})), prune ? a.scout_u : nullptr, a.scout_bias,
+                           prune ? a.chain_rows : nullptr, a.chain_sizes, a.chain_ncap);
     } else if (!weighted && !forbid && a.below_init) SH_LAUNCH(false, false, true);
     else if (!weighted && !forbid) SH_LAUNCH(false, false, false);
     else if (weighted && !forbid) SH_LAUNCH(true, false, false);
diff --git a/sina_amd/csrc/scout.hip b/sina_amd/csrc/scout.hip
--- a/sina_amd/csrc/scout.hip
+++ /dev/null
@@ -1,202 +0,0 @@
-#include <algorithm>
-
-#include "common.h"
-#include "ctx.h"
-
-namespace sina_hip {
-namespace {
-
-constexpr float kScoutDead = 1000000.0f;
-
-template <int K>
-__global__ void __launch_bounds__(64) chain_scout_kernel(const QDesc *__restrict__ qdv, const uint32_t *__restrict__ orderv,
-                                                         const uint4 *__restrict__ recv, const uint32_t *__restrict__ node_posv,
-                                                         const uint8_t *__restrict__ qmaskv, const uint32_t *__restrict__ ref_ab,
-                                                         const uint64_t *__restrict__ ref_off, const uint32_t *__restrict__ chain_ref,
-                                                         uint32_t nq, float ms, float mms, float gp, float gpe,
-                                                         float *__restrict__ out_u) {
-    static_assert(K % 4 == 0 && K >= 8 && K <= 32, "band width");
-    const uint32_t slot = blockIdx.x * 64u + threadIdx.x;
-    if (slot >= nq) return;
-    const uint32_t qi = orderv[slot];
-    const QDesc d = qdv[qi];
-    const uint32_t N = d.N, L = d.L;
-    const uint4 *__restrict__ rec = recv + d.node_off;
-    const uint32_t *__restrict__ node_pos = node_posv + d.node_off;
-    const uint32_t member = chain_ref[qi];
-    const uint64_t b0 = ref_off[member], b1 = ref_off[member + 1];
-    const int c_max = L > (uint32_t)K ? (int)(L - (uint32_t)K) : 0;
-    const float credit = (float)d.gmin * kPruneUnit;
-
-    float best = __builtin_inff();
-    float pv[K], pg[K];
-#pragma unroll
-    for (int k = 0; k < K; k++) pv[k] = pg[k] = kScoutDead;
-    int c = 0;
-    int a_rel = K / 2;
-    bool have_prev = false;
-    uint32_t m = 0;
-    uint32_t w[K / 4 + 1];
-#pragma unroll
-    for (int i = 0; i <= K / 4; i++) w[i] = 0u;
-    uint64_t w_at = ~(uint64_t)0 - 16;
-    uint32_t ab_next = b0 < b1 ? ref_ab[b0] : 0u;
-    uint32_t wpos[3] = {0xFFFFFFFFu, 0xFFFFFFFFu, 0xFFFFFFFFu};
-    uint4 wrec[3] = {};
-    auto load_window = [&](uint32_t at) {
-#pragma unroll
-        for (int i = 0; i < 3; i++) {
-            const uint32_t x = at + (uint32_t)i;
-            wpos[i] = x < N ? node_pos[x] : 0xFFFFFFFFu;
-            wrec[i] = rec[x < N ? x : 0];
-        }
-    };
-    load_window(0);
-    for (uint64_t bi = b0; bi < b1; ++bi) {
-        const uint32_t ab = ab_next;
-        if (bi + 1 < b1) ab_next = ref_ab[bi + 1];
-        const uint32_t col = ab & 0xFFFFFFu, bmask = (ab >> 24) & 31u;
-        uint32_t row = N;
-        uint4 r = wrec[0];
-        bool found = false;
-#pragma unroll
-        for (int i = 0; i < 3; i++)
-            if (!found && wpos[i] == col && ((wrec[i].z >> 8) & 31u) == bmask) {
-                found = true;
-                row = m + (uint32_t)i;
-                r = wrec[i];
-            }
-        if (!found) {
-            while (m < N && node_pos[m] < col) ++m;
-            row = m;
-            r = rec[row < N ? row : 0];
-            while (row < N && ((r.z >> 8) & 31u) != bmask) {
-                ++row;
-                if (row < N) r = rec[row];
-            }
-            if (row >= N || node_pos[row] != col) break;
-        }
-        m = row + 1;
-        load_window(m);
-        const uint32_t mmask = (r.z >> 8) & 0xfu;
-        const float wgt = __uint_as_float(r.y);
-        const float vM = ms * wgt, vX = mms * wgt;
-        int delta = 0;
-        if (have_prev) {
-            delta = a_rel + 1 - K / 2;
-            delta = delta < 0 ? 0 : (delta > 2 ? 2 : delta);
-        }
-        int cn = c + delta;
-        cn = cn > c_max ? c_max : cn;
-        delta = cn - c;
-        c = cn;
-        float csel[K];
-        {
-            const uint64_t at = d.q_off + (uint64_t)c;
-            const uint64_t at4 = at & ~(uint64_t)3;
-            if (at4 != w_at) {
-                const uint32_t *qw = reinterpret_cast<const uint32_t *>(qmaskv + at4);
-                if (at4 == w_at + 4) {
-#pragma unroll
-                    for (int i = 0; i < K / 4; i++) w[i] = w[i + 1];
-                    w[K / 4] = qw[K / 4];
-                } else {
-#pragma unroll
-                    for (int i = 0; i <= K / 4; i++) w[i] = qw[i];
-                }
-                w_at = at4;
-            }
-            const uint32_t sh = ((uint32_t)at & 3u) * 8u;
-#pragma unroll
-            for (int i = 0; i < K / 4; i++) {
-                const uint32_t x = sh ? ((w[i] >> sh) | (w[i + 1] << (32u - sh))) : w[i];
-#pragma unroll
-                for (int j = 0; j < 4; j++) {
-                    const int k = 4 * i + j;
-                    const uint32_t s = (uint32_t)c + (uint32_t)k;
-                    const uint32_t q = s < L ? ((x >> (8 * j)) & 0xfu) : 0u;
-                    csel[k] = (q & mmask) != 0u ? vM : vX;
-                }
-            }
-        }
-        const bool col0 = c == 0;
-        float loc[K], gm[K];
-        if (!have_prev) {
-            const bool source = (r.z & 0xffu) == 0u;
-#pragma unroll
-            for (int k = 0; k < K; k++) loc[k] = gm[k] = (source || (k == 0 && col0)) ? 1.0f : kScoutDead;
-        } else {
-            float sv[K + 1], sg[K];
-#pragma unroll
-            for (int k = 0; k <= K; k++) {
-                const float d0 = k >= 1 ? pv[k - 1] : kScoutDead;
-                const float d1 = k < K ? pv[k] : kScoutDead;
-                const float d2 = k + 1 < K ? pv[k + 1] : kScoutDead;
-                sv[k] = delta == 0 ? d0 : (delta == 1 ? d1 : d2);
-            }
-#pragma unroll
-            for (int k = 0; k < K; k++) {
-                const float d0 = pg[k];
-                const float d1 = k + 1 < K ? pg[k + 1] : kScoutDead;
-                const float d2 = k + 2 < K ? pg[k + 2] : kScoutDead;
-                sg[k] = delta == 0 ? d0 : (delta == 1 ? d1 : d2);
-            }
-#pragma unroll
-            for (int k = 0; k < K; k++) {
-                const float v = sv[k + 1] + gp;
-                const float g = sg[k] + gpe;
-                const float cand = v < g ? v : g;
-                gm[k] = cand;
-                float mv = sv[k] + csel[k];
-                float dv = cand;
-                if (k == 0 && col0) {
-                    mv = __builtin_inff();
-                    dv = cand < 1.0f ? cand : 1.0f;
-                }
-                loc[k] = mv < dv ? mv : dv;
-            }
-        }
-        float fv[K];
-        fv[0] = loc[0];
-        bool e_prev = col0 && fv[0] == 1.0f;
-#pragma unroll
-        for (int k = 1; k < K; k++) {
-            const float gsx = fv[k - 1] + (e_prev ? gpe : gp);
-            const bool ins = gsx <= loc[k];
-            fv[k] = ins ? gsx : loc[k];
-            e_prev = ins;
-        }
-        float vmin = __builtin_inff(), vcred = __builtin_inff();
-#pragma unroll
-        for (int k = 0; k < K; k++) {
-            const bool real = (uint32_t)c + (uint32_t)k < L;
-            fv[k] = real ? fv[k] : kScoutDead;
-            gm[k] = real ? gm[k] : kScoutDead;
-            vmin = fv[k] < vmin ? fv[k] : vmin;
-            const float cr = fv[k] + credit * (float)k;
-            if (cr < vcred) {
-                vcred = cr;
-                a_rel = k;
-            }
-            if ((uint32_t)c + (uint32_t)k == L - 1u) best = fv[k] < best ? fv[k] : best;
-            pv[k] = fv[k];
-            pg[k] = gm[k];
-        }
-        if (r.z & kRecSink) best = vmin < best ? vmin : best;
-        have_prev = true;
-    }
-    out_u[qi] = best;
-}
-
-}
-
-int launch_chain_scout(const DpArgs &a, uint32_t nq, const uint32_t *ref_ab, const uint64_t *ref_off,
-                       const uint32_t *chain_ref, float *out_u, hipStream_t s) {
-    const uint32_t blocks = (nq + 63u) / 64u;
-    hipLaunchKernelGGL((chain_scout_kernel<kScoutBand>), dim3(blocks), dim3(64), 0, s, a.qd, a.order, a.rec, a.node_pos,
-                       a.qmask, ref_ab, ref_off, chain_ref, nq, a.ms, a.mms, a.gp, a.gpe, out_u);
-    SH_CHECK(hipGetLastError());
-    return 0;
-}
-
-}
```
